# henryhcooperr/FaceRecognition-MultiArchitecture-Pipeline

Measured on AMD Instinct MI355X. Metric: faces/sec (224x224 embed+match), higher is better.
Workload: dtype bf16; 1 GPU; ResNet18 ('cnn') embed + L2-normalise + top-1 match, batch 256/GPU, 36-ID gallery, 224x224x3 fp32 NCHW inputs resident in HBM, seeded random-init weights with calibrated BatchNorm statistics (BASELINE.json configs[1]); global_batch=256, parallelism=dp1 (faces sharded, 1 all-gather of 8 B/face), execution=HIP graph replay, 2 concurrent micro-batch streams

## Files before the change

facerecognition-multiarchitecture-pipeline_amd/_lib.py:

```python
from __future__ import annotations

import ctypes as C
import os
import threading

_PKG_DIR = os.path.dirname(os.path.abspath(__file__))
LIB_PATH = os.environ.get("FRMAP_LIB") or os.path.join(_PKG_DIR, "libfrmap_hip.so")
ABI_VERSION = 10

_lock = threading.Lock()
_lib = None

_vp, _i, _f, _sz = C.c_void_p, C.c_int, C.c_float, C.c_size_t

PROTOTYPES = {
    "frmap_abi_version": (_i, []),
    "frmap_set_batch_invariant": (_i, [_i]),
    "frmap_last_error": (C.c_char_p, []),
    "frmap_pack_input_nchw_f32": (_i, [_vp, _vp, _i, _i, _i, _i, _vp]),
    "frmap_pack_conv_weight": (_i, [_vp, _vp, _i, _i, _i, _i, _i, _vp]),
    "frmap_small_cin_kpad": (_i, [_i, _i]),
    "frmap_pack_conv_weight_c3": (_i, [_vp, _vp, _i, _i, _i, _i, _vp]),
    "frmap_conv_small_cin": (_i, [_vp, _vp, _vp, _vp, _i, _i, _i, _i, _i, _i, _i, _i, _i, _i, _vp]),
    "frmap_match_gallery_pack_bytes": (_sz, [_i, _i]),
    "frmap_match_pack_gallery": (_i, [_vp, _vp, _vp, _i, _i, _vp]),
    "frmap_match_pack_gallery_rows": (_i, [_vp, _vp, _vp, _i, _i, _i, _i, _vp]),
    "frmap_match_top1_packed": (_i, [_vp, _vp, _vp, _vp, _vp, _vp, _vp, _vp, _f, _vp, _vp, _i, _i, _i, _vp]),
    "frmap_resize_bilinear_u8": (_i, [_vp, _vp, _vp, _vp, _i, _i, _i, _i, _i, _vp]),
    "frmap_crop_resize_u8": (_i, [_vp, _i, _vp, _vp, _i, _i, _i, _i, _i, _i, _vp]),
    "frmap_resize_coeffs_host": (_i, [_i, _i, _vp, _vp, _vp]),
    "frmap_align_crop_resize_u8": (_i, [_vp, _i, _vp, _vp, _vp, _i, _i, _i, _i, _i, _i, _vp]),
    "frmap_align_warp_host": (_i, [_vp, _i, _i, C.c_longlong, _vp, _i, _i, _i, _i, _i, _vp]),
    "frmap_track_state_bytes": (_sz, [_i, _i]),
    "frmap_track_step": (_i, [_vp, _vp, _vp, _vp, _vp, _i, _i, C.c_double, C.c_double, _vp, _vp, _vp]),
    "frmap_track_step_host": (_i, [_vp, _vp, _vp, _vp, _vp, _i, _i, C.c_double, C.c_double, _vp, _vp]),
    "frmap_track_fuse_state_bytes": (_sz, [_i, _i, _i]),
    "frmap_track_fuse": (_i, [_vp, _vp, _vp, _vp, _vp, _i, _i, _i, _i, _f, _vp, _vp, _vp]),
    "frmap_track_fuse_host": (_i, [_vp, _vp, _vp, _vp, _vp, _i, _i, _i, _i, _f, _vp, _vp]),
    "frmap_gap_linear_norm": (_i, [_vp, _vp, _vp, _vp, _vp, _vp, _f, _i, _i, _i, _i, _i, _i, _vp]),
    "frmap_conv_small_cin_pool2": (_i, [_vp, _vp, _vp, _vp, _i, _i, _i, _i, _i, _i, _vp]),
    "frmap_conv_igemm_pool2_supported": (_i, [_i, _i, _i, _i, _i]),
    "frmap_conv_igemm_pool2_form": (_i, [_i, _i, _i, _i, _i]),
    "frmap_conv3x3_pp_pool_layout": (_i, [_i, _i, _i, _i, _i]),
    "frmap_conv_igemm_pool2": (_i, [_vp, _vp, _vp, _vp, _i, _i, _i, _i, _i, _i, _i, _vp]),
    "frmap_stem7x7_maxpool": (_i, [_vp, _vp, _vp, _vp, _i, _i, _i, _i, _vp]),
    "frmap_stem7x7_maxpool2": (_i, [_vp, _vp, _vp, _vp, _i, _i, _i, _i, _vp]),
    "frmap_stem7x7_maxpool_u8": (_i, [_vp, C.POINTER(C.c_float), C.POINTER(C.c_float), _vp, _vp, _vp, _i, _i, _i, _i, _i, _vp]),
    "frmap_conv_igemm": (_i, [_vp, _vp, _vp, _vp, _vp, _i, _i, _i, _i, _i, _i, _i, _i, _i, _i, _vp]),
    "frmap_conv_pp_tuning": (_i, [_i, _i, _i]),
    "frmap_conv_pp_ri": (_i, [_i]),
    "frmap_conv_pp_pitch": (_i, [_i]),
    "frmap_conv_pp_ds": (_i, [_i]),
    "frmap_conv_pp_im": (_i, [_i]),
    "frmap_conv1x1_pp_layout": (_i, [_i, _i, _i, _i, _i, _i]),
    "frmap_conv3x3_pp_layout": (_i, [_i, _i, _i, _i, _i]),
    "frmap_conv3x3s2_pp_layout": (_i, [_i, _i, _i, _i, _i]),
    "frmap_conv3x3_pp_ds_layout": (_i, [_i, _i, _i, _i, _i, _i, _i, _i, _i]),
    "frmap_conv_igemm_ds_supported": (_i, [_i, _i, _i, _i, _i, _i, _i, _i, _i]),
    "frmap_conv_igemm_ds": (_i, [_vp, _vp, _vp, _vp, _vp, _vp, _i, _i, _i, _i, _i, _i, _i, _i, _i, _i, _i, _vp]),
    "frmap_linear_mfma_workspace_bytes": (_sz, [_i, _i, _i]),
    "frmap_linear_mfma": (_i, [_vp, _vp, _vp, _vp, _vp, _vp, _i, _i, _i, _i, _i, _vp]),
    "frmap_maxpool": (_i, [_vp, _vp, _i, _i, _i, _i, _i, _i, _i, _i, _vp]),
    "frmap_avgpool_global": (_i, [_vp, _vp, _i, _i, _i, _i, _vp]),
    "frmap_avgpool_adaptive": (_i, [_vp, _vp, _i, _i, _i, _i, _i, _i, _i, _vp]),
    "frmap_linear_f32": (_i, [_vp, _vp, _vp, _vp, _vp, _i, _i, _i, _i, _vp]),
    "frmap_l2_normalize_f32": (_i, [_vp, _vp, _i, _i, _f, _vp]),
    "frmap_cast_to_f32": (_i, [_vp, _vp, _sz, _i, _vp]),
    "frmap_cast_from_f32": (_i, [_vp, _vp, _sz, _i, _vp]),
    "frmap_add_pos_layernorm": (_i, [_vp, _vp, _vp, _vp, _vp, _vp, _i, _i, _i, _f, _i, _vp]),
    "frmap_mha_tokens": (_i, [_vp, _vp, _i, _i, _i, _i, _i, _vp]),
    "frmap_mean_layernorm": (_i, [_vp, _vp, _vp, _vp, _i, _i, _i, _f, _i, _vp]),
    "frmap_cnn_attention": (_i, [_vp, _vp, _vp, _vp, _vp, _vp, _vp, _i, _i, _i, _i, _i, _i, _i, _vp]),
    "frmap_normalize_u8_hwc": (_i, [_vp, _vp, _vp, _i, _i, _i, C.POINTER(C.c_float), C.POINTER(C.c_float), _i, _vp]),
    "frmap_softmax_argmax": (_i, [_vp, _vp, _vp, _i, _i, _vp]),
    "frmap_pairwise_distance": (_i, [_vp, _vp, _vp, _vp, _f, _i, _i, _vp]),
    "frmap_head_workspace_bytes": (_sz, [_i, _i]),
    "frmap_match_workspace_bytes": (_sz, [_i, _i]),
    "frmap_match_top1": (_i, [_vp, _vp, _vp, _vp, _vp, _vp, _f, _vp, _i, _i, _i, _vp]),
    "frmap_match_topk_workspace_bytes": (_sz, [_i, _i, _i, _i]),
    "frmap_match_topk": (_i, [_vp, _vp, _vp, _vp, _vp, _vp, _vp, _i, _i, _i, _i, _vp]),
    "frmap_match_topk_packed": (_i, [_vp, _vp, _vp, _vp, _vp, _vp, _vp, _vp, _vp, _i, _i, _i, _i, _vp]),
    "frmap_verify_workspace_bytes": (_sz, [_i, _i, _i, _i]),
    "frmap_verify_counts": (_i, [_vp, _vp, _i, _vp, _vp, _i, _i, _i, _vp, _i, _vp, _vp, _vp, _vp]),
    "frmap_verify_counts_packed": (_i, [_vp, _vp, _i, _vp, _vp, _vp, _vp, _i, _i, _i, _vp, _i, _vp, _vp, _vp, _vp]),
    "frmap_match_radius_workspace_bytes": (_sz, [_i, _i, _i]),
    "frmap_match_radius": (_i, [_vp, _vp, _i, _vp, _vp, _i, _i, _i, _f, _i, _vp, _vp, _vp, _vp, C.c_longlong, _vp, _vp, _vp]),
    "frmap_match_radius_packed": (_i, [_vp, _vp, _i, _vp, _vp, _vp, _vp, _i, _i, _i, _f, _i, _vp, _vp, _vp, _vp, C.c_longlong, _vp,
                                       _vp, _vp]),
    "frmap_gap_norm_match": (_i, [_vp, _vp, _vp, _vp, _vp, _vp, _vp, _f, _i, _f, _i, _i, _i, _i, _i, _vp]),
    "frmap_cosine_logits": (_i, [_vp, _vp, _vp, _vp, _vp, _i, _i, _i, _f, _vp]),
    "frmap_arcmargin_eval": (_i, [_vp, _vp, _vp, _vp, _vp, _vp, _i, _i, _i, _f, _f, _i, _vp]),
    "frmap_model_create": (_i, [C.POINTER(_vp), C.c_char_p, _i, _i]),
    "frmap_model_load_tensor": (_i, [_vp, C.c_char_p, _vp, _sz, _i]),
    "frmap_model_set_input_normalization": (_i, [_vp, C.POINTER(C.c_float), C.POINTER(C.c_float)]),
    "frmap_model_finalize": (_i, [_vp, _vp]),
    "frmap_model_embedding_dim": (_i, [_vp]),
    "frmap_model_workspace_bytes": (_sz, [_vp, _i, _i, _i]),
    "frmap_model_match_workspace_bytes": (_sz, [_vp, _i, _i, _i, _i]),
    "frmap_model_forward": (_i, [_vp, _vp, _i, _i, _i, _i, _i, _vp, _vp, _vp]),
    "frmap_model_embed_and_match": (_i, [_vp, _vp, _i, _i, _i, _i, _vp, _vp, _vp, _i, _f, _i, _vp, _vp, _vp, _vp, _vp, _vp, _vp]),
    "frmap_model_search_workspace_bytes": (_sz, [_vp, _i, _i, _i, _i, _i]),
    "frmap_model_embed_and_search": (_i, [_vp, _vp, _i, _i, _i, _i, _vp, _vp, _vp, _vp, _i, _i, _i, _vp, _vp, _vp, _vp, _vp, _vp]),
    "frmap_model_trace": (_i, [_vp, _i]),
    "frmap_model_trace_read": (_i, [_vp, _vp, _i]),
    "frmap_model_destroy": (None, [_vp]),
}


def lib_available() -> bool:
    return os.path.isfile(LIB_PATH)


def load() -> C.CDLL:
    global _lib
    if _lib is not None:
        return _lib
    with _lock:
        if _lib is not None:
            return _lib
        if not lib_available():
            raise RuntimeError(
                f"HIP extension not built: {LIB_PATH} is missing. Build it with "
                "`python -c 'import __graft_entry__ as g; g.build()'` (hipcc --offload-arch=gfx950). "
                "There is no CPU / PyTorch fallback for this path.")
        lib = C.CDLL(LIB_PATH)
        for name, (res, args) in PROTOTYPES.items():
            fn = getattr(lib, name)
            fn.restype = res
            fn.argtypes = args
        if lib.frmap_abi_version() != ABI_VERSION:
            raise RuntimeError(f"libfrmap_hip.so ABI {lib.frmap_abi_version()} != expected {ABI_VERSION}; rebuild")
        _lib = lib
    return _lib


def check(rc: int, what: str) -> None:
# ... 6 lines not shown
```

facerecognition-multiarchitecture-pipeline_amd/csrc/conv_igemm.hip:

```cpp
#include "frmap_common.h"
#include <stdlib.h>
#include <string.h>

struct ConvParams {
  const void* in;
  const void* wpk;
  const float* shift;
  const void* res;
  void* out;
  int N, Hi, Wi, Cin, Ho, Wo, Cout;
  int stride, pad, relu;
  int M, HoWo, Hp, Wp;
  uint32_t magic_Wp, magic_Hp;
  FrmapDiv dHoWo, dWo;
  int nchunks;
  int halo_bytes;
  int nblocks;
  int ksplit;
  float* slab;
  int dbg;
  const void* ds_in;
  const void* ds_w;
  int ds_Hi, ds_Wi, ds_Cin, ds_stride, ds_chunks;
  FrmapPoolOrder pool;
// ... 873 lines not shown
  u32x4_t hv[CKS][NIT], wv[CKS];
  auto prefetch = [&](int stg) {
#pragma unroll
    for (int sc = 0; sc < CKS; ++sc) {
#pragma unroll
      for (int it = 0; it < NIT; ++it) hv[sc][it] = *(const u32x4_t*)(inp + gsrc[it] + (size_t)(stg * CKS + sc) * 32);
      wv[sc] = *(const u32x4_t*)(wbase + (size_t)(stg * CKS + sc) * 4096);
    }
  };
  f32x4_t acc[MI][NI];
#pragma unroll
  for (int mi = 0; mi < MI; ++mi)
#pragma unroll
    for (int ni = 0; ni < NI; ++ni) acc[mi][ni] = (f32x4_t){0.f, 0.f, 0.f, 0.f};

  if (st_lo < st_hi) prefetch(st_lo);
  for (int stg = st_lo; stg < st_hi; ++stg) {
    if (stg > st_lo) __syncthreads();
#pragma unroll
    for (int sc = 0; sc < CKS; ++sc) {
      *(u32x4_t*)(wl + sc * 4096 + tid * 16) = wv[sc];
#pragma unroll
      for (int it = 0; it < NIT; ++it)
        *(u32x4_t*)(halo + sc * (BM * 64) + px_off<1>((it * 256 + tid) >> 2, tid & 3)) = hv[sc][it];
    }
    __syncthreads();
    if (stg + 1 < st_hi) prefetch(stg + 1);
#pragma unroll
    for (int sc = 0; sc < CKS; ++sc) {
      vec8 wf[NI], pf[MI];
#pragma unroll
      for (int ni = 0; ni < NI; ++ni) wf[ni] = *(const vec8*)(wl + sc * 4096 + ni * 1024 + woff);
#pragma unroll
      for (int mi = 0; mi < MI; ++mi) pf[mi] = *(const vec8*)(halo + sc * (BM * 64) + poff[mi]);
#pragma unroll
      for (int mi = 0; mi < MI; ++mi)
#pragma unroll
        for (int ni = 0; ni < NI; ++ni) acc[mi][ni] = TT::mfma(wf[ni], pf[mi], acc[mi][ni]);
    }
  }
  __syncthreads();
  if (p.ksplit > 1)
    conv_epilogue_partial<MI, NI>(acc, smem + wave * (16 * (NI * 64 + 16)), m0 + wave * 64, p.M, p.Cout, nt << 6,
                                  p.slab + (size_t)kslice * p.M * p.Cout, lane);
  else
    conv_epilogue<TT, MI, NI>(acc, smem + wave * (16 * (NI * 64 + 16)), m0 + wave * 64, p.M, p.Cout, nt << 6, p.shift,
                              (const typename TT::elem*)p.res, (typename TT::elem*)p.out, p.relu, lane);
}

template <typename TT>
__global__ void splitk_finalize_kernel(const float* __restrict__ slab, int ksplit, const float* __restrict__ shift,
                                       const typename TT::elem* __restrict__ res, typename TT::elem* __restrict__ out,
                                       size_t MN, int N, int act) {
  size_t i = ((size_t)blockIdx.x * blockDim.x + threadIdx.x) * 4;
  const size_t stride = (size_t)gridDim.x * blockDim.x * 4;
  for (; i < MN; i += stride) {
    f32x4_t a = *(const f32x4_t*)(slab + i);
    for (int s = 1; s < ksplit; ++s) {
      const f32x4_t b = *(const f32x4_t*)(slab + (size_t)s * MN + i);
      a[0] += b[0]; a[1] += b[1]; a[2] += b[2]; a[3] += b[3];
    }
    const int n = (int)(i % N);
    const f32x4_t sh = *(const f32x4_t*)(shift + n);
    float v[4] = {a[0] + sh[0], a[1] + sh[1], a[2] + sh[2], a[3] + sh[3]};
    if (res) {
      float r[4];
      unpack4<TT>(*(const u32x2_t*)(res + i), r);
      v[0] += r[0]; v[1] += r[1]; v[2] += r[2]; v[3] += r[3];
    }
#pragma unroll
    for (int e = 0; e < 4; ++e) {
      if (act == 1) v[e] = fmaxf(v[e], 0.f);
      else if (act == 2) v[e] = 0.5f * v[e] * (1.0f + erff(v[e] * 0.70710678118654752f));
    }
    *(u32x2_t*)(out + i) = pack4<TT>(v[0], v[1], v[2], v[3]);
  }
}

static ConvPlan plan_of(const ConvLayer& L) { return conv_plan(L, conv_tuning(), frmap_cu_count(), frmap_batch_invariant() != 0); }
ConvPlan frmap_conv_plan(const ConvLayer& L) { return plan_of(L); }

struct ConvPtrs {
  const void* in; const void* w; const float* shift; const void* res; void* out;
  const void* ds_in; const void* ds_w; float* slab;
};

static ConvParams conv_params(const ConvLayer& L, const ConvPlan& q, const ConvPtrs& a, int relu, int dbg) {
  ConvParams p{};
  p.in = a.in; p.wpk = a.w; p.shift = a.shift; p.res = a.res; p.out = a.out;
  p.N = L.B; p.Hi = L.Hi; p.Wi = L.Wi; p.Cin = L.Cin; p.Ho = L.Ho(); p.Wo = L.Wo(); p.Cout = L.Cout;
  p.stride = L.stride; p.pad = L.pad; p.relu = relu;
  p.M = L.B * p.Ho * p.Wo; p.HoWo = p.Ho * p.Wo; p.Hp = L.Hi + 2 * L.pad; p.Wp = q.Wp;
  p.magic_Wp = frmap_magic((uint32_t)p.Wp); p.magic_Hp = frmap_magic((uint32_t)p.Hp);
  p.dHoWo = frmap_div_make((uint32_t)p.HoWo); p.dWo = frmap_div_make((uint32_t)p.Wo);
  p.nchunks = L.Cin / 32 / (q.kernel == CK_1X1 ? q.CKS : 1);
  p.halo_bytes = q.halo_bytes; p.nblocks = q.nblocks;
  p.ksplit = q.ksplit; p.slab = a.slab; p.dbg = dbg;
  if (L.fuse == FUSE_SHORTCUT) {
    p.ds_in = a.ds_in; p.ds_w = a.ds_w; p.ds_Hi = L.ds_Hi; p.ds_Wi = L.ds_Wi; p.ds_Cin = L.ds_Cin; p.ds_stride = L.ds_stride;
    p.ds_chunks = L.ds_Cin / 32;
  }
  if (L.fuse == FUSE_POOL2) {
    p.pool.Wo2 = L.Wi / 2; p.pool.Win = (L.Hi / 2) * (L.Wi / 2);
    p.pool.dWo2 = frmap_div_make((uint32_t)p.pool.Wo2); p.pool.dWin = frmap_div_make((uint32_t)p.pool.Win);
  }
  return p;
}

typedef void (*conv_kern_t)(const ConvParams);
template <typename TT>
static conv_kern_t conv_kernel(const ConvPlan& q) {
  switch (q.kernel) {
    case CK_IGEMM:
      if (q.POOL) return q.BM == 256 ? conv_igemm_kernel<TT, 256, 3, 1, true> : conv_igemm_kernel<TT, 128, 3, 1, true>;
      if (q.KS == 1) return conv_igemm_kernel<TT, 256, 1, 1>;
      if (q.BM == 256) return q.SWZ == 1 ? conv_igemm_kernel<TT, 256, 3, 1> : conv_igemm_kernel<TT, 256, 3, 2>;
      return q.SWZ == 1 ? conv_igemm_kernel<TT, 128, 3, 1> : conv_igemm_kernel<TT, 128, 3, 2>;
    case CK_1X1: return q.CKS == 4 ? conv1x1_kernel<TT, 4> : (q.CKS == 2 ? conv1x1_kernel<TT, 2> : conv1x1_kernel<TT, 1>);
    case CK_WAVE:
      if (!q.POOL) return conv3x3_c64_wave_kernel<TT, 2, false>;
      return q.NCH == 2 ? conv3x3_c64_wave_kernel<TT, 2, true> : conv3x3_c64_wave_kernel<TT, 1, true>;
    case CK_FAST: return q.DS ? conv3x3_fast_kernel<TT, true> : conv3x3_fast_kernel<TT, false>;
    case CK_S2_SPLIT: return conv3x3s2_split_kernel<TT>;
    case CK_S2_FAST: return conv3x3s2_fast_kernel<TT>;
    default: return nullptr;
  }
}

static int conv_launch(const ConvPlan& q, const ConvParams& p, int dtype, hipStream_t st) {
  const conv_kern_t kern = dtype == FRMAP_BF16 ? conv_kernel<BF16>(q) : conv_kernel<F16>(q);
  FRMAP_REQUIRE(kern, "conv_igemm: no kernel for plan %d", q.kernel);
  if (frmap_big_lds((const void*)kern, 160 * 1024)) return -2;
  hipLaunchKernelGGL(kern, dim3(q.nblocks), dim3(q.kernel == CK_WAVE ? 512 : 256), q.lds_bytes, st, p);
  FRMAP_LAUNCH_CHECK();
  return 0;
}

static int conv_run(const ConvLayer& L, const ConvPlan& q, const ConvPtrs& a, int relu, int dtype, hipStream_t st) {
  if (q.kernel >= CK_PP) return frmap_conv_pp_launch(L, q, a.in, a.w, a.shift, a.res, a.out, a.ds_in, a.ds_w, relu, dtype, st);
  return conv_launch(q, conv_params(L, q, a, relu, L.fuse == FUSE_POOL2 ? 0 : conv_tuning().debug), dtype, st);
}

static int conv_igemm_impl(const ConvLayer& L, const ConvPtrs& a, int relu, int dtype, void* stream) {
  FRMAP_REQUIRE(a.in && a.w && a.shift && a.out, "conv_igemm: null pointer");
  FRMAP_REQUIRE(L.K == 1 || L.K == 3, "conv_igemm: kernel size %d not supported (1 or 3)", L.K);
  FRMAP_REQUIRE(L.stride == 1 || L.stride == 2, "conv_igemm: stride %d not supported", L.stride);
  FRMAP_REQUIRE((L.K == 3 && L.pad == 1) || (L.K == 1 && L.pad == 0), "conv_igemm: pad %d with K=%d not supported", L.pad, L.K);
  FRMAP_REQUIRE(L.Cin > 0 && L.Cin % 32 == 0, "conv_igemm: Cin=%d must be a multiple of 32", L.Cin);
  FRMAP_REQUIRE(L.Cout > 0 && L.Cout % 64 == 0, "conv_igemm: Cout=%d must be a multiple of 64", L.Cout);
  FRMAP_REQUIRE(dtype == FRMAP_BF16 || dtype == FRMAP_F16, "conv_igemm: bad dtype %d", dtype);
  FRMAP_REQUIRE(L.B > 0 && L.Hi > 0 && L.Wi > 0, "conv_igemm: empty input");
  FRMAP_REQUIRE(L.Ho() > 0 && L.Wo() > 0, "conv_igemm: empty output");
  FRMAP_REQUIRE((long long)L.B * L.Ho() * L.Wo() < (1ll << 31), "conv_igemm: too many output pixels");
  FRMAP_REQUIRE(L.Wi + 2 * L.pad < 32768 && L.Hi + 2 * L.pad < 32768, "conv_igemm: image too large");
  const ConvPlan q = plan_of(L);
  FRMAP_REQUIRE(q.taken(), "%s", q.error);
  return conv_run(L, q, a, relu, dtype, (hipStream_t)stream);
}

extern "C" int frmap_conv_igemm(const void* in, const void* w_packed, const float* shift, const void* residual,
                                void* out, int B, int Hi, int Wi, int Cin, int Cout, int K, int stride, int pad,
                                int relu, int dtype, void* stream) {
  const ConvLayer L = {B, Hi, Wi, Cin, Cout, K, stride, pad, residual ? FUSE_RESIDUAL : FUSE_NONE, 0, 0, 0, 0};
  return conv_igemm_impl(L, ConvPtrs{in, w_packed, shift, residual, out, nullptr, nullptr, nullptr}, relu, dtype, stream);
}

extern "C" int frmap_conv_igemm_ds_supported(int B, int Hi, int Wi, int Cin, int Cout, int ds_Hi, int ds_Wi, int ds_Cin,
                                             int ds_stride) {
  const ConvLayer L = {B, Hi, Wi, Cin, Cout, 3, 1, 1, FUSE_SHORTCUT, ds_Hi, ds_Wi, ds_Cin, ds_stride};
  return conv_ds_supported(L, conv_tuning(), frmap_batch_invariant() != 0);
}

extern "C" int frmap_conv_igemm_ds(const void* in, const void* w_packed, const float* shift, const void* ds_in,
                                   const void* ds_w_packed, void* out, int B, int Hi, int Wi, int Cin, int Cout,
                                   int ds_Hi, int ds_Wi, int ds_Cin, int ds_stride, int relu, int dtype, void* stream) {
  FRMAP_REQUIRE(ds_in && ds_w_packed, "conv_igemm_ds: null shortcut pointer");
  const ConvLayer L = {B, Hi, Wi, Cin, Cout, 3, 1, 1, FUSE_SHORTCUT, ds_Hi, ds_Wi, ds_Cin, ds_stride};
  return conv_igemm_impl(L, ConvPtrs{in, w_packed, shift, nullptr, out, ds_in, ds_w_packed, nullptr}, relu, dtype, stream);
}

extern "C" int frmap_conv_igemm_pool2_form(int B, int Hi, int Wi, int Cin, int Cout) {
  return plan_of(ConvLayer{B, Hi, Wi, Cin, Cout, 3, 1, 1, FUSE_POOL2, 0, 0, 0, 0}).layout;
}
extern "C" int frmap_conv_igemm_pool2_supported(int B, int Hi, int Wi, int Cin, int Cout) {
  const int f = frmap_conv_igemm_pool2_form(B, Hi, Wi, Cin, Cout);
  return f >= 2 || (f == 1 && Cin <= 96);
}

extern "C" int frmap_conv_igemm_pool2(const void* in, const void* w_packed, const float* shift, void* out, int B, int Hi,
                                      int Wi, int Cin, int Cout, int relu, int dtype, void* stream) {
  FRMAP_REQUIRE(in && w_packed && shift && out, "conv_igemm_pool2: null pointer");
  FRMAP_REQUIRE(dtype == FRMAP_BF16 || dtype == FRMAP_F16, "conv_igemm_pool2: bad dtype %d", dtype);
  FRMAP_REQUIRE(relu == 0 || relu == 1, "conv_igemm_pool2: activation %d does not commute with the max", relu);
  const ConvLayer L = {B, Hi, Wi, Cin, Cout, 3, 1, 1, FUSE_POOL2, 0, 0, 0, 0};
  const ConvPlan q = plan_of(L);
  FRMAP_REQUIRE(q.taken(),
                "conv_igemm_pool2: shape B=%d %dx%d Cin=%d Cout=%d not taken (even H and W, Cin %% 32 == 0, Cout %% 64 == 0, rows fit LDS)",
                B, Hi, Wi, Cin, Cout);
  return conv_run(L, q, ConvPtrs{in, w_packed, shift, nullptr, out, nullptr, nullptr, nullptr}, relu, dtype, (hipStream_t)stream);
}

extern "C" size_t frmap_linear_mfma_workspace_bytes(int M, int K, int N) {
  if (M <= 0 || K <= 0 || N <= 0) return 0;
  const int ks = linear_ksplit(M, K, N, frmap_batch_invariant() != 0);
  return ks > 1 ? (size_t)ks * M * N * sizeof(float) : 0;
}

extern "C" int frmap_linear_mfma(const void* x, const void* w_packed, const float* shift, const void* residual, void* out,
                                 void* workspace, int M, int K, int N, int act, int dtype, void* stream) {
  FRMAP_REQUIRE(x && w_packed && shift && out, "linear_mfma: null pointer");
  FRMAP_REQUIRE(M > 0 && K > 0 && K % 32 == 0 && N > 0 && N % 64 == 0, "linear_mfma: need K %% 32 == 0 and N %% 64 == 0 (M=%d K=%d N=%d)", M, K, N);
  FRMAP_REQUIRE(dtype == FRMAP_BF16 || dtype == FRMAP_F16, "linear_mfma: bad dtype");
  const int ks = linear_ksplit(M, K, N, frmap_batch_invariant() != 0);
  if (ks == 1) return frmap_conv_igemm(x, w_packed, shift, residual, out, M, 1, 1, K, N, 1, 1, 0, act, dtype, stream);
  FRMAP_REQUIRE(workspace, "linear_mfma: workspace required (frmap_linear_mfma_workspace_bytes)");
  const ConvLayer L = {M, 1, 1, K, N, 1, 1, 0, FUSE_NONE, 0, 0, 0, 0};
  const ConvPlan q = plan_1x1(L, ks);
  if (q.ksplit < 2) return frmap_conv_igemm(x, w_packed, shift, residual, out, M, 1, 1, K, N, 1, 1, 0, act, dtype, stream);
  hipStream_t st = (hipStream_t)stream;
  const int rc = conv_launch(q, conv_params(L, q, ConvPtrs{x, w_packed, shift, nullptr, out, nullptr, nullptr, (float*)workspace}, 0, 0), dtype, st);
  if (rc) return rc;
  const size_t MN = (size_t)M * N;
  const int blocks = (int)((MN / 4 + 255) / 256 < 4096 ? (MN / 4 + 255) / 256 : 4096);
  if (dtype == FRMAP_BF16)
    hipLaunchKernelGGL(splitk_finalize_kernel<BF16>, dim3(blocks), dim3(256), 0, st, (const float*)workspace, q.ksplit, shift,
                       (const __bf16*)residual, (__bf16*)out, MN, N, act);
  else
    hipLaunchKernelGGL(splitk_finalize_kernel<F16>, dim3(blocks), dim3(256), 0, st, (const float*)workspace, q.ksplit, shift,
                       (const _Float16*)residual, (_Float16*)out, MN, N, act);
  FRMAP_LAUNCH_CHECK();
  return 0;
}
```

facerecognition-multiarchitecture-pipeline_amd/csrc/conv_plan.cpp:

```cpp
#include "conv_plan.h"

#include <stdio.h>
#include <stdlib.h>
#include <string.h>

#include <array>
#include <map>
#include <mutex>

static int env_int(const char* name, int dflt) {
  const char* e = getenv(name);
  return e ? atoi(e) : dflt;
}

ConvTuning& conv_tuning() {
  static ConvTuning t = [] {
    ConvTuning v{};
    v.debug = env_int("FRMAP_CONV_DEBUG", 0);
    v.s2fast = env_int("FRMAP_CONV_S2FAST", 1);
    v.wres = env_int("FRMAP_CONV_WRES", 1);
    v.dsfuse = env_int("FRMAP_CONV_DSFUSE", 1);
    v.ds_unfuse_small = env_int("FRMAP_DS_UNFUSE_SMALL", 0);
    v.pool_wave = env_int("FRMAP_POOL_WAVE", 1);
    v.pool_min_cin = env_int("FRMAP_PP_POOL_MIN_CIN", 128);
    v.pp = env_int("FRMAP_CONV_PP", 1);
    v.pp_s2 = env_int("FRMAP_CONV_PP_S2", 1);
    v.pp_pool = env_int("FRMAP_CONV_PP_POOL", 1);
    v.pp_1x1 = env_int("FRMAP_CONV_PP_1X1", 1);
    v.pp_ds = env_int("FRMAP_CONV_PP_DS", 1);
    v.min_tiles = env_int("FRMAP_PP_MIN_TILES", 200);
    v.min_cin = env_int("FRMAP_PP_MIN_CIN", 128);
    v.s2_min_cin = env_int("FRMAP_PP_S2_MIN_CIN", 64);
    v.tile_px = env_int("FRMAP_PP_TILE_PX", 0);
    v.bn = env_int("FRMAP_PP_BN", 0);
    v.pitch = env_int("FRMAP_PP_PITCH", 0);
    v.ri = env_int("FRMAP_PP_RI", 0);
    v.im = env_int("FRMAP_PP_IM", 0);
    v.h_on = v.h_px = v.h_bn = v.h_ks = v.h_ds = v.h_pitch = v.h_im = v.h_ri = -1;
    return v;
  }();
  return t;
}

static const long long LDS_MAX = 160 * 1024, LDS_HALF = 80 * 1024;

static long long round1k(long long v) { return (v + 1023) & ~1023ll; }

static int plan_lds(const ConvPlan& q) {
  int lds = 0, scratch = 4 * 16 * (4 * 64 + 16);
  const int wb = (q.KS == 2 ? 2 : 8 / (q.WM ? q.WM : 8)) * 64 * 64;
  const int xch = q.KS == 2 ? 4 * q.MI * 4 * 1024 : 0;
  switch (q.kernel) {
    case CK_IGEMM: case CK_FAST: lds = q.halo_bytes + q.KS * q.KS * 4096; break;
    case CK_S2_SPLIT: case CK_S2_FAST: lds = q.halo_bytes + 6 * 4096; break;
    case CK_1X1: lds = q.CKS * (256 * 64 + 4096); break;
    case CK_WAVE: lds = q.NCH * 9 * 4096 + 8 * (10 * 16 * 64); break;
    case CK_PP:
      lds = q.KS * (2 * q.NHP * (8 / q.KS) * 1024 + (q.RI && q.KS == 1 ? 5 : 4) * wb) + (q.DS ? ((q.WM * q.MI + 7) / 8) * 8192 : 0);
      break;
    case CK_PP_S2: lds = 4 * q.NHP * 8192 + 4 * wb; break;
    case CK_PP_1X1: {
      const int cap = (q.KS == 2 ? 2 : q.WM) * q.MI * 16, gw = 8 / q.KS, ngp = (cap / 16 + gw - 1) / gw;
      lds = q.KS * (3 * ngp * gw * 1024 + 4 * wb);
      break;
    }
  }
  if (q.kernel >= CK_PP) scratch *= 2;
  if (lds < scratch) lds = scratch;
  if (q.kernel >= CK_PP && lds < xch) lds = xch;
  return lds;
}
static ConvPlan finish(ConvPlan q, const char* label) {
  q.label = label;
  if (q.kernel >= CK_PP) q.nblocks = q.mtiles * q.ntiles;
  if (!q.ksplit) q.ksplit = 1;
  if (!q.wg_per_cu) q.wg_per_cu = 1;
  q.lds_bytes = plan_lds(q);
  return q;
}

static int halo_rows_bound(int BM, int Ho, int Wo, int Hp, int stride, int KS) {
  const int rows = (BM + Wo - 2) / Wo + 1;
  const int cross = (BM + Ho * Wo - 2) / (Ho * Wo);
  const int cross_step = Hp - (Ho - 1) * stride;
  const int x = cross < rows - 1 ? cross : rows - 1;
  int gdiff = (rows - 1 - x) * stride + x * (cross_step > stride ? cross_step : stride);
  return gdiff + KS;
}
static int pool_rows_bound(int BM, int Ho, int Wo) {
  const int nw = BM / 4, Wo2 = Wo / 2, Win = (Ho / 2) * Wo2;
  const int pairs = (nw + Wo2 - 2) / Wo2 + 1;
  const int cross = (nw + Win - 2) / Win;
  const int x = cross < pairs - 1 ? cross : pairs - 1;
  return 2 * pairs + 2 * x + 2;
}
static bool prefetch_offsets_fit(int HoWo, long long H, long long W, long long C) { return (256 / HoWo + 3) * H * W * C * 2 < (1ll << 31); }

int pp_max_rows(long long M, int tile_px, int howo, int wo, int hp, int extra, bool inv) {
  if (inv) M = (long long)howo * tile_px;
  static std::mutex mu;
  static std::map<std::array<long long, 6>, int> memo;
  const std::array<long long, 6> key = {M, tile_px, howo, wo, hp, extra};
  {
    std::lock_guard<std::mutex> lock(mu);
    auto it = memo.find(key);
    if (it != memo.end()) return it->second;
  }
  int best = 0;
  const long long mtiles = (M + tile_px - 1) / tile_px;
  const long long lim = mtiles < howo ? mtiles : howo;
  for (long long mt = 0; mt < lim; ++mt) {
    const long long m0 = mt * tile_px, mend = (m0 + tile_px < M ? m0 + tile_px : M) - 1;
    const long long n0 = m0 / howo, n1 = mend / howo;
    const int oy0 = (int)((m0 - n0 * howo) / wo), oy1 = (int)((mend - n1 * howo) / wo);
    const int rows = (int)(n1 - n0) * hp + oy1 - oy0 + extra;
    if (rows > best) best = rows;
  }
  {
    std::lock_guard<std::mutex> lock(mu);
    if (memo.size() > 4096) memo.clear();
    memo[key] = best;
  }
  return best;
}

static int pp_tile_px(int cap, int H, int W, int forced_env, int forced_hook) {
  int tile_px;
  if (H * W <= cap) tile_px = (cap / (H * W)) * H * W;
  else {
    int rows = cap / W;
    for (int r = rows; r * 8 >= rows * 7 && r >= 1; --r)
      if (H % r == 0) { rows = r; break; }
    tile_px = rows * W;
  }
  if (forced_env > 0 && forced_env <= cap) tile_px = forced_env;
  if (forced_hook > 0 && forced_hook <= cap) tile_px = forced_hook;
  return tile_px;
}
static int pp_bn(int Cout, int forced_env, int forced_hook) {
  int bn = Cout % 256 == 0 ? 256 : 128;
  if (forced_env == 128 || forced_env == 256) bn = (forced_env == 256 && Cout % 256) ? 128 : forced_env;
  if (forced_hook == 128 || forced_hook == 256) bn = (forced_hook == 256 && Cout % 256) ? 128 : forced_hook;
  return bn;
}
static bool pp_sizes_fit(long long M, long long in_elems) { return M < (1ll << 31) && in_elems * 2 < (1ll << 46); }

ConvPlan plan_pp_3x3(const ConvLayer& L, const ConvTuning& t, bool inv) {
  constexpr int MI = 7;
  ConvPlan q{};
  const int B = L.B, Hi = L.Hi, Wi = L.Wi, Cin = L.Cin, Cout = L.Cout;
  const bool has_ds = L.fuse == FUSE_SHORTCUT;
  if (!t.pp_enabled(1, Cin, t.min_cin)) return q;
  if (Cin % 32 || Cin > 1024 || Cout % 128) return q;
  const long long Mll = (long long)B * Hi * Wi;
  if (!pp_sizes_fit(Mll, Mll * Cin)) return q;
  const int Hp = Hi + 2;
  int Wp = Wi + 2;
  if (ConvTuning::pick(t.h_pitch, t.pitch)) { while (Wp % 8 != Wi % 8) ++Wp; }
  if (has_ds) {
    if (L.ds_Cin <= 0 || L.ds_Cin % 32 || L.ds_stride < 1 || (L.ds_Hi - 1) / L.ds_stride + 1 != Hi ||
        (L.ds_Wi - 1) / L.ds_stride + 1 != Wi || (long long)B * L.ds_Hi * L.ds_Wi * L.ds_Cin * 2 >= (1ll << 46))
      return q;
    if (!ConvTuning::pick(t.h_ds, t.pp_ds) && !t.forced()) return q;
  }
  auto layout = [&](int cap, int bn, int ks, int& tile_px, int& mtiles, int& ntiles, int& hbytes_out) -> int {
    if (Wi > cap || Cout % bn || (ks == 2 && (Cin / 32) % 2)) return 0;
    tile_px = pp_tile_px(cap, Hi, Wi, t.tile_px, t.h_px);
    mtiles = (int)((Mll + tile_px - 1) / tile_px);
    ntiles = Cout / bn;
    const long long hbytes = (long long)pp_max_rows(Mll, tile_px, Hi * Wi, Wi, Hp, 3, inv) * Wp * 64;
    if (hbytes / 64 >= 65536) return 0;
    hbytes_out = (int)hbytes;
    const int per = (8 / ks) * 1024;
    const int nhp = (int)((hbytes + per - 1) / per);
    return nhp <= (ks == 2 ? 6 : 5) ? nhp : 0;
  };
  int tpx = 0, mtl = 0, ntl = 0, hby = 0, ks = 1, bn = pp_bn(Cout, t.bn, t.h_bn);
  int nhp = layout(bn == 256 ? 2 * MI * 16 : 4 * MI * 16, bn, 1, tpx, mtl, ntl, hby);
  const bool want_ks2 = !has_ds && !inv && (t.h_ks == 2 || (t.h_ks < 0 && (!nhp || (long long)mtl * ntl < t.min_tiles)));
  if (want_ks2 && t.h_ks != 1) {
    int t2 = 0, m2 = 0, n2 = 0, h2 = 0;
    const int nhp2 = layout(2 * MI * 16, 128, 2, t2, m2, n2, h2);
    if (nhp2 && (t.h_ks == 2 || !nhp || (long long)m2 * n2 > (long long)mtl * ntl)) {
      nhp = nhp2; tpx = t2; mtl = m2; ntl = n2; hby = h2; ks = 2; bn = 128;
    }
  }
  if (!nhp) return q;
  if (!inv && !t.forced() && (long long)mtl * ntl < t.min_tiles / 2) return q;
  if (!inv && has_ds && (long long)mtl * ntl < t.min_tiles && !t.forced()) return q;
  q.kernel = CK_PP; q.MI = MI; q.KS = ks; q.DS = has_ds;
  q.tile_px = tpx; q.mtiles = mtl; q.ntiles = ntl; q.Wp = Wp; q.halo_bytes = hby;
  q.layout = ks == 2 ? 3 : (bn == 256 ? 1 : 2);
  q.WM = bn == 256 || ks == 2 ? 2 : 4;
  if (has_ds) {
    q.NHP = bn == 256 && nhp <= 3 ? 3 : 5;
    return finish(q, "conv3x3_pp_kernel<%s, DS>");
  }
  q.RI = ConvTuning::pick(t.h_ri, t.ri) != 0 && !(ks == 2 && nhp > 4);
  q.IM = !q.RI && ConvTuning::pick(t.h_im, t.im) != 0;
  q.NHP = ks == 2 ? (nhp <= 4 ? 4 : 6) : (nhp <= 3 ? 3 : 5);
  return finish(q, "conv3x3_pp_kernel<%s>");
}

ConvPlan plan_pp_s2(const ConvLayer& L, const ConvTuning& t, bool inv) {
  constexpr int MI = 7;
  ConvPlan q{};
  const int B = L.B, Hi = L.Hi, Wi = L.Wi, Cin = L.Cin, Cout = L.Cout;
  if (!t.pp_enabled(t.pp_s2, Cin, t.s2_min_cin)) return q;
  if (Hi % 2 || Wi % 2 || Cin % 32 || Cin > 1024 || Cout % 128) return q;
  const int Ho = Hi / 2, Wo = Wi / 2;
  const long long Mll = (long long)B * Ho * Wo;
  if (!pp_sizes_fit(Mll, (long long)B * Hi * Wi * Cin) || (long long)Hi * Wi * Cin * 2 >= (1ll << 31)) return q;
  const int bn = pp_bn(Cout, 0, t.h_bn);
  const int cap = (bn == 256 ? 2 : 4) * MI * 16;
  if (Wo > cap) return q;
  const int tile_px = pp_tile_px(cap, Ho, Wo, 0, t.h_px);
  q.MI = MI; q.WM = bn == 256 ? 2 : 4; q.KS = 1;
  q.Wp = Wo + 1;
  q.tile_px = tile_px;
  q.mtiles = (int)((Mll + tile_px - 1) / tile_px);
  q.ntiles = Cout / bn;
  const long long hbytes = (long long)pp_max_rows(Mll, tile_px, Ho * Wo, Wo, Ho + 1, 2, inv) * q.Wp * 64;
  if (hbytes / 64 >= 65536) return q;
  q.halo_bytes = (int)hbytes;
  const int need = (int)((hbytes + 8191) / 8192);
  q.NHP = need <= 1 ? 1 : (need <= 2 ? 2 : (need <= 4 ? 4 : 0));
  if (!q.NHP || (q.NHP == 4 && bn == 256)) return q;
  if (!inv && !t.forced() && (long long)q.mtiles * q.ntiles < t.min_tiles) return q;
  q.kernel = CK_PP_S2;
  q.layout = bn == 256 ? 1 : 2;
  return finish(q, "conv3x3s2_pp_kernel<%s>");
}

ConvPlan plan_pp_pool(const ConvLayer& L, const ConvTuning& t, bool inv) {
  ConvPlan q{};
  const int B = L.B, Hi = L.Hi, Wi = L.Wi, Cin = L.Cin, Cout = L.Cout;
  if (!t.pp_enabled(t.pp_pool, Cin, 0)) return q;
  if (Hi % 2 || Wi % 2 || 112 % (2 * Wi) || Cin % 32 || Cin > 1024 || Cout % 128) return q;
  const long long Mll = (long long)B * Hi * Wi;
  if (!pp_sizes_fit(Mll, Mll * Cin)) return q;
  q.Wp = Wi + 2;
  int bn = pp_bn(Cout, 0, t.h_bn), nhp = 0;
  for (int attempt = 0; attempt < 2 && !nhp; ++attempt) {
    const int tile_px = (bn == 256 ? 2 : 4) * 112;
    const long long hbytes = (long long)pp_max_rows(Mll, tile_px, Hi * Wi, Wi, Hi + 2, 3, inv) * q.Wp * 64;
    const int n = (int)((hbytes + 8191) / 8192);
    if (hbytes / 64 < 65536 && n <= 5) { nhp = n; q.tile_px = tile_px; q.halo_bytes = (int)hbytes; }
    else bn = bn == 256 ? 128 : 256;
    if (!nhp && Cout % bn) break;
  }
  if (!nhp) return q;
  q.kernel = CK_PP; q.PL = true; q.MI = 7; q.KS = 1;
  q.WM = bn == 256 ? 2 : 4; q.NHP = nhp <= 3 ? 3 : 5;
  q.mtiles = (int)((Mll + q.tile_px - 1) / q.tile_px); q.ntiles = Cout / bn;
  q.layout = 3;
  return finish(q, "conv3x3_pp_kernel<%s, PL>");
}

ConvPlan plan_pp_1x1(const ConvLayer& L, const ConvTuning& t, int cus, bool inv) {
  ConvPlan q{};
  const int B = L.B, Hi = L.Hi, Wi = L.Wi, Cin = L.Cin, Cout = L.Cout, stride = L.stride;
  if (!t.pp_enabled(t.pp_1x1, Cin, 0)) return q;
  if (inv && !t.forced()) return q;
  if (Cin % 32 || Cin > 16384 || Cout % 128 || stride < 1) return q;
  const int Ho = (Hi - 1) / stride + 1, Wo = (Wi - 1) / stride + 1, nchunks = Cin / 32;
  const long long Mll = (long long)B * Ho * Wo;
  if (!pp_sizes_fit(Mll, (long long)B * Hi * Wi * Cin)) return q;
  auto est_us = [&](int lay) -> double {
    if (lay == 1 && Cout % 256) return 1e30;
    if (lay == 3 && nchunks % 2) return 1e30;
    const int px = lay == 2 ? 448 : 224, bn = lay == 1 ? 256 : 128;
    const long long tiles = ((Mll + px - 1) / px) * (Cout / bn);
    const long long rounds = (tiles + cus - 1) / cus;
    return (double)rounds * ((lay == 3 ? nchunks / 2 : nchunks) * 0.6 + 7.5);
  };
  int layout = 0;
  double best = 1e30;
  for (int lay = 1; lay <= 3; ++lay) {
    if (t.h_bn == 256 && t.h_ks != 2 && lay != 1 && Cout % 256 == 0) continue;
    if (t.h_bn == 128 && t.h_ks == 1 && lay != 2) continue;
    if (t.h_ks == 2 && lay != 3 && nchunks % 2 == 0) continue;
    const double e = est_us(lay);
    if (e < best) { best = e; layout = lay; }
  }
  if (!layout || best >= 1e30) return q;
  if (!t.forced()) {
    const double gen1_us = 2.0 * (double)Mll * Cin * Cout / 470e6;
    if (best > 0.9 * gen1_us || t.min_tiles < 0) return q;
  }
  q.kernel = CK_PP_1X1; q.MI = 7; q.WM = layout == 2 ? 4 : 2; q.KS = layout == 3 ? 2 : 1;
  q.Wp = Wo;
  q.tile_px = layout == 2 ? 448 : 224;
  q.mtiles = (int)((Mll + q.tile_px - 1) / q.tile_px);
  q.ntiles = Cout / (layout == 1 ? 256 : 128);
  q.layout = layout;
  return finish(q, "conv1x1_pp_kernel<%s>");
}

ConvPlan match_gemm_plan(int P, int Gpad) {
  const long long t1 = ((P + 223) / 224) * (long long)(Gpad / 256), t2 = ((P + 447) / 448) * (long long)(Gpad / 128);
  const long long r1 = (t1 + 255) / 256, r2 = (t2 + 255) / 256;
  const bool wide = r2 < r1 || (r2 == r1 && t2 > t1);
  ConvPlan q{};
  q.kernel = CK_PP_1X1; q.MI = 7; q.WM = wide ? 4 : 2; q.KS = 1;
  q.Wp = 1;
  q.tile_px = wide ? 448 : 224;
  q.mtiles = (P + q.tile_px - 1) / q.tile_px;
  q.ntiles = Gpad / (wide ? 128 : 256);
  q.layout = wide ? 2 : 1;
  return finish(q, "conv1x1_pp_kernel<F16, MATCH>");
}

ConvPlan plan_wave(const ConvLayer& L, const ConvTuning& t, int cus) {
// ... 145 lines not shown
```

facerecognition-multiarchitecture-pipeline_amd/csrc/conv_plan.h:

```cpp
#pragma once
#include <stdint.h>

struct ConvTuning {
  int debug;
  int s2fast;
  int wres;
  int dsfuse;
  int ds_unfuse_small;
  int pool_wave;
  int pool_min_cin;
  int pp;
  int pp_s2, pp_pool, pp_1x1;
  int pp_ds;
  int min_tiles;
  int min_cin;
  int s2_min_cin;
  int tile_px, bn;
  int pitch;
  int ri;
  int im;
  int h_on, h_px, h_bn, h_ks, h_ds, h_pitch, h_im, h_ri;

  void set_tuning(int enable, int px, int bn_) {
    h_on = enable;
    h_px = px;
    h_bn = bn_ == 1282 ? 128 : bn_;
    h_ks = bn_ == 1282 ? 2 : (bn_ == 128 || bn_ == 256 ? 1 : -1);
  }
  bool forced() const { return h_on >= 0; }
  bool pp_enabled(int family_on, int cin, int cin_min) const { return h_on >= 0 ? h_on != 0 : (pp && family_on && cin >= cin_min); }
  static int pick(int hook, int env) { return hook >= 0 ? hook : env; }
};
ConvTuning& conv_tuning();

enum ConvFuse { FUSE_NONE = 0, FUSE_RESIDUAL, FUSE_SHORTCUT, FUSE_POOL2 };
struct ConvLayer {
  int B, Hi, Wi, Cin, Cout, K, stride, pad;
  int fuse;
  int ds_Hi, ds_Wi, ds_Cin, ds_stride;
  int Ho() const { return (Hi + 2 * pad - K) / stride + 1; }
  int Wo() const { return (Wi + 2 * pad - K) / stride + 1; }
};

enum ConvKernel {
  CK_NONE = 0,
  CK_IGEMM,
  CK_1X1,
  CK_WAVE,
  CK_FAST,
  CK_S2_SPLIT,
  CK_S2_FAST,
  CK_PP,
  CK_PP_S2,
  CK_PP_1X1,
};
struct ConvPlan {
  int kernel;
  int BM, KS, SWZ, CKS, NCH;
  int MI, WM, NHP;
  bool DS, IM, PL, RI, POOL;
  int tile_px, mtiles, ntiles;
  int nblocks;
  int halo_bytes, Wp, lds_bytes, ksplit;
  int wg_per_cu;
  int layout;
  const char* label;
  char error[112];
  bool taken() const { return kernel != CK_NONE; }
};

ConvPlan plan_pp_3x3(const ConvLayer& L, const ConvTuning& t, bool inv);
ConvPlan plan_pp_s2(const ConvLayer& L, const ConvTuning& t, bool inv);
ConvPlan plan_pp_pool(const ConvLayer& L, const ConvTuning& t, bool inv);
ConvPlan plan_pp_1x1(const ConvLayer& L, const ConvTuning& t, int cus, bool inv);
ConvPlan plan_wave(const ConvLayer& L, const ConvTuning& t, int cus);
ConvPlan plan_fast(const ConvLayer& L, const ConvTuning& t);
ConvPlan plan_s2(const ConvLayer& L, const ConvTuning& t);
ConvPlan plan_1x1(const ConvLayer& L, int ksplit);
ConvPlan plan_generic(const ConvLayer& L);

ConvPlan conv_plan(const ConvLayer& L, const ConvTuning& t, int cus, bool inv);

int conv_ds_supported(const ConvLayer& L, const ConvTuning& t, bool inv);

int linear_ksplit(int M, int K, int N, bool inv);
ConvPlan match_gemm_plan(int P, int Gpad);

int pp_max_rows(long long M, int tile_px, int howo, int wo, int hp, int extra, bool inv);
```

facerecognition-multiarchitecture-pipeline_amd/csrc/conv_pp.hip:

```cpp
#include "frmap_common.h"
#include <stdlib.h>
#include <string.h>

#include <utility>

struct PPParams {
  const void* in;
  const void* wpk;
  const float* shift;
  const void* res;
  void* out;
  int N, Hi, Wi, Cin, Cout, relu;
  int M, HoWo, Hp, Wp;
  uint32_t magic_Wp, magic_Hp;
  FrmapDiv dHoWo, dWo;
  int nchunks;
  int tile_px;
  int mtiles, ntiles;
  const void* ds_in;
  const void* ds_w;
  int ds_Hi, ds_Wi, ds_Cin, ds_stride, dsc;
  int Wo2;
  FrmapDiv dWo2;
  const float* m_stat_a;
  const float* m_stat_w;
  void* m_records;
  int m_G, m_D;
};
struct PPHistParams : PPParams {
  const float* h_A;
  const float* h_B;
  const int32_t* h_lab_a;
  const int32_t* h_lab_b;
  const float* h_tab;
  unsigned long long* h_hist;
  unsigned long long* h_rescored;
  int h_row0, h_T;
};
struct PPJoinParams : PPParams {
  const float* j_A;
  const float* j_B;
  const int32_t* j_lab_a;
  const int32_t* j_lab_b;
  RadiusOut j_out;
  unsigned long long* j_rescored;
  float j_hi;
  int j_row0, j_filter;
};
template <int MM> struct PPArg { using type = PPParams; };
template <> struct PPArg<MATCH_HIST> { using type = PPHistParams; };
template <> struct PPArg<MATCH_JOIN> { using type = PPJoinParams; };
__device__ __forceinline__ bool pp_hist_self(const PPParams&) { return false; }
__device__ __forceinline__ bool pp_hist_self(const PPHistParams& p) { return p.h_row0 >= 0; }
__device__ __forceinline__ bool pp_hist_self(const PPJoinParams& p) { return p.j_row0 >= 0; }

__device__ __attribute__((aligned(4096))) unsigned int g_pp_zero[1024];

__device__ __forceinline__ int pp_xcd_remap(int b, int nb) {
  const int qd = nb >> 3, rm = nb & 7, xcd = b & 7;
  return (xcd < rm ? xcd * (qd + 1) : rm * (qd + 1) + (xcd - rm) * qd) + (b >> 3);
}

__device__ __forceinline__ void pp_dma16(const void* gsrc, unsigned lds_base) {
  unsigned keep;
  asm volatile("s_mov_b32 %0, m0\n\ts_mov_b32 m0, %2\n\ts_nop 0\n\tglobal_load_lds_dwordx4 %1, off\n\ts_mov_b32 m0, %0"
               : "=&s"(keep)
               : "v"(gsrc), "s"(lds_base)
               : "memory");
}
template <int N>
__device__ __forceinline__ void pp_wait_vm() {
  asm volatile("s_waitcnt vmcnt(%0)" ::"i"(N) : "memory");
}
__device__ __forceinline__ void pp_wait_lgkm0() { asm volatile("s_waitcnt lgkmcnt(0)" ::: "memory"); }
__device__ __forceinline__ void pp_barrier() {
  __builtin_amdgcn_sched_barrier(0);
  asm volatile("s_barrier" ::: "memory");
  __builtin_amdgcn_sched_barrier(0);
}

template <int... Is, typename F>
__device__ __forceinline__ void pp_static_for(std::integer_sequence<int, Is...>, F&& f) {
  (f(std::integral_constant<int, Is>{}), ...);
}

template <typename TT, int MI, int WM, int NHP, int KS, bool DS, bool IM = false, bool PL = false, bool RI = false>
__global__ __launch_bounds__(512, 2) void conv3x3_pp_kernel(const PPParams p) {
  static_assert(!(DS && KS == 2), "the fused shortcut is built for the pixel-split layouts only");
  static_assert(!RI || (!DS && !IM), "the interleaved fragment reads are built for the plain layers");
  static_assert(!PL || (KS == 1 && !DS && !IM), "the pooled epilogue is built for the plain pixel-split layouts");
  static_assert(!(DS && IM), "the fused shortcut keeps its DMA in the LOAD segments");
  constexpr int NI = 4, WN = KS == 2 ? 2 : 8 / WM;
  constexpr int CAP = WM * MI * 16;
  constexpr int NGP = DS ? (CAP / 16 + 7) / 8 : 0;
  constexpr int GBYTES = NGP * 8 * 1024;
  constexpr int XT = DS ? 8 - NHP : 1;
  constexpr int PPT = DS ? (NGP + XT - 1) / XT : 0;
  constexpr int TAPS = 9, BN = WN * 64, WB = BN * 64;
  constexpr int GW = 8 / KS;
  constexpr int NWI = (WB / 1024) / GW;
  constexpr int RING = (RI && KS == 1) ? 5 : 4;
  constexpr int HB = NHP * GW * 1024;
  constexpr int GSZ = 2 * HB + RING * WB;
  constexpr int PD = (RI && KS == 1) ? 3 : 2;
  auto slot_of = [](int k) { return RING == 4 ? (k & 3) : k % RING; };
  using vec8 = typename TT::vec8;
  using elem = typename TT::elem;
  extern __shared__ __attribute__((aligned(16))) char smem[];
  const unsigned lds0 = (unsigned)(uintptr_t)(__attribute__((address_space(3))) char*)smem;
  const int tid = threadIdx.x, lane = tid & 63;
  const int wave = __builtin_amdgcn_readfirstlane(tid >> 6);
  const int grp = wave >> 2, q = wave & 3;
  const int gw = KS == 2 ? q : wave;
  const int wn = (KS == 2 || WM == 4) ? (wave & 1) : q;
  const int mslice = KS == 2 ? (q >> 1) : (WM == 2 ? grp : grp * 2 + (q >> 1));
  const int gbase = KS == 2 ? grp * GSZ : 0;
  const int lr = lane & 15, g = lane >> 4;

  const int L = pp_xcd_remap(blockIdx.x, gridDim.x);
  const int mt = L / p.ntiles, nt = L - mt * p.ntiles;
  const int m0 = mt * p.tile_px, mend = min(m0 + p.tile_px, p.M);
  const int nch = p.nchunks / KS;
  const int nk = nch * TAPS;

  const int n0 = frmap_div(m0, p.dHoWo), oy0 = frmap_div(m0 - n0 * p.HoWo, p.dWo);
  const int n1 = frmap_div(mend - 1, p.dHoWo), oy1 = frmap_div(mend - 1 - n1 * p.HoWo, p.dWo);
  const int nrows = (n1 - n0) * p.Hp + oy1 - oy0 + 3;
  const int nitems = nrows * p.Wp * 4;

  const char* hsrc[NHP];
#pragma unroll
  for (int j = 0; j < NHP; ++j) {
    const int item = ((gw + GW * j) << 6) + lane;
    const int px = item >> 2, ps = item & 3;
    const int cg = ps ^ (((px >> 2) & 1) << 1);
    const int r = (int)fast_div((uint32_t)px, p.magic_Wp);
    const int c = px - r * p.Wp;
    const int rr = oy0 + r;
    const int dn = (int)fast_div((uint32_t)rr, p.magic_Hp);
    const int iy = rr - dn * p.Hp - 1, ix = c - 1, n = n0 + dn;
    const bool ok = item < nitems && n < p.N && (unsigned)iy < (unsigned)p.Hi && (unsigned)ix < (unsigned)p.Wi;
    hsrc[j] = ok ? (const char*)p.in + ((((size_t)n * p.Hi + iy) * p.Wi + ix) * p.Cin + cg * 8) * sizeof(elem)
                 : (const char*)g_pp_zero + cg * 16;
  }
  const int wblk = NWI == 2 ? (gw >> 1) : (gw >> 2);
  const int wpart = NWI == 2 ? ((gw & 1) << 1) : (gw & 3);
  const char* wsrc = (const char*)p.wpk + ((size_t)(nt * (BN / 64) + wblk) * p.nchunks * TAPS) * 4096 + wpart * 1024 + lane * 16;
  const unsigned wdst = lds0 + gbase + 2 * HB + wblk * 4096 + wpart * 1024;
  const unsigned hdst = lds0 + gbase + gw * 1024;

  const char* gsrc[DS ? NGP : 1];
  const char* wsrc_ds = nullptr;
  if (DS) {
    const size_t img = (size_t)p.ds_Hi * p.ds_Wi * p.ds_Cin;
#pragma unroll
    for (int e = 0; e < NGP; ++e) {
      const int item = ((wave + 8 * e) << 6) + lane;
      const int px = item >> 2, ps = item & 3;
      const int cg = ps ^ (((px >> 2) & 1) << 1);
      const int m = m0 + px;
      const int n = frmap_div(min(m, p.M - 1), p.dHoWo), rem = min(m, p.M - 1) - n * p.HoWo, oy = frmap_div(rem, p.dWo), ox = rem - oy * p.Wi;
      gsrc[e] = (px < CAP && m < mend)
                    ? (const char*)p.ds_in + ((size_t)n * img + ((size_t)(oy * p.ds_stride) * p.ds_Wi + ox * p.ds_stride) * p.ds_Cin + cg * 8) * sizeof(elem)
                    : (const char*)g_pp_zero + cg * 16;
    }
    wsrc_ds = (const char*)p.ds_w + ((size_t)(nt * (BN / 64) + wblk) * p.dsc) * 4096 + wpart * 1024 + lane * 16;
  }
  auto gbuf = [&](int d) -> unsigned {
    const int r = d % 3;
    return r == 0 ? (unsigned)(nch & 1) * HB : (r == 1 ? (unsigned)(2 * HB + RING * WB) : (unsigned)((nch - 1) & 1) * HB);
// ... 163 lines not shown
        for (int mi = 0; mi < MI; ++mi) asm volatile("" : "+v"(A[mi]));
#pragma unroll
        for (int mi = 0; mi < MI; ++mi) {
#pragma unroll
          for (int ni = 0; ni < NI; ++ni) acc[mi][ni] = TT::mfma(CUR ? wf1[ni] : wf0[ni], pf[mi], acc[mi][ni]);
          __builtin_amdgcn_sched_barrier(0);
          pf[mi] = *(const vec8*)(hb1 + frag_addr(mi, toff1));
          if (mi < NI) {
            if (CUR) wf0[mi] = *(const vec8*)(sl1 + mi * 1024);
            else wf1[mi] = *(const vec8*)(sl1 + mi * 1024);
          }
          __builtin_amdgcn_sched_barrier(0);
        }
        pp_barrier();
      });
    };
    int ci = 0;
    for (; ci + 1 < nch; ci += 2) {
      chunk_ri(ci, std::integral_constant<int, 0>{});
      chunk_ri(ci + 1, std::integral_constant<int, 1>{});
    }
    if (ci < nch) chunk_ri(ci, std::integral_constant<int, 0>{});
  } else if (DS) {
    for (int ci = 0; ci + 1 < nch; ++ci) chunk_body(ci, std::false_type{});
    chunk_body(nch - 1, std::true_type{});
  } else {
    for (int ci = 0; ci < nch; ++ci) chunk_body(ci, std::false_type{});
  }
  if (DS) {
    int Ag[MI];
#pragma unroll
    for (int mi = 0; mi < MI; ++mi) {
      const int at = ((((mslice * MI + mi) << 4) + lr) << 6) | (g << 4);
      Ag[mi] = at ^ ((at >> 3) & 32);
    }
    for (int d = 0; d < p.dsc; ++d) {
      const int k = nk + d;
      vec8 wf[NI], pf[MI];
      {
        const char* sl = slabs + slot_of(k) * WB;
#pragma unroll
        for (int ni = 0; ni < NI; ++ni) wf[ni] = *(const vec8*)(sl + ni * 1024);
        const char* gb = smem + gbuf(d);
#pragma unroll
        for (int mi = 0; mi < MI; ++mi) pf[mi] = *(const vec8*)(gb + Ag[mi]);
      }
#pragma unroll
      for (int e = 0; e < NGP; ++e) issue_gather(d + 2, e);
      issue_slab(nch + (d + 2) / TAPS, (d + 2) % TAPS, slot_of(k + 2));
      pp_wait_vm<NWI + NGP>();
      pp_wait_lgkm0();
      pp_barrier();
      __builtin_amdgcn_sched_barrier(0);
#pragma unroll
      for (int ni = 0; ni < NI; ++ni)
#pragma unroll
        for (int mi = 0; mi < MI; ++mi) acc[mi][ni] = TT::mfma(wf[ni], pf[mi], acc[mi][ni]);
      pp_barrier();
    }
  }
  if (grp == 0) pp_barrier();
  pp_wait_vm<0>();
  pp_barrier();

  if (KS == 2) {
    char* xch = smem + (size_t)q * (MI * NI * 1024) + lane * 16;
    if (grp == 1) {
#pragma unroll
      for (int mi = 0; mi < MI; ++mi)
#pragma unroll
        for (int ni = 0; ni < NI; ++ni) *(f32x4_t*)(xch + (mi * NI + ni) * 1024) = acc[mi][ni];
    }
    __syncthreads();
    if (grp == 0) {
#pragma unroll
      for (int mi = 0; mi < MI; ++mi)
#pragma unroll
        for (int ni = 0; ni < NI; ++ni) {
          const f32x4_t o = *(const f32x4_t*)(xch + (mi * NI + ni) * 1024);
          acc[mi][ni][0] += o[0]; acc[mi][ni][1] += o[1]; acc[mi][ni][2] += o[2]; acc[mi][ni][3] += o[3];
        }
    }
    __syncthreads();
    if (grp == 1) return;
  }

  if constexpr (PL)
    conv_epilogue_pool2<TT, MI, NI>(acc, smem + wave * (16 * (NI * 64 + 16)), (m0 + mslice * (MI * 16)) >> 2, mend >> 2, p.Cout,
                                    nt * BN + wn * 64, p.shift, (elem*)p.out, p.relu, lane);
  else
    conv_epilogue<TT, MI, NI>(acc, smem + (KS == 2 ? q : wave) * (16 * (NI * 64 + 16)), m0 + mslice * (MI * 16), mend, p.Cout,
                              nt * BN + wn * 64, p.shift, (const elem*)p.res, (elem*)p.out, p.relu, lane);
}

template <typename TT, int MI, int WM, int KS, int MM = MATCH_NONE>
__global__ __launch_bounds__(512, 2) void conv1x1_pp_kernel(const typename PPArg<MM>::type p) {
  constexpr int NI = 4, WN = KS == 2 ? 2 : 8 / WM;
  constexpr int CAP = (KS == 2 ? 2 : WM) * MI * 16;
  constexpr int BN = WN * 64, WB = BN * 64;
  constexpr int GW = 8 / KS;
  constexpr int NWI = (WB / 1024) / GW;
  constexpr int NGP = (CAP / 16 + GW - 1) / GW;
  constexpr int IMGB = NGP * GW * 1024;
  constexpr int RING = 4;
  constexpr int GSZ = 3 * IMGB + RING * WB;
  using vec8 = typename TT::vec8;
  using elem = typename TT::elem;
  extern __shared__ __attribute__((aligned(16))) char smem[];
  const unsigned lds0 = (unsigned)(uintptr_t)(__attribute__((address_space(3))) char*)smem;
  const int tid = threadIdx.x, lane = tid & 63;
  const int wave = __builtin_amdgcn_readfirstlane(tid >> 6);
  const int grp = wave >> 2, q = wave & 3;
  const int gw = KS == 2 ? q : wave;
  const int wn = (KS == 2 || WM == 4) ? (wave & 1) : q;
  const int mslice = KS == 2 ? (q >> 1) : (WM == 2 ? grp : grp * 2 + (q >> 1));
  const int gbase = KS == 2 ? grp * GSZ : 0;
  const int lr = lane & 15, g = lane >> 4;

  const int L = pp_hist_self(p) ? (int)blockIdx.x : pp_xcd_remap(blockIdx.x, gridDim.x);
  const int mt = L / p.ntiles, nt = L - mt * p.ntiles;
  const int m0 = mt * p.tile_px, mend = min(m0 + p.tile_px, p.M);
  if constexpr (MM == MATCH_HIST) {
    if (p.h_row0 >= 0 && nt * BN + BN - 1 <= p.h_row0 + m0) return;
  }
  if constexpr (MM == MATCH_JOIN) {
    if (p.j_row0 >= 0 && nt * BN + BN - 1 <= p.j_row0 + m0) return;
  }
  const int nst = p.nchunks / KS;

  const char* gsrc[NGP];
#pragma unroll
  for (int e = 0; e < NGP; ++e) {
    const int item = ((gw + GW * e) << 6) + lane;
    const int px = item >> 2, ps = item & 3;
    const int cg = ps ^ (((px >> 2) & 1) << 1);
    const int m = min(m0 + px, p.M - 1);
    const int n = frmap_div(m, p.dHoWo), rem = m - n * p.HoWo, oy = frmap_div(rem, p.dWo), ox = rem - oy * p.Wp;
    gsrc[e] = (px < CAP && m0 + px < mend)
                  ? (const char*)p.in + ((((size_t)n * p.Hi + (size_t)(oy * p.ds_stride)) * p.Wi + (size_t)(ox * p.ds_stride)) * p.Cin + cg * 8) * sizeof(elem)
                  : (const char*)g_pp_zero + cg * 16;
  }
  const int wblk = NWI == 2 ? (gw >> 1) : (gw >> 2);
  const int wpart = NWI == 2 ? ((gw & 1) << 1) : (gw & 3);
  const char* wsrc = (const char*)p.wpk + ((size_t)(nt * (BN / 64) + wblk) * p.nchunks) * 4096 + wpart * 1024 + lane * 16;
  const unsigned wdst = lds0 + gbase + 3 * IMGB + wblk * 4096 + wpart * 1024;
  const unsigned gdst = lds0 + gbase + gw * 1024;

  auto chunk_of = [&](int st) { return KS == 2 ? grp + 2 * st : st; };
  auto issue_step = [&](int st) {
    const int sc = st < nst ? st : nst - 1;
    const size_t coff = (size_t)chunk_of(sc) * 64;
#pragma unroll
    for (int e = 0; e < NGP; ++e)
      pp_dma16(st < nst ? gsrc[e] + coff : (const char*)g_pp_zero, gdst + (unsigned)(st % 3) * IMGB + e * (GW * 1024));
    const char* sp = wsrc + (size_t)chunk_of(sc) * 4096;
    const unsigned dp = wdst + (unsigned)(st & (RING - 1)) * WB;
    pp_dma16(sp, dp);
    if (NWI == 2) pp_dma16(sp + 1024, dp + 1024);
  };
  issue_step(0);
  issue_step(1);

  int Ag[MI];
#pragma unroll
  for (int mi = 0; mi < MI; ++mi) {
    const int at = ((((mslice * MI + mi) << 4) + lr) << 6) | (g << 4);
    Ag[mi] = at ^ ((at >> 3) & 32);
// ... 14 lines not shown

  for (int st = 0; st < nst; ++st) {
    vec8 wf[NI], pf[MI];
    {
      const char* sl = slabs + (st & (RING - 1)) * WB;
#pragma unroll
      for (int ni = 0; ni < NI; ++ni) wf[ni] = *(const vec8*)(sl + ni * 1024);
      const char* gb = imgs + (st % 3) * IMGB;
#pragma unroll
      for (int mi = 0; mi < MI; ++mi) pf[mi] = *(const vec8*)(gb + Ag[mi]);
    }
    issue_step(st + 2);
    pp_wait_vm<NWI + NGP>();
    pp_wait_lgkm0();
    pp_barrier();
    __builtin_amdgcn_sched_barrier(0);
#pragma unroll
    for (int ni = 0; ni < NI; ++ni)
#pragma unroll
      for (int mi = 0; mi < MI; ++mi) acc[mi][ni] = TT::mfma(wf[ni], pf[mi], acc[mi][ni]);
    pp_barrier();
  }
  if (grp == 0) pp_barrier();
  pp_wait_vm<0>();
  pp_barrier();

  if (KS == 2) {
    char* xch = smem + (size_t)q * (MI * NI * 1024) + lane * 16;
    if (grp == 1) {
#pragma unroll
      for (int mi = 0; mi < MI; ++mi)
#pragma unroll
        for (int ni = 0; ni < NI; ++ni) *(f32x4_t*)(xch + (mi * NI + ni) * 1024) = acc[mi][ni];
    }
    __syncthreads();
    if (grp == 0) {
#pragma unroll
      for (int mi = 0; mi < MI; ++mi)
#pragma unroll
        for (int ni = 0; ni < NI; ++ni) {
          const f32x4_t o = *(const f32x4_t*)(xch + (mi * NI + ni) * 1024);
          acc[mi][ni][0] += o[0]; acc[mi][ni][1] += o[1]; acc[mi][ni][2] += o[2]; acc[mi][ni][3] += o[3];
        }
    }
    __syncthreads();
    if (grp == 1) return;
  }
  if constexpr (MM == MATCH_HIST) {
    unsigned* hist = (unsigned*)(smem + VERIFY_LDS_HIST);
    float* tl = (float*)(smem + VERIFY_LDS_T);
    const int T = p.h_T, nb = 2 * (T + 1);
    for (int i = tid; i < nb; i += 512) hist[i] = 0u;
    for (int i = tid; i < 3 * T; i += 512) tl[(i / T) * VERIFY_MAX_T + i % T] = p.h_tab[i];
    __syncthreads();
    const int b_base = m0 + mslice * (MI * 16), n0 = nt * BN + wn * 64;
    unsigned short* queue = (unsigned short*)(smem + VERIFY_LDS_Q) + wave * VERIFY_QCAP;
    const int cnt = match_epilogue_hist<MI>(acc, b_base, mend, n0, p.m_G, p.m_D, p.M, p.m_stat_a, p.m_stat_w, p.h_lab_a, p.h_lab_b,
                                            p.h_row0, (const float*)(smem + VERIFY_LDS_LO), (const float*)(smem + VERIFY_LDS_HI),
                                            hist, queue, T, lane);
    verify_drain_queue(queue, cnt, b_base, n0, p.h_A, p.h_B, p.h_lab_a, p.h_lab_b, p.m_D, tl, hist, T, lane);
    if (lane == 0 && cnt) atomicAdd(p.h_rescored, (unsigned long long)cnt);
    __syncthreads();
    for (int i = tid; i < nb; i += 512)
      if (hist[i]) atomicAdd(p.h_hist + i, (unsigned long long)hist[i]);
    return;
  } else if constexpr (MM == MATCH_JOIN) {
    const int b_base = m0 + mslice * (MI * 16), n0 = nt * BN + wn * 64;
    unsigned short* queue = (unsigned short*)smem + wave * VERIFY_QCAP;
    const int cnt = match_epilogue_join<MI>(acc, b_base, mend, n0, p.m_G, p.m_D, p.M, p.m_stat_a, p.m_stat_w, p.j_lab_a, p.j_lab_b,
                                            p.j_row0, p.j_filter, p.j_hi, queue, lane);
    int* obuf = (int*)(smem + 8 * VERIFY_QCAP * 2 + wave * RADIUS_OB_BYTES);
    radius_drain_queue(queue, cnt, b_base, n0, p.j_A, p.j_B, p.m_D, p.j_out, obuf, lane);
    if (lane == 0 && cnt) atomicAdd(p.j_rescored, (unsigned long long)cnt);
    return;
  } else if constexpr (MM != MATCH_NONE) {
    match_epilogue<MM, MI>(acc, m0 + mslice * (MI * 16), mend, nt * BN + wn * 64, p.m_G, p.m_D, p.M, p.m_stat_a, p.m_stat_w,
                           p.m_records, lane);
    return;
  }
  conv_epilogue<TT, MI, NI>(acc, smem + (KS == 2 ? q : wave) * (16 * (NI * 64 + 16)), m0 + mslice * (MI * 16), mend, p.Cout,
                            nt * BN + wn * 64, p.shift, (const elem*)p.res, (elem*)p.out, p.relu, lane);
}

template <typename TT, int MI, int WM, int NHP2>
__global__ __launch_bounds__(512, 2) void conv3x3s2_pp_kernel(const PPParams p) {
  constexpr int NI = 4, WN = 8 / WM;
  constexpr int TAPS = 9, BN = WN * 64, WB = BN * 64;
  constexpr int NWI = (WB / 1024) / 8;
  constexpr int RING = 4;
  constexpr int HB = NHP2 * 8 * 1024;
  constexpr int PPH = NHP2 >= 2 ? NHP2 / 2 : 1;
  using vec8 = typename TT::vec8;
  using elem = typename TT::elem;
  extern __shared__ __attribute__((aligned(16))) char smem[];
  const unsigned lds0 = (unsigned)(uintptr_t)(__attribute__((address_space(3))) char*)smem;
  const int tid = threadIdx.x, lane = tid & 63;
  const int wave = __builtin_amdgcn_readfirstlane(tid >> 6);
  const int grp = wave >> 2, q = wave & 3;
  const int wn = WM == 4 ? (wave & 1) : q;
  const int mslice = WM == 2 ? grp : grp * 2 + (q >> 1);
  const int lr = lane & 15, g = lane >> 4;

  const int L = pp_xcd_remap(blockIdx.x, gridDim.x);
  const int mt = L / p.ntiles, nt = L - mt * p.ntiles;
  const int m0 = mt * p.tile_px, mend = min(m0 + p.tile_px, p.M);
  const int nch = p.nchunks, nk = nch * TAPS;
  const int Wo = p.Wi >> 1;

  const int n0 = frmap_div(m0, p.dHoWo), oy0 = frmap_div(m0 - n0 * p.HoWo, p.dWo);
  const int n1 = frmap_div(mend - 1, p.dHoWo), oy1 = frmap_div(mend - 1 - n1 * p.HoWo, p.dWo);
  const int nrows = (n1 - n0) * p.Hp + oy1 - oy0 + 2;
  const int nitems = nrows * p.Wp * 4;

  const char* hsrc[NHP2];
  unsigned hval = 0;
#pragma unroll
  for (int j = 0; j < NHP2; ++j) {
    const int item = ((wave + 8 * j) << 6) + lane;
    const int px = item >> 2, ps = item & 3;
    const int cg = ps ^ (((px >> 2) & 1) << 1);
    const int r = (int)fast_div((uint32_t)px, p.magic_Wp);
    const int c = px - r * p.Wp;
    const int rr = oy0 + r;
    const int dn = (int)fast_div((uint32_t)rr, p.magic_Hp);
    const int yh = rr - dn * p.Hp - 1, xh = c - 1, n = n0 + dn;
    const bool ok = item < nitems && n < p.N && yh >= 0 && xh >= 0;
    hsrc[j] = ok ? (const char*)p.in + ((((size_t)n * p.Hi + 2 * yh) * p.Wi + 2 * xh) * p.Cin + cg * 8) * sizeof(elem)
                 : (const char*)g_pp_zero + cg * 16;
    hval |= ok ? (1u << j) : 0u;
  }
  const int wblk = NWI == 2 ? (wave >> 1) : (wave >> 2);
  const int wpart = NWI == 2 ? ((wave & 1) << 1) : (wave & 3);
  const char* wsrc = (const char*)p.wpk + ((size_t)(nt * (BN / 64) + wblk) * p.nchunks * TAPS) * 4096 + wpart * 1024 + lane * 16;
  const unsigned wdst = lds0 + 4 * HB + wblk * 4096 + wpart * 1024;
  const unsigned hdst = lds0 + wave * 1024;
  const int rowb = p.Wi * p.Cin * (int)sizeof(elem), pxb = p.Cin * (int)sizeof(elem);

  constexpr int TAP_OF[9] = {4, 3, 5, 1, 7, 0, 2, 6, 8};
  constexpr int IMG_OF[9] = {0, 1, 1, 2, 2, 3, 3, 3, 3};
  constexpr int A1_OF[9] = {1, 1, 1, 0, 1, 0, 0, 1, 1};
  constexpr int B1_OF[9] = {1, 0, 1, 1, 1, 0, 1, 0, 1};

  auto issue_slab = [&](int ci, int t, int slot) {
    const int cc = ci < nch ? ci : nch - 1;
    const int tap = ci < nch ? TAP_OF[t] : 8;
    const char* s = wsrc + (size_t)(cc * TAPS + tap) * 4096;
    const unsigned d = wdst + (unsigned)slot * WB;
    pp_dma16(s, d);
    if (NWI == 2) pp_dma16(s + 1024, d + 1024);
  };
  auto issue_img = [&](int ci, int sp, int j) {
    const int off = (sp >> 1) * rowb + (sp & 1) * pxb + ci * 64;
    const bool live = ci < nch && ((hval >> j) & 1u);
    const char* s = live ? hsrc[j] + off : (ci < nch ? hsrc[j] : (const char*)g_pp_zero);
    pp_dma16(s, hdst + (unsigned)sp * HB + j * 8192);
  };

#pragma unroll
  for (int sp = 0; sp < 3; ++sp)
#pragma unroll
    for (int j = 0; j < NHP2; ++j) issue_img(0, sp, j);
  issue_slab(0, 0, 0);
  issue_slab(0, 1, 1);

  int A[MI];
#pragma unroll
  for (int mi = 0; mi < MI; ++mi) {
    const int m = min(m0 + (mslice * MI + mi) * 16 + lr, mend - 1);
    const int n = frmap_div(m, p.dHoWo), rem = m - n * p.HoWo, oy = frmap_div(rem, p.dWo), ox = rem - oy * Wo;
    A[mi] = ((((n - n0) * p.Hp + oy - oy0) * p.Wp + ox) << 6) | (g << 4);
  }
  const int woff = (lr << 6) + ((g ^ (((lr >> 2) & 1) << 1)) << 4);
  const char* slabs = smem + 4 * HB + wn * 4096 + woff;

  f32x4_t acc[MI][NI];
#pragma unroll
  for (int mi = 0; mi < MI; ++mi)
#pragma unroll
    for (int ni = 0; ni < NI; ++ni) acc[mi][ni] = (f32x4_t){0.f, 0.f, 0.f, 0.f};

  pp_wait_vm<0>();
  pp_barrier();
  if (grp == 1) pp_barrier();

  for (int ci = 0; ci < nch; ++ci) {
    pp_static_for(std::make_integer_sequence<int, TAPS>{}, [&](auto tc) {
      constexpr int t = decltype(tc)::value;
      const int k = ci * TAPS + t;
      vec8 wf[NI], pf[MI];
      {
        const char* sl = slabs + (k & (RING - 1)) * WB;
#pragma unroll
        for (int ni = 0; ni < NI; ++ni) wf[ni] = *(const vec8*)(sl + ni * 1024);
        const char* hb = smem + IMG_OF[t] * HB;
        const int toff = (A1_OF[t] * p.Wp + B1_OF[t]) << 6;
#pragma unroll
        for (int mi = 0; mi < MI; ++mi) {
          const int at = A[mi] + toff;
          pf[mi] = *(const vec8*)(hb + (at ^ ((at >> 3) & 32)));
        }
      }
      constexpr int NH = t >= 1 ? ((NHP2 == 1 && ((t - 1) & 1)) ? 0 : PPH) : 0;
      if (t >= 1) {
        constexpr int qi = (t - 1) >> 1, h = (t - 1) & 1;
#pragma unroll
        for (int e = 0; e < NH; ++e) issue_img(qi == 0 ? ci : ci + 1, qi == 0 ? 3 : qi - 1, h * PPH + e);
      }
      issue_slab(t + 2 < TAPS ? ci : ci + 1, (t + 2) % TAPS, (k + 2) & (RING - 1));
      pp_wait_vm<NWI + NH>();
      pp_barrier();
      pp_wait_lgkm0();
      __builtin_amdgcn_sched_barrier(0);
#pragma unroll
      for (int ni = 0; ni < NI; ++ni)
#pragma unroll
        for (int mi = 0; mi < MI; ++mi) acc[mi][ni] = TT::mfma(wf[ni], pf[mi], acc[mi][ni]);
      pp_barrier();
    });
  }
  if (grp == 0) pp_barrier();
  pp_wait_vm<0>();
  pp_barrier();

  conv_epilogue<TT, MI, NI>(acc, smem + wave * (16 * (NI * 64 + 16)), m0 + mslice * (MI * 16), mend, p.Cout,
                            nt * BN + wn * 64, p.shift, (const elem*)p.res, (elem*)p.out, p.relu, lane);
}

extern "C" int frmap_conv_pp_tuning(int enable, int tile_px, int bn) { conv_tuning().set_tuning(enable, tile_px, bn); return 0; }
extern "C" int frmap_conv_pp_pitch(int v) { conv_tuning().h_pitch = v; return 0; }
extern "C" int frmap_conv_pp_ds(int v) { conv_tuning().h_ds = v; return 0; }
extern "C" int frmap_conv_pp_im(int v) { conv_tuning().h_im = v; return 0; }
extern "C" int frmap_conv_pp_ri(int v) { conv_tuning().h_ri = v; return 0; }

static PPParams pp_params(const ConvPlan& q, const void* in, const void* w, int N, int Hi, int Wi, int Cin, int Cout, int Ho, int Wo,
                          int Hp) {
  PPParams p{};
  p.in = in; p.wpk = w;
  p.N = N; p.Hi = Hi; p.Wi = Wi; p.Cin = Cin; p.Cout = Cout;
  p.M = N * Ho * Wo; p.HoWo = Ho * Wo; p.Hp = Hp; p.Wp = q.Wp;
  p.magic_Wp = frmap_magic((uint32_t)p.Wp); p.magic_Hp = frmap_magic((uint32_t)p.Hp);
  p.dHoWo = frmap_div_make((uint32_t)p.HoWo); p.dWo = frmap_div_make((uint32_t)Wo); p.dWo2 = frmap_div_make(1u);
  p.nchunks = Cin / 32;
  p.tile_px = q.tile_px; p.mtiles = q.mtiles; p.ntiles = q.ntiles;
  return p;
}

template <typename TT, int WM, int NHP, int KS>
static const void* pp_kernel_3x3(const ConvPlan& q) {
  if constexpr (KS == 1 && !(WM == 4 && NHP == 3)) {
    if (q.DS) return (const void*)conv3x3_pp_kernel<TT, 7, WM, NHP, KS, true, false>;
  }
  if constexpr (KS == 1) {
    if (q.PL) return (const void*)conv3x3_pp_kernel<TT, 7, WM, NHP, KS, false, false, true>;
  }
  if constexpr (NHP != 6) {
    if (q.RI) return (const void*)conv3x3_pp_kernel<TT, 7, WM, NHP, KS, false, false, false, true>;
  }
  return q.IM ? (const void*)conv3x3_pp_kernel<TT, 7, WM, NHP, KS, false, true> : (const void*)conv3x3_pp_kernel<TT, 7, WM, NHP, KS, false, false>;
}
template <typename TT>
static const void* pp_kernel(const ConvPlan& q) {
  const int key = q.WM * 100 + q.NHP * 10 + q.KS;
  switch (q.kernel) {
    case CK_PP:
      switch (key) {
        case 231: return pp_kernel_3x3<TT, 2, 3, 1>(q);
        case 251: return pp_kernel_3x3<TT, 2, 5, 1>(q);
        case 431: return pp_kernel_3x3<TT, 4, 3, 1>(q);
        case 451: return pp_kernel_3x3<TT, 4, 5, 1>(q);
        case 242: return pp_kernel_3x3<TT, 2, 4, 2>(q);
        case 262: return pp_kernel_3x3<TT, 2, 6, 2>(q);
      }
      return nullptr;
    case CK_PP_S2:
      switch (key) {
        case 211: return (const void*)conv3x3s2_pp_kernel<TT, 7, 2, 1>;
        case 221: return (const void*)conv3x3s2_pp_kernel<TT, 7, 2, 2>;
        case 411: return (const void*)conv3x3s2_pp_kernel<TT, 7, 4, 1>;
        case 421: return (const void*)conv3x3s2_pp_kernel<TT, 7, 4, 2>;
        case 441: return (const void*)conv3x3s2_pp_kernel<TT, 7, 4, 4>;
      }
      return nullptr;
    case CK_PP_1X1:
      if (q.KS == 2) return (const void*)conv1x1_pp_kernel<TT, 7, 2, 2>;
      return q.WM == 4 ? (const void*)conv1x1_pp_kernel<TT, 7, 4, 1> : (const void*)conv1x1_pp_kernel<TT, 7, 2, 1>;
  }
  return nullptr;
}

template <typename P>
static int pp_launch(const void* kern, const ConvPlan& q, int lds, const P& p, hipStream_t st) {
  FRMAP_REQUIRE(kern, "conv_pp: no kernel for plan %d (WM %d, NHP %d, KS %d)", q.kernel, q.WM, q.NHP, q.KS);
  if (frmap_big_lds(kern, 160 * 1024)) return -2;
  void* args[] = {(void*)&p};
  (void)hipLaunchKernel(kern, dim3(q.mtiles * q.ntiles), dim3(512), args, lds, st);
  FRMAP_LAUNCH_CHECK();
  return 0;
}

int frmap_conv_pp_launch(const ConvLayer& L, const ConvPlan& q, const void* in, const void* w_packed, const float* shift,
                         const void* residual, void* out, const void* ds_in, const void* ds_w, int relu, int dtype, hipStream_t st) {
  const int Ho = L.Ho(), Wo = L.Wo(), Hp = q.kernel == CK_PP ? L.Hi + 2 : (q.kernel == CK_PP_S2 ? Ho + 1 : Ho);
  PPParams p = pp_params(q, in, w_packed, L.B, L.Hi, L.Wi, L.Cin, L.Cout, Ho, Wo, Hp);
  p.shift = shift; p.res = residual; p.out = out; p.relu = relu;
  if (q.kernel == CK_PP_1X1) p.ds_stride = L.stride;
  if (q.DS) {
    p.ds_in = ds_in; p.ds_w = ds_w; p.ds_Hi = L.ds_Hi; p.ds_Wi = L.ds_Wi; p.ds_Cin = L.ds_Cin; p.ds_stride = L.ds_stride;
    p.dsc = L.ds_Cin / 32;
  }
  if (q.PL) { p.Wo2 = L.Wi / 2; p.dWo2 = frmap_div_make((uint32_t)p.Wo2); }
  return pp_launch(dtype == FRMAP_BF16 ? pp_kernel<BF16>(q) : pp_kernel<F16>(q), q, q.lds_bytes, p, st);
}

template <int MM>
static int pp_match_launch(const ConvPlan& q, const typename PPArg<MM>::type& p, hipStream_t st) {
  int lds = q.lds_bytes;
  if (MM == MATCH_HIST && lds < VERIFY_LDS_GEMM) lds = VERIFY_LDS_GEMM;
  if (MM == MATCH_JOIN && lds < 8 * (VERIFY_QCAP * 2 + RADIUS_OB_BYTES)) lds = 8 * (VERIFY_QCAP * 2 + RADIUS_OB_BYTES);
  const void* kern = q.WM == 4 ? (const void*)conv1x1_pp_kernel<F16, 7, 4, 1, MM> : (const void*)conv1x1_pp_kernel<F16, 7, 2, 1, MM>;
  return pp_launch(kern, q, lds, p, st);
}

int frmap_match_gemm(int mode, const void* probes3, const void* gallery_packed, const float* stat_a, const float* stat_w, void* out,
                     int P, int G, int D, hipStream_t st) {
  const int K3 = 3 * D, Gpad = (G + 255) / 256 * 256;
  const FrmapVerifyGemm* v = mode == MATCH_HIST ? (const FrmapVerifyGemm*)out : nullptr;
  if (K3 % 32 || K3 > 16384 || P <= 0 || G <= 0 || (v && (v->T < 1 || v->T > VERIFY_MAX_T))) return 0;
  if (!probes3) return 1;
  const ConvPlan q = match_gemm_plan(P, Gpad);
  PPHistParams p{};
  static_cast<PPParams&>(p) = pp_params(q, probes3, gallery_packed, P, 1, 1, K3, Gpad, 1, 1, 1);
  p.ds_stride = 1;
  p.m_stat_a = stat_a; p.m_stat_w = stat_w; p.m_G = G; p.m_D = D;
  int rc;
  if (mode == MATCH_JOIN) {
    const FrmapRadiusGemm* r = (const FrmapRadiusGemm*)out;
    PPJoinParams pj{};
    static_cast<PPParams&>(pj) = p;
    pj.j_A = r->A; pj.j_B = r->B; pj.j_lab_a = r->lab_a; pj.j_lab_b = r->lab_b; pj.j_out = r->out; pj.j_rescored = r->rescored;
    pj.j_hi = r->hi; pj.j_row0 = r->row0; pj.j_filter = r->filter;
    rc = pp_match_launch<MATCH_JOIN>(q, pj, st);
  } else if (v) {
    p.h_A = v->A; p.h_B = v->B; p.h_lab_a = v->lab_a; p.h_lab_b = v->lab_b; p.h_tab = v->tab; p.h_hist = v->hist;
    p.h_rescored = v->rescored; p.h_row0 = v->row0; p.h_T = v->T;
    rc = pp_match_launch<MATCH_HIST>(q, p, st);
  } else {
    p.m_records = out;
    rc = mode == MATCH_TOPR ? pp_match_launch<MATCH_TOPR>(q, static_cast<const PPParams&>(p), st)
                            : pp_match_launch<MATCH_TOP1>(q, static_cast<const PPParams&>(p), st);
  }
  return rc ? rc : 1;
}

static bool pp_query_ok(int B, int Hi, int Wi, int Cin, int Cout) { return B > 0 && Hi > 0 && Wi > 0 && Cin > 0 && Cout > 0; }
static bool pp_inv() { return frmap_batch_invariant() != 0; }

extern "C" int frmap_conv1x1_pp_layout(int B, int Hi, int Wi, int Cin, int Cout, int stride) {
  if (!pp_query_ok(B, Hi, Wi, Cin, Cout)) return 0;
  return plan_pp_1x1(ConvLayer{B, Hi, Wi, Cin, Cout, 1, stride, 0, FUSE_NONE, 0, 0, 0, 0}, conv_tuning(), frmap_cu_count(), pp_inv()).layout;
}
extern "C" int frmap_conv3x3_pp_pool_layout(int B, int Hi, int Wi, int Cin, int Cout) {
  if (!pp_query_ok(B, Hi, Wi, Cin, Cout)) return 0;
  return plan_pp_pool(ConvLayer{B, Hi, Wi, Cin, Cout, 3, 1, 1, FUSE_POOL2, 0, 0, 0, 0}, conv_tuning(), pp_inv()).taken();
}
extern "C" int frmap_conv3x3_pp_layout(int B, int Hi, int Wi, int Cin, int Cout) {
  if (!pp_query_ok(B, Hi, Wi, Cin, Cout)) return 0;
  return plan_pp_3x3(ConvLayer{B, Hi, Wi, Cin, Cout, 3, 1, 1, FUSE_NONE, 0, 0, 0, 0}, conv_tuning(), pp_inv()).layout;
}
extern "C" int frmap_conv3x3_pp_ds_layout(int B, int Hi, int Wi, int Cin, int Cout, int ds_Hi, int ds_Wi, int ds_Cin, int ds_stride) {
  if (!pp_query_ok(B, Hi, Wi, Cin, Cout)) return 0;
  return plan_pp_3x3(ConvLayer{B, Hi, Wi, Cin, Cout, 3, 1, 1, FUSE_SHORTCUT, ds_Hi, ds_Wi, ds_Cin, ds_stride}, conv_tuning(), pp_inv()).layout;
}
extern "C" int frmap_conv3x3s2_pp_layout(int B, int Hi, int Wi, int Cin, int Cout) {
  if (!pp_query_ok(B, Hi, Wi, Cin, Cout)) return 0;
  return plan_pp_s2(ConvLayer{B, Hi, Wi, Cin, Cout, 3, 2, 1, FUSE_NONE, 0, 0, 0, 0}, conv_tuning(), pp_inv()).layout;
}
```

facerecognition-multiarchitecture-pipeline_amd/csrc/frmap_common.h:

```cpp
#pragma once
#include <hip/hip_runtime.h>
#include <stdint.h>
#include <stdio.h>

#include "../../include/frmap_hip.h"
#include "conv_plan.h"

typedef __attribute__((ext_vector_type(8))) __bf16 bf16x8_t;
typedef __attribute__((ext_vector_type(8))) _Float16 f16x8_t;
typedef __attribute__((ext_vector_type(4))) float f32x4_t;
typedef __attribute__((ext_vector_type(16))) float f32x16_t;
typedef __attribute__((ext_vector_type(4))) unsigned int u32x4_t;
typedef __attribute__((ext_vector_type(2))) unsigned int u32x2_t;

struct BF16 {
  using elem = __bf16;
  using vec8 = bf16x8_t;
  static __device__ __forceinline__ f32x4_t mfma(vec8 a, vec8 b, f32x4_t c) {
    return __builtin_amdgcn_mfma_f32_16x16x32_bf16(a, b, c, 0, 0, 0);
  }
  static __device__ __forceinline__ float to_f32(elem v) { return (float)v; }
  static __device__ __forceinline__ elem from_f32(float v) { return (elem)v; }
};
struct F16 {
// ... 364 lines not shown
    atomicAdd(o.count + i, 1);
    const int pos = w + __popcll(m & ((1ull << lane) - 1ull));
    ((int2*)obuf)[pos] = make_int2(i, j);
    ((float*)(obuf + 2 * RADIUS_OB))[pos] = dist;
  }
  w += __popcll(m);
  if (w > RADIUS_OB - NB) radius_flush(o, obuf, w, lane);
}

template <int MI>
__device__ __forceinline__ int match_epilogue_join(const f32x4_t (&acc)[MI][4], int b_base, int b_end, int n0, int G, int D, int M,
                                                   const float* __restrict__ stat_a, const float* __restrict__ stat_w,
                                                   const int32_t* __restrict__ lab_a, const int32_t* __restrict__ lab_b, int row0,
                                                   int filter, float hi, unsigned short* queue, int lane) {
  const int lr = lane & 15, g = lane >> 4;
  const float eps = 1e-6f, kf = (float)D, keps = kf * eps * eps, kap = match_kappa(3 * D);
  int cnt = 0;
#pragma unroll
  for (int mi = 0; mi < MI; ++mi) {
    const int b = b_base + mi * 16 + lr;
    const f32x4_t sa = *(const f32x4_t*)(stat_a + 4 * (size_t)min(b, M - 1));
    const float a2 = sa[0], as = sa[1], ai = sa[2], ab = sa[3] + keps;
    const int la = filter ? lab_a[min(b, M - 1)] : 0;
    const int nmin = row0 >= 0 ? row0 + b + 1 : 0;
    const float* sw_p = stat_w;
    const int32_t* lb_p = lab_b;
    asm volatile("" : "+s"(sw_p), "+s"(lb_p));
#pragma unroll
    for (int ni = 0; ni < 4; ++ni) {
#pragma unroll
      for (int j = 0; j < 4; ++j) {
        const int n = n0 + ni * 16 + 4 * g + j;
        const f32x4_t sw = *(const f32x4_t*)(sw_p + 4 * (size_t)min(n, G - 1));
        const float d2 = a2 + sw[0] - 2.f * (acc[mi][ni][j] * ai * sw[2]) + 2.f * eps * (as - sw[1]) + keps;
        const float L = d2 - kap * (ab + sw[3]);
        bool keep = n < G && b < b_end && n >= nmin && !(L > hi);
        if (filter && keep) keep = radius_filter_ok(filter, la, lb_p[min(n, G - 1)]);
        const unsigned long long m = __ballot(keep);
        if (keep) {
          const int pos = cnt + (int)__builtin_amdgcn_mbcnt_hi((unsigned)(m >> 32), __builtin_amdgcn_mbcnt_lo((unsigned)m, 0u));
          queue[pos] = (unsigned short)(((mi * 16 + lr) << 6) | (ni * 16 + 4 * g + j));
        }
        cnt += __popcll(m);
      }
    }
    __builtin_amdgcn_sched_barrier(0);
  }
  return cnt;
}

__device__ __forceinline__ void radius_drain_queue(const unsigned short* queue, int cnt, int b_base, int n0, const float* __restrict__ A,
                                                   const float* __restrict__ B, int D, const RadiusOut& o, int* obuf, int lane) {
  constexpr int NB = 8;
  int w = 0;
  for (int q0 = 0; q0 < cnt; q0 += NB) {
    const float* pa[NB];
    const float* pb[NB];
    bool valid[NB];
    int pi[NB], pj[NB];
#pragma unroll
    for (int q = 0; q < NB; ++q) {
      valid[q] = q0 + q < cnt;
      const int e = queue[valid[q] ? q0 + q : q0];
      pi[q] = b_base + (e >> 6); pj[q] = n0 + (e & 63);
      pa[q] = A + (size_t)pi[q] * D; pb[q] = B + (size_t)pj[q] * D;
    }
    double d2[NB];
    match_exact_d2_n<NB>(pa, pb, D, lane, d2);
    radius_emit<NB>(d2, valid, pi, pj, o, obuf, w, lane);
  }
  radius_flush(o, obuf, w, lane);
}

template <int MM, int MI>
__device__ __forceinline__ void match_epilogue(const f32x4_t (&acc)[MI][4], int b_base, int b_end, int n0, int G, int D, int M,
                                               const float* __restrict__ stat_a, const float* __restrict__ stat_w, void* recs,
                                               int lane) {
  if constexpr (MM == MATCH_TOP1)
    match_epilogue_records<MI>(acc, b_base, b_end, n0, G, D, M, stat_a, stat_w, (MatchRec*)recs, lane);
  else
    match_epilogue_topr<MI>(acc, b_base, b_end, n0, G, D, M, stat_a, stat_w, (MatchRecK*)recs, lane);
}

template <typename TT, int MI, int NI>
__device__ __forceinline__ void conv_epilogue(const f32x4_t (&acc)[MI][NI], char* scratch, int m_wave0, int M,
                                              int Cout, int co0, const float* __restrict__ shift,
                                              const typename TT::elem* __restrict__ res,
                                              typename TT::elem* __restrict__ out, int relu, int lane,
                                              const u32x4_t* rv_pre = nullptr) {
  constexpr int PITCH = NI * 64 + 16;
  constexpr int PARTS = NI * 2;
  constexpr int PER_LANE = PARTS / 4;
  const int lr = lane & 15, g = lane >> 4;
  float sh[PER_LANE][8];
  int part[PER_LANE], prow[PER_LANE];
#pragma unroll
  for (int j = 0; j < PER_LANE; ++j) {
    const int idx = j * 64 + lane;
    prow[j] = idx / PARTS;
    part[j] = idx % PARTS;
    const f32x4_t s0 = *(const f32x4_t*)(shift + co0 + part[j] * 8), s1 = *(const f32x4_t*)(shift + co0 + part[j] * 8 + 4);
    sh[j][0] = s0[0]; sh[j][1] = s0[1]; sh[j][2] = s0[2]; sh[j][3] = s0[3];
    sh[j][4] = s1[0]; sh[j][5] = s1[1]; sh[j][6] = s1[2]; sh[j][7] = s1[3];
  }
  u32x4_t rv[MI][PER_LANE];
  if (res) {
#pragma unroll
    for (int mi = 0; mi < MI; ++mi)
#pragma unroll
      for (int j = 0; j < PER_LANE; ++j) {
        const int m = m_wave0 + mi * 16 + prow[j];
        rv[mi][j] = (u32x4_t){0u, 0u, 0u, 0u};
        if (rv_pre) rv[mi][j] = rv_pre[mi * PER_LANE + j];
        else if (m < M) rv[mi][j] = *(const u32x4_t*)(res + (size_t)m * Cout + co0 + part[j] * 8);
      }
  }
#pragma unroll
  for (int mi = 0; mi < MI; ++mi) {
#pragma unroll
    for (int ni = 0; ni < NI; ++ni) *(f32x4_t*)(scratch + lr * PITCH + ni * 64 + g * 16) = acc[mi][ni];
#pragma unroll
    for (int j = 0; j < PER_LANE; ++j) {
      const f32x4_t a = *(const f32x4_t*)(scratch + prow[j] * PITCH + part[j] * 32);
      const f32x4_t b = *(const f32x4_t*)(scratch + prow[j] * PITCH + part[j] * 32 + 16);
      const int m = m_wave0 + mi * 16 + prow[j];
      if (m < M) {
        const size_t o = (size_t)m * Cout + co0 + part[j] * 8;
        float v[8] = {a[0] + sh[j][0], a[1] + sh[j][1], a[2] + sh[j][2], a[3] + sh[j][3],
                      b[0] + sh[j][4], b[1] + sh[j][5], b[2] + sh[j][6], b[3] + sh[j][7]};
        if (res) {
          float r[8];
          unpack8<TT>(rv[mi][j], r);
#pragma unroll
          for (int e = 0; e < 8; ++e) v[e] += r[e];
        }
        if (relu == 1) {
#pragma unroll
          for (int e = 0; e < 8; ++e) v[e] = fmaxf(v[e], 0.f);
        } else if (relu == 2) {
#pragma unroll
          for (int e = 0; e < 8; ++e) v[e] = 0.5f * v[e] * (1.0f + erff(v[e] * 0.70710678118654752f));
        }
        *(u32x4_t*)(out + o) = pack8<TT>(v);
      }
    }
  }
}

template <typename TT, int MI, int NI>
__device__ __forceinline__ void conv_epilogue_pool2(const f32x4_t (&acc)[MI][NI], char* scratch, int mp_wave0, int MP,
                                                    int Cout, int co0, const float* __restrict__ shift,
                                                    typename TT::elem* __restrict__ out, int relu, int lane) {
  constexpr int PITCH = NI * 64 + 16, PARTS = NI * 2;
  const int lr = lane & 15, g = lane >> 4;
  const bool active = lane < 4 * PARTS;
  const int win = (lane / PARTS) & 3, part = lane % PARTS;
  float sh[8];
  {
    const f32x4_t s0 = *(const f32x4_t*)(shift + co0 + part * 8), s1 = *(const f32x4_t*)(shift + co0 + part * 8 + 4);
    sh[0] = s0[0]; sh[1] = s0[1]; sh[2] = s0[2]; sh[3] = s0[3];
    sh[4] = s1[0]; sh[5] = s1[1]; sh[6] = s1[2]; sh[7] = s1[3];
  }
#pragma unroll
  for (int mi = 0; mi < MI; ++mi) {
    __builtin_amdgcn_wave_barrier();
#pragma unroll
    for (int ni = 0; ni < NI; ++ni) *(f32x4_t*)(scratch + lr * PITCH + ni * 64 + g * 16) = acc[mi][ni];
    __builtin_amdgcn_wave_barrier();
    const char* src = scratch + (win * 4) * PITCH + part * 32;
    f32x4_t a = *(const f32x4_t*)src, b = *(const f32x4_t*)(src + 16);
#pragma unroll
    for (int q = 1; q < 4; ++q) {
      const f32x4_t a2 = *(const f32x4_t*)(src + q * PITCH), b2 = *(const f32x4_t*)(src + q * PITCH + 16);
#pragma unroll
      for (int e = 0; e < 4; ++e) { a[e] = fmaxf(a[e], a2[e]); b[e] = fmaxf(b[e], b2[e]); }
    }
    const int mp = mp_wave0 + mi * 4 + win;
    if (active && mp < MP) {
      float v[8] = {a[0] + sh[0], a[1] + sh[1], a[2] + sh[2], a[3] + sh[3], b[0] + sh[4], b[1] + sh[5], b[2] + sh[6], b[3] + sh[7]};
      if (relu == 1) {
#pragma unroll
        for (int e = 0; e < 8; ++e) v[e] = fmaxf(v[e], 0.f);
      }
      *(u32x4_t*)(out + (size_t)mp * Cout + co0 + part * 8) = pack8<TT>(v);
    }
  }
}

template <int MI, int NI>
__device__ __forceinline__ void conv_epilogue_partial(const f32x4_t (&acc)[MI][NI], char* scratch, int m_wave0, int M,
                                                      int Cout, int co0, float* __restrict__ slab, int lane) {
  constexpr int PITCH = NI * 64 + 16, PARTS = NI * 2, PER_LANE = PARTS / 4;
  const int lr = lane & 15, g = lane >> 4;
#pragma unroll
  for (int mi = 0; mi < MI; ++mi) {
#pragma unroll
    for (int ni = 0; ni < NI; ++ni) *(f32x4_t*)(scratch + lr * PITCH + ni * 64 + g * 16) = acc[mi][ni];
#pragma unroll
    for (int j = 0; j < PER_LANE; ++j) {
      const int idx = j * 64 + lane, prow = idx / PARTS, part = idx % PARTS;
      const f32x4_t a = *(const f32x4_t*)(scratch + prow * PITCH + part * 32);
      const f32x4_t b = *(const f32x4_t*)(scratch + prow * PITCH + part * 32 + 16);
      const int m = m_wave0 + mi * 16 + prow;
      if (m < M) {
        float* o = slab + (size_t)m * Cout + co0 + part * 8;
        *(f32x4_t*)o = a;
        *(f32x4_t*)(o + 4) = b;
      }
    }
  }
}

__host__ __device__ inline uint32_t frmap_magic(uint32_t d) {
  return (uint32_t)(((1ull << 32) + d - 1) / d);
}
__device__ __forceinline__ uint32_t fast_div(uint32_t n, uint32_t magic) { return __umulhi(n, magic); }

struct FrmapDiv {
  uint32_t m;
  uint32_t sh;
};
__host__ inline FrmapDiv frmap_div_make(uint32_t d) {
  FrmapDiv r = {0u, 0u};
  if (d <= 1) return r;
  uint32_t k = 0;
  while ((1ull << k) < d) ++k;
  r.m = (uint32_t)((((unsigned long long)1 << (31 + k)) + d - 1) / d);
  r.sh = k - 1;
  return r;
}
__device__ __forceinline__ int frmap_div(int n, FrmapDiv d) { return d.m ? (int)(__umulhi((uint32_t)n, d.m) >> d.sh) : n; }

struct FrmapPoolOrder {
  FrmapDiv dWin, dWo2;
  int Win, Wo2;
};
__device__ __forceinline__ void frmap_pool_coords(int m, const FrmapPoolOrder& o, int& n, int& oy, int& ox) {
  const int w = m >> 2, q = m & 3;
  n = frmap_div(w, o.dWin);
  const int rem = w - n * o.Win;
  const int py = frmap_div(rem, o.dWo2);
  oy = 2 * py + (q >> 1);
  ox = 2 * (rem - py * o.Wo2) + (q & 1);
}

void frmap_set_error(const char* fmt, ...);
int frmap_big_lds(const void* kern, int bytes);
int frmap_stem_s2d(const float* x_nchw, const unsigned char* x_u8, const float* mean3, const float* std3, const void* w_packed_c3,
                   const float* shift, void* out, int B, int Hi, int Wi, int dtype, hipStream_t st);
int frmap_batch_invariant();
int frmap_cu_count();
ConvPlan frmap_conv_plan(const ConvLayer& L);
int frmap_conv_pp_launch(const ConvLayer& L, const ConvPlan& q, const void* in, const void* w_packed, const float* shift,
                         const void* residual, void* out, const void* ds_in, const void* ds_w, int relu, int dtype, hipStream_t st);
struct FrmapVerifyGemm {
  const float* A;
  const float* B;
  const int32_t* lab_a;
  const int32_t* lab_b;
  const float* tab;
  unsigned long long* hist;
  unsigned long long* rescored;
  int row0;
  int T;
};
struct FrmapRadiusGemm {
  const float* A;
  const float* B;
  const int32_t* lab_a;
  const int32_t* lab_b;
  RadiusOut out;
  unsigned long long* rescored;
  float hi;
  int row0;
  int filter;
};
int frmap_match_gemm(int mode, const void* probes3, const void* gallery_packed, const float* stat_a, const float* stat_w, void* out,
                     int P, int G, int D, hipStream_t st);
int frmap_match_topk_fill_labels(int32_t* label_out, int n, hipStream_t st);
#define FRMAP_REQUIRE(cond, ...)        \
  do {                                  \
    if (!(cond)) {                      \
      frmap_set_error(__VA_ARGS__);     \
      return -1;                        \
    }                                   \
  } while (0)
#define FRMAP_LAUNCH_CHECK()                                           \
  do {                                                                 \
    hipError_t e__ = hipGetLastError();                                \
    if (e__ != hipSuccess) {                                           \
      frmap_set_error("launch failed: %s", hipGetErrorString(e__));    \
      return -2;                                                       \
    }                                                                  \
  } while (0)
```

facerecognition-multiarchitecture-pipeline_amd/csrc/head_match.hip:

```cpp
#include "frmap_common.h"
#include <type_traits>

enum { MODE_LINEAR = 0, MODE_COS = 1, MODE_ARC = 2, MODE_DIST = 3 };

struct GemmEpi {
  const float* scale;
  const float* shift;
  int relu;
  const float* inv_a;
  const float* inv_w;
  float s;
  float m;
  int easy;
  const int64_t* label;
  unsigned int* minmax_key;
  unsigned long long* argkey;
  const float* stat_a;
  const float* stat_w;
  MatchRec* recs;
  float* out;
};

static inline int waves_blocks(int rows) { return (rows + 3) / 4; }

// ... 253 lines not shown
  const float* a = emb + (size_t)b * D;
  float ug = INFINITY;
  for (int s = lane; s < nslots; s += 64) ug = fminf(ug, recs[(size_t)s * B + b].up);
#pragma unroll
  for (int o = 32; o > 0; o >>= 1) ug = fminf(ug, __shfl_xor(ug, o, 64));
  double best = INFINITY;
  int besti = -1;
  for (int s0 = 0; s0 < nslots; s0 += 64) {
    MatchRec r; r.lo1 = INFINITY; r.idx = -1; r.lo2 = INFINITY; r.up = INFINITY;
    if (s0 + lane < nslots) r = recs[(size_t)(s0 + lane) * B + b];
    unsigned long long mask = __ballot(r.lo1 <= ug && r.idx >= 0);
    while (mask) {
      const int l = __ffsll((long long)mask) - 1;
      mask &= mask - 1;
      const int ci = __shfl(r.idx, l, 64);
      const float l2 = __shfl(r.lo2, l, 64);
      if (l2 <= ug) {
        const int g0 = (s0 + l) * slot_w, g1 = min(g0 + slot_w, G);
        for (int g = g0; g < g1; ++g) {
          const double d = match_exact_d2(a, gal + (size_t)g * D, D, lane);
          if (d < best) { best = d; besti = g; }
        }
      } else {
        const double d = match_exact_d2(a, gal + (size_t)ci * D, D, lane);
        if (d < best) { best = d; besti = ci; }
      }
    }
  }
  if (lane == 0) {
    const float d = besti >= 0 ? (float)sqrt(best) : INFINITY;
    idx_out[b] = besti; dist_out[b] = d;
    const int idt = (besti >= 0 && d <= thresh) ? besti : -1;
    if (id_thr_out) id_thr_out[b] = idt;
    if (packed_out) { packed_out[2 * b] = idt; packed_out[2 * b + 1] = __float_as_int(d); }
  }
}

__global__ __launch_bounds__(256) void match_small_kernel(const float* __restrict__ emb, const float* __restrict__ gal,
                                                          int32_t* __restrict__ idx_out, float* __restrict__ dist_out,
                                                          int32_t* __restrict__ id_thr_out, int32_t* __restrict__ packed_out,
                                                          float thresh, int B, int G, int D) {
  __shared__ float s_best[4];
  __shared__ int s_idx[4];
  const int b = blockIdx.x, lane = threadIdx.x & 63, wave = threadIdx.x >> 6;
  float best = INFINITY;
  int besti = 0x7FFFFFFF;
  for (int g0 = wave * 8; g0 < G; g0 += 32) {
    float s2[8];
#pragma unroll
    for (int j = 0; j < 8; ++j) s2[j] = 0.f;
    for (int k = lane; k < D; k += 64) {
      const float e = emb[(size_t)b * D + k];
#pragma unroll
      for (int j = 0; j < 8; ++j) {
        const int gi = min(g0 + j, G - 1);
        const float d = (e - gal[(size_t)gi * D + k]) + 1e-6f;
        s2[j] += d * d;
      }
    }
#pragma unroll
    for (int j = 0; j < 8; ++j) {
      float v = s2[j];
#pragma unroll
      for (int o = 32; o > 0; o >>= 1) v += __shfl_xor(v, o, 64);
      if (g0 + j < G && v < best) { best = v; besti = g0 + j; }
    }
  }
  if (lane == 0) { s_best[wave] = best; s_idx[wave] = besti; }
  __syncthreads();
  if (threadIdx.x == 0) {
    for (int w = 1; w < 4; ++w)
      if (s_best[w] < best || (s_best[w] == best && s_idx[w] < besti)) { best = s_best[w]; besti = s_idx[w]; }
    const bool any = besti != 0x7FFFFFFF;
    const float d = any ? sqrtf(best) : INFINITY;
    const int bi = any ? besti : -1;
    idx_out[b] = bi;
    dist_out[b] = d;
    const int idt = (any && d <= thresh) ? bi : -1;
    if (id_thr_out) id_thr_out[b] = idt;
    if (packed_out) { packed_out[2 * b] = idt; packed_out[2 * b + 1] = __float_as_int(d); }
  }
}

template <typename TT>
__global__ __launch_bounds__(256) void gap_norm_match_kernel(const typename TT::elem* __restrict__ map, const float* __restrict__ gal,
                                                             float* __restrict__ emb_out, int32_t* __restrict__ idx_out,
                                                             float* __restrict__ dist_out, int32_t* __restrict__ id_thr_out,
                                                             int32_t* __restrict__ packed_out, float thresh, int normalize,
                                                             float eps, int HW, int C, int G) {
  extern __shared__ float s_e[];
  float* s_red = s_e + C;
  int* s_idx = (int*)(s_red + 4);
  const int b = blockIdx.x, tid = threadIdx.x, lane = tid & 63, wave = tid >> 6;
  const typename TT::elem* src = map + (size_t)b * HW * C;
  const int C8 = C >> 3, nparts = C8 < 256 ? 256 / C8 : 1;
  float* s_part = s_e + C + 8;
  auto pool_group = [&](int c8, int part) {
    float a[8] = {0, 0, 0, 0, 0, 0, 0, 0};
    int s = part;
    for (; s + 15 * nparts < HW; s += 16 * nparts) {
      u32x4_t r[16];
#pragma unroll
      for (int q = 0; q < 16; ++q) r[q] = *(const u32x4_t*)(src + (size_t)(s + q * nparts) * C + c8 * 8);
#pragma unroll
      for (int q = 0; q < 16; ++q) {
        float f[8];
        unpack8<TT>(r[q], f);
#pragma unroll
        for (int j = 0; j < 8; ++j) a[j] += f[j];
      }
    }
    {
      u32x4_t r[16];
      const int n = s < HW ? (HW - 1 - s) / nparts + 1 : 0;
#pragma unroll
      for (int q = 0; q < 16; ++q) r[q] = *(const u32x4_t*)(src + (size_t)min(s + q * nparts, HW - 1) * C + c8 * 8);
#pragma unroll
      for (int q = 0; q < 16; ++q) {
        float f[8];
        unpack8<TT>(r[q], f);
        const float wq = q < n ? 1.0f : 0.0f;
#pragma unroll
        for (int j = 0; j < 8; ++j) a[j] = fmaf(wq, f[j], a[j]);
      }
    }
#pragma unroll
    for (int j = 0; j < 8; ++j) s_part[part * C + c8 * 8 + j] = a[j];
  };
  if (C8 < 256) {
    if (tid < C8 * nparts) pool_group(tid % C8, tid / C8);
  } else {
    for (int c8 = tid; c8 < C8; c8 += 256) pool_group(c8, 0);
  }
  __syncthreads();
  float ss = 0.f;
  {
    const float inv = 1.0f / (float)HW;
    for (int k = tid; k < C; k += 256) {
      float v = 0.f;
      for (int q = 0; q < nparts; ++q) v += s_part[q * C + k];
      v *= inv;
      s_e[k] = v;
      ss += v * v;
    }
  }
#pragma unroll
  for (int o = 32; o > 0; o >>= 1) ss += __shfl_xor(ss, o, 64);
  if (lane == 0) s_red[wave] = ss;
  __syncthreads();
  if (normalize) {
    const float denom = fmaxf(sqrtf(s_red[0] + s_red[1] + s_red[2] + s_red[3]), eps);
    for (int k = tid; k < C; k += 256) s_e[k] = s_e[k] / denom;
    __syncthreads();
  }
  if (emb_out)
    for (int k = tid; k < C; k += 256) emb_out[(size_t)b * C + k] = s_e[k];
  float best = INFINITY;
  int besti = 0x7FFFFFFF;
  constexpr int RPW = 10;
  for (int g0 = 0; g0 < G; g0 += 4 * RPW) {
    float s2[RPW];
#pragma unroll
    for (int j = 0; j < RPW; ++j) s2[j] = 0.f;
    for (int kk = lane * 8; kk < C; kk += 512) {
      f32x4_t r[RPW][2];
#pragma unroll
      for (int j = 0; j < RPW; ++j) {
        const float* gp = gal + (size_t)min(g0 + 4 * j + wave, G - 1) * C + kk;
        r[j][0] = *(const f32x4_t*)gp;
        r[j][1] = *(const f32x4_t*)(gp + 4);
      }
      const f32x4_t e0 = *(const f32x4_t*)(s_e + kk), e1 = *(const f32x4_t*)(s_e + kk + 4);
#pragma unroll
      for (int j = 0; j < RPW; ++j)
#pragma unroll
        for (int c = 0; c < 4; ++c) {
          const float d0 = (e0[c] - r[j][0][c]) + 1e-6f, d1 = (e1[c] - r[j][1][c]) + 1e-6f;
          s2[j] = fmaf(d0, d0, s2[j]);
          s2[j] = fmaf(d1, d1, s2[j]);
        }
    }
#pragma unroll
    for (int j = 0; j < RPW; ++j) {
      float v = s2[j];
#pragma unroll
      for (int o = 32; o > 0; o >>= 1) v += __shfl_xor(v, o, 64);
      const int gi = g0 + 4 * j + wave;
      if (gi < G && v < best) { best = v; besti = gi; }
    }
  }
  __syncthreads();
  if (lane == 0) { s_red[wave] = best; s_idx[wave] = besti; }
  __syncthreads();
  if (tid == 0) {
    for (int w = 1; w < 4; ++w)
      if (s_red[w] < best || (s_red[w] == best && s_idx[w] < besti)) { best = s_red[w]; besti = s_idx[w]; }
    const bool any = besti != 0x7FFFFFFF;
    const float d = any ? sqrtf(best) : INFINITY;
    const int bi = any ? besti : -1;
    idx_out[b] = bi;
    dist_out[b] = d;
    const int idt = (any && d <= thresh) ? bi : -1;
    if (id_thr_out) id_thr_out[b] = idt;
    if (packed_out) { packed_out[2 * b] = idt; packed_out[2 * b + 1] = __float_as_int(d); }
  }
}

extern "C" int frmap_gap_norm_match(const void* map, const float* gallery, float* emb_out, int32_t* idx_out, float* dist_out,
                                    int32_t* id_or_unknown_out, int32_t* packed_out, float thresh, int normalize, float eps,
                                    int B, int HW, int C, int G, int dtype, void* stream) {
  FRMAP_REQUIRE(map && idx_out && dist_out, "gap_norm_match: null pointer");
  FRMAP_REQUIRE(dtype == FRMAP_BF16 || dtype == FRMAP_F16, "gap_norm_match: bad dtype");
  FRMAP_REQUIRE(B > 0 && HW > 0 && C > 0 && C % 8 == 0 && C <= 4096, "gap_norm_match: bad shape B=%d HW=%d C=%d", B, HW, C);
  FRMAP_REQUIRE(G >= 0 && G <= 64 && (G == 0 || gallery), "gap_norm_match: gallery of 0..64 rows expected (got %d)", G);
  const int c8 = C / 8, nparts = c8 < 256 ? 256 / c8 : 1;
  const size_t lds = (size_t)(C + 8 + nparts * C) * sizeof(float);
  hipStream_t st = (hipStream_t)stream;
  if (dtype == FRMAP_BF16)
    hipLaunchKernelGGL(gap_norm_match_kernel<BF16>, dim3(B), dim3(256), lds, st, (const __bf16*)map, gallery, emb_out, idx_out,
                       dist_out, id_or_unknown_out, packed_out, thresh, normalize, eps, HW, C, G);
  else
    hipLaunchKernelGGL(gap_norm_match_kernel<F16>, dim3(B), dim3(256), lds, st, (const _Float16*)map, gallery, emb_out, idx_out,
                       dist_out, id_or_unknown_out, packed_out, thresh, normalize, eps, HW, C, G);
  FRMAP_LAUNCH_CHECK();
  return 0;
}

template <typename TT, int FB, int NPT>
__global__ __launch_bounds__(256) void gap_linear_norm_kernel(const typename TT::elem* __restrict__ map, const float* __restrict__ wt,
                                                              const float* __restrict__ scale, const float* __restrict__ shift,
                                                              float* __restrict__ pre_out, float* __restrict__ emb_out, float eps,
                                                              int B, int HW, int K, int relu, int stagger) {
  constexpr int N = NPT * 256;
  extern __shared__ float s_all[];
  float* s_x = s_all;
  float* s_red = s_all + K * FB;
  const int tid = threadIdx.x, lane = tid & 63, wave = tid >> 6;
  const int b0 = blockIdx.x * FB;
  const int C8 = K >> 3;
  const float inv = 1.0f / (float)HW;
  static_assert(FB == 8, "two faces per wave, four waves");
  const int nsub = C8 >= 64 ? 1 : 64 / C8;
  float* s_part = s_red + FB * 4;
  {
    const int fa = wave, fb = wave + 4;
    const typename TT::elem* sa = map + (size_t)min(b0 + fa, B - 1) * HW * K;
    const typename TT::elem* sb = map + (size_t)min(b0 + fb, B - 1) * HW * K;
    const int sub = nsub > 1 ? lane / C8 : 0;
    for (int c8 = nsub > 1 ? lane % C8 : lane; c8 < C8 && sub < nsub; c8 += 64) {
      float a[8] = {0, 0, 0, 0, 0, 0, 0, 0}, c[8] = {0, 0, 0, 0, 0, 0, 0, 0};
      for (int s0 = sub; s0 < HW; s0 += 8 * nsub) {
        u32x4_t ra[8], rb[8];
#pragma unroll
        for (int q = 0; q < 8; ++q) {
          const size_t o = (size_t)min(s0 + q * nsub, HW - 1) * K + c8 * 8;
          ra[q] = *(const u32x4_t*)(sa + o);
          rb[q] = *(const u32x4_t*)(sb + o);
        }
#pragma unroll
        for (int q = 0; q < 8; ++q) {
          float va[8], vb[8];
          unpack8<TT>(ra[q], va);
          unpack8<TT>(rb[q], vb);
          const float wq = s0 + q * nsub < HW ? 1.0f : 0.0f;
#pragma unroll
          for (int j = 0; j < 8; ++j) { a[j] = fmaf(wq, va[j], a[j]); c[j] = fmaf(wq, vb[j], c[j]); }
        }
      }
      if (nsub == 1) {
#pragma unroll
        for (int j = 0; j < 8; ++j) {
          s_x[(c8 * 8 + j) * FB + fa] = a[j] * inv;
          s_x[(c8 * 8 + j) * FB + fb] = c[j] * inv;
        }
      } else {
#pragma unroll
        for (int j = 0; j < 8; ++j) {
          s_part[((size_t)fa * nsub + sub) * K + c8 * 8 + j] = a[j];
          s_part[((size_t)fb * nsub + sub) * K + c8 * 8 + j] = c[j];
        }
      }
      if (nsub > 1) break;
    }
  }
  __syncthreads();
  if (nsub > 1) {
    for (int i = tid; i < K * FB; i += 256) {
      const int k = i / FB, f = i - k * FB;
      float v = 0.f;
      for (int q = 0; q < nsub; ++q) v += s_part[((size_t)f * nsub + q) * K + k];
      s_x[i] = v * inv;
    }
    __syncthreads();
  }
  float acc[NPT][FB];
#pragma unroll
  for (int j = 0; j < NPT; ++j)
#pragma unroll
    for (int f = 0; f < FB; ++f) acc[j][f] = 0.f;
  const int kstart = (int)(((long long)blockIdx.x * stagger) % (K / 8)) * 8;
  auto krow = [&](int it) { return it + kstart < K ? it + kstart : it + kstart - K; };
  float wc[8][NPT], wn[8][NPT];
  auto load_w = [&](float (&w)[8][NPT], int k0) {
#pragma unroll
    for (int u = 0; u < 8; ++u)
#pragma unroll
// ... 878 lines not shown
```

facerecognition-multiarchitecture-pipeline_amd/csrc/model_api.cpp:

```cpp
#include <math.h>
#include <string.h>

#include "model_api.h"

namespace {

const int kStagePlanes[4] = {64, 128, 256, 512};

bool canonical_key(int kind, const std::string& key, std::string* out) {
  static const char* feat_child[8] = {"conv1", "bn1", nullptr, nullptr, "layer1", "layer2", "layer3", "layer4"};
  auto starts = [&](const char* p) { return key.compare(0, strlen(p), p) == 0; };
  if (key.size() > 19 && key.compare(key.size() - 19, 19, "num_batches_tracked") == 0) return false;
  if (starts("features.")) {
    const size_t dot = key.find('.', 9);
    if (dot == std::string::npos) return false;
    const int idx = atoi(key.substr(9, dot - 9).c_str());
    if (idx < 0 || idx > 7 || !feat_child[idx]) return false;
    *out = std::string("trunk.") + feat_child[idx] + key.substr(dot);
    return true;
  }
  if (kind >= KIND_BASELINE) return frmap_family_key(kind, key, out);
  if (kind == KIND_CNN) {
    if (starts("resnet.fc.1.")) { *out = "fc." + key.substr(12); return true; }
    if (starts("resnet.fc.")) return false;
// ... 85 lines not shown
                     int k, int stride, int pad, PackedConv* pc, hipStream_t st, const std::vector<float>* w_override) {
  std::vector<float> scale(cout, 1.f), shift(cout, 0.f);
  if (!bnkey.empty()) frmap_model_bn_fold(m, bnkey, cout, &scale, &shift);
  if (!bkey.empty()) {
    const auto& b = m->raw.at(bkey);
    for (int o = 0; o < cout; ++o) { volatile float bs = b[o] * scale[o]; shift[o] = shift[o] + bs; }
  }
  std::vector<float> w = w_override ? *w_override : m->raw.at(wkey);
  const size_t per = (size_t)cin * k * k;
  if (!bnkey.empty())
    for (int o = 0; o < cout; ++o)
      for (size_t i = 0; i < per; ++i) w[o * per + i] *= scale[o];
  float* wdev = nullptr;
  if (hipMalloc((void**)&wdev, w.size() * sizeof(float)) != hipSuccess) { frmap_set_error("model_finalize: out of device memory"); return -2; }
  hipMemcpy(wdev, w.data(), w.size() * sizeof(float), hipMemcpyHostToDevice);
  const size_t elems = cin == 3 ? (size_t)cout * frmap_small_cin_kpad(k, k) : w.size();
  pc->wpk = frmap_model_dev_alloc(m, elems * 2);
  pc->shift = frmap_model_dev_upload(m, shift);
  pc->cout = cout; pc->cin = cin; pc->k = k; pc->stride = stride; pc->pad = pad;
  int rc = -2;
  if (pc->wpk && pc->shift)
    rc = cin == 3 ? frmap_pack_conv_weight_c3(wdev, pc->wpk, cout, k, k, m->dtype, st)
                  : frmap_pack_conv_weight(wdev, pc->wpk, cout, cin, k, k, m->dtype, st);
  hipStreamSynchronize(st);
  hipFree(wdev);
  pc->shift_host = shift;
  return rc;
}

frmap_traced::frmap_traced(frmap_run& r_, const char* fmt, double flop, double bytes) : r(r_), on(r_.m->trace && !r_.dry) {
  if (!on) return;
  snprintf(rec.kernel, sizeof(rec.kernel), fmt, r.dt);
  rec.flop = flop; rec.bytes = bytes;
  hipEventCreate(&rec.e0); hipEventCreate(&rec.e1);
  hipEventRecord(rec.e0, r.st);
}
frmap_traced::~frmap_traced() {
  if (!on) return;
  hipEventRecord(rec.e1, r.st);
  std::lock_guard<std::mutex> lock(r.m->trace_mu);
  r.m->recs.push_back(rec);
}

namespace {

auto& dev_alloc = frmap_model_dev_alloc;
auto& dev_upload = frmap_model_dev_upload;
auto& bn_fold = frmap_model_bn_fold;
int pack_conv(frmap_model* m, const std::string& wkey, const std::string& bnkey, int cout, int cin, int k, int stride, int pad,
              PackedConv* pc, std::vector<float>* shift_host, hipStream_t st) {
  const int rc = frmap_model_pack(m, wkey, "", bnkey, cout, cin, k, stride, pad, pc, st);
  if (shift_host) *shift_host = pc->shift_host;
  return rc;
}

using Run = frmap_run;
using Traced = frmap_traced;

const char* dt_name(int dtype) { return dtype == FRMAP_BF16 ? "BF16" : "F16"; }

void conv(Run& r, const PackedConv& c, const void* in, int Hi, int Wi, const void* residual, void* out, int relu) {
  if (r.rc) return;
  const int Ho = (Hi + 2 * c.pad - c.k) / c.stride + 1, Wo = (Wi + 2 * c.pad - c.k) / c.stride + 1;
  const char* name = "conv_igemm_kernel<%s>";
  if (r.m->trace && !r.dry) {
    const ConvPlan q = frmap_conv_plan(ConvLayer{r.B, Hi, Wi, c.cin, c.cout, c.k, c.stride, c.pad, residual ? FUSE_RESIDUAL : FUSE_NONE, 0, 0, 0, 0});
    if (q.taken()) name = q.label;
  }
  const double M = (double)r.B * Ho * Wo;
  Traced t(r, name, 2.0 * M * c.cout * c.cin * c.k * c.k,
           2.0 * ((double)r.B * Hi * Wi * c.cin + M * c.cout * (residual ? 2 : 1) + (double)c.cout * c.cin * c.k * c.k));
  r.rc = frmap_conv_igemm(in, c.wpk, c.shift, residual, out, r.B, Hi, Wi, c.cin, c.cout, c.k, c.stride, c.pad, relu, r.m->dtype, r.st);
}

struct MapOut { void* p; int h, w; };

size_t act_slot_bytes(int B, int H, int W) {
  const int Hc = (H - 1) / 2 + 1, Wc = (W - 1) / 2 + 1;
  const size_t conv_out = (size_t)B * Hc * Wc * 64 * 2, in4 = (size_t)B * H * W * 4 * 2;
  const size_t s = conv_out > in4 ? conv_out : in4;
  return (s + 255) / 256 * 256;
}

MapOut trunk_features(Run& r, const void* x, int x_kind, int H, int W, char* slots, size_t slot, void* final_out) {
  frmap_model* m = r.m;
  void* buf[3] = {slots, slots + slot, slots + 2 * slot};
  const int Hc = (H + 6 - 7) / 2 + 1, Wc = (W + 6 - 7) / 2 + 1;
  const int Hq = (Hc + 2 - 3) / 2 + 1, Wq = (Wc + 2 - 3) / 2 + 1;
  int cur = 0;
  const double stem_flop = 2.0 * r.B * Hc * Wc * 64 * 147;
  const double stem_out = (double)r.B * Hq * Wq * 64 * 2;
  if (x_kind == 1) {
    if (Wq <= 56 && W % 4 == 0) {
      Traced t(r, ((uintptr_t)x & 3) == 0 ? "stem_s2d_kernel<%s, U8>" : "stem_pool_u8_kernel<%s>", stem_flop, (double)r.B * H * W * 3 + stem_out);
      r.rc = frmap_stem7x7_maxpool_u8((const unsigned char*)x, m->mean, m->stdv, m->stem.wpk, m->stem.shift, buf[0], r.B, H, W, 1, m->dtype, r.st);
    } else {
      r.rc = frmap_normalize_u8_hwc((const unsigned char*)x, nullptr, buf[1], r.B, H, W, m->mean, m->stdv, m->dtype, r.st);
      if (!r.rc) r.rc = frmap_conv_small_cin(buf[1], m->stem.wpk, m->stem.shift, buf[2], r.B, H, W, 64, 7, 7, 2, 3, 1, m->dtype, r.st);
      if (!r.rc) r.rc = frmap_maxpool(buf[2], buf[0], r.B, Hc, Wc, 64, 3, 2, 1, m->dtype, r.st);
    }
  } else if (Wq <= 56) {
    Traced t(r, (W % 4 == 0 && ((uintptr_t)x & 15) == 0) ? "stem_s2d_kernel<%s>" : "stem_pool_kernel<%s>", stem_flop, (double)r.B * H * W * 3 * 4 + stem_out);
    r.rc = frmap_stem7x7_maxpool((const float*)x, m->stem.wpk, m->stem.shift, buf[0], r.B, H, W, m->dtype, r.st);
  } else {
    r.rc = frmap_pack_input_nchw_f32((const float*)x, buf[1], r.B, H, W, m->dtype, r.st);
    if (!r.rc) r.rc = frmap_conv_small_cin(buf[1], m->stem.wpk, m->stem.shift, buf[2], r.B, H, W, 64, 7, 7, 2, 3, 1, m->dtype, r.st);
    if (!r.rc) r.rc = frmap_maxpool(buf[2], buf[0], r.B, Hc, Wc, 64, 3, 2, 1, m->dtype, r.st);
  }
  int h = Hq, w = Wq;
  for (int bi = 0; bi < 8 && !r.rc; ++bi) {
    const Block& b = m->blocks[bi];
    const bool last = bi == 7 && final_out;
    void* xin = buf[cur];
    void* hb = buf[(cur + 1) % 3];
    void* third = buf[(cur + 2) % 3];
    const int ho = (h + 2 - 3) / b.c1.stride + 1, wo = (w + 2 - 3) / b.c1.stride + 1;
    conv(r, b.c1, xin, h, w, nullptr, hb, 1);
    if (!b.has_ds) {
      void* dst = last ? final_out : third;
      conv(r, b.c2, hb, ho, wo, xin, dst, 1);
      if (!last) cur = (cur + 2) % 3;
      else buf[cur] = dst;
    } else if (b.ds.k == 1 && frmap_conv_igemm_ds_supported(r.B, ho, wo, b.c2.cin, b.c2.cout, h, w, b.ds.cin, b.ds.stride)) {
      void* dst = last ? final_out : third;
      if (!r.rc) {
        const double M = (double)r.B * ho * wo;
        const char* name = "conv3x3_fast_kernel<%s, true>";
        if (m->trace && !r.dry) {
          const ConvPlan q = frmap_conv_plan(ConvLayer{r.B, ho, wo, b.c2.cin, b.c2.cout, 3, 1, 1, FUSE_SHORTCUT, h, w, b.ds.cin, b.ds.stride});
          if (q.taken()) name = q.label;
        }
        Traced t(r, name, 2.0 * M * b.c2.cout * (b.c2.cin * 9 + b.ds.cin),
                 2.0 * (M * b.c2.cin + M * b.c2.cout + (double)b.c2.cout * b.c2.cin * 9 + (double)b.c2.cout * b.ds.cin + M * b.ds.cin));
        r.rc = frmap_conv_igemm_ds(hb, b.c2.wpk, b.fshift, xin, b.ds.wpk, dst, r.B, ho, wo, b.c2.cin, b.c2.cout, h, w, b.ds.cin,
                                   b.ds.stride, 1, m->dtype, r.st);
      }
      if (!last) cur = (cur + 2) % 3;
      else buf[cur] = dst;
    } else {
      conv(r, b.ds, xin, h, w, nullptr, third, 0);
      void* dst = last ? final_out : xin;
      conv(r, b.c2, hb, ho, wo, third, dst, 1);
      if (last) buf[cur] = dst;
    }
    h = ho; w = wo;
  }
  return MapOut{buf[cur], h, w};
}

size_t align256(size_t v) { return (v + 255) / 256 * 256; }

int check_ready(const frmap_model* m, const char* what) {
  if (!m) { frmap_set_error("%s: null model", what); return -1; }
  if (!m->finalized) { frmap_set_error("%s: frmap_model_finalize has not run", what); return -1; }
  int dev = -1;
  hipGetDevice(&dev);
  if (dev != m->device) { frmap_set_error("%s: the model lives on device %d but the calling thread's current device is %d", what, m->device, dev); return -1; }
  return 0;
}

}

extern "C" int frmap_model_create(frmap_model** out, const char* model_type, int num_classes, int dtype) {
  FRMAP_REQUIRE(out && model_type, "model_create: null pointer");
  FRMAP_REQUIRE(dtype == FRMAP_BF16 || dtype == FRMAP_F16, "model_create: bad dtype %d", dtype);
  int kind;
  if (!strcmp(model_type, "cnn")) kind = KIND_CNN;
  else if (!strcmp(model_type, "arcface")) kind = KIND_ARCFACE;
  else if (!strcmp(model_type, "resnet18_trunk")) kind = KIND_TRUNK;
  else if (!strcmp(model_type, "baseline")) kind = KIND_BASELINE;
  else if (!strcmp(model_type, "siamese")) kind = KIND_SIAMESE;
  else if (!strcmp(model_type, "hybrid")) kind = KIND_HYBRID;
  else { frmap_set_error("Invalid model type: %s (model handles exist for 'baseline', 'cnn', 'siamese', 'arcface', 'hybrid', 'resnet18_trunk')", model_type); return -1; }
  FRMAP_REQUIRE(kind == KIND_TRUNK || kind == KIND_SIAMESE || num_classes > 0, "model_create: num_classes=%d", num_classes);
  frmap_model* m = new (std::nothrow) frmap_model();
  FRMAP_REQUIRE(m, "model_create: out of host memory");
  m->kind = kind; m->dtype = dtype; m->num_classes = num_classes;
  if (hipGetDevice(&m->device) != hipSuccess) { delete m; frmap_set_error("model_create: no HIP device"); return -2; }
  *out = m;
  return 0;
}

extern "C" int frmap_model_load_tensor(frmap_model* m, const char* key, const void* data, size_t numel, int on_device) {
  FRMAP_REQUIRE(m && key && data, "model_load_tensor: null pointer");
  FRMAP_REQUIRE(!m->finalized, "model_load_tensor: the model is finalized (create a new handle for new weights)");
  std::string ck;
  if (!canonical_key(m->kind, key, &ck)) return 1;
  const auto want = expected_tensors(m);
  const auto it = want.find(ck);
  if (it == want.end()) return 1;
  FRMAP_REQUIRE(it->second == numel, "model_load_tensor: %s has %zu elements, expected %zu", key, numel, it->second);
  std::vector<float> v(numel);
  if (on_device) {
    const hipError_t e = hipMemcpy(v.data(), data, numel * sizeof(float), hipMemcpyDeviceToHost);
    if (e != hipSuccess) { frmap_set_error("model_load_tensor: %s", hipGetErrorString(e)); return -2; }
  } else {
    memcpy(v.data(), data, numel * sizeof(float));
  }
  m->raw[ck] = std::move(v);
  return 0;
// ... 118 lines not shown
    return r.rc;
  }
  const MapOut map = trunk_features(r, x, x_kind, H, W, ws, slot, what == FRMAP_OUT_TRUNK_MAP ? out : nullptr);
  if (r.rc) return r.rc;
  const int HW = map.h * map.w;
  if (what == FRMAP_OUT_TRUNK_MAP) return 0;
  FRMAP_REQUIRE(m->kind != KIND_HYBRID || what == FRMAP_OUT_POOLED, "model_forward: bad output selector");
  const bool arc = m->kind == KIND_ARCFACE;
  if (what == FRMAP_OUT_POOLED || (!arc && what == FRMAP_OUT_EMBEDDING))
    return frmap_avgpool_global(map.p, (float*)out, B, HW, 512, m->dtype, r.st);
  if (!arc) {
    int rc = frmap_avgpool_global(map.p, scratch0, B, HW, 512, m->dtype, r.st);
    if (!rc) rc = frmap_linear_f32(scratch0, m->fc_w, nullptr, m->fc_b, (float*)out, B, 512, m->num_classes, 0, r.st);
    return rc;
  }
  float* emb = what == FRMAP_OUT_EMBEDDING ? (float*)out : scratch0;
  {
    Traced t(r, "gap_linear_norm_kernel<%s>", 2.0 * B * 512 * 512, 2.0 * B * HW * 512 + 4.0 * 512 * 512 + 4.0 * B * 512);
    r.rc = frmap_gap_linear_norm(map.p, m->emb_wt, m->bn_scale, m->bn_shift, nullptr, emb, 1e-12f, B, HW, 512, 512, 0, m->dtype, r.st);
  }
  if (r.rc || what == FRMAP_OUT_EMBEDDING) return r.rc;
  return frmap_linear_f32(emb, m->cls_wn, nullptr, m->cls_b, (float*)out, B, 512, m->num_classes, 0, r.st);
}

static int model_match_embedding(Run& r, const void* x, int x_kind, int H, int W, int normalize, float* emb_out, char* ws, float** emb_ptr) {
  frmap_model* m = r.m;
  const int B = r.B;
  const size_t slot = act_slot_bytes(B, H, W);
  if (m->kind >= KIND_BASELINE) {
    const size_t model_ws = frmap_model_workspace_bytes(m, B, H, W);
    float* e0 = (float*)(ws + model_ws - 2 * align256((size_t)B * 512 * sizeof(float)) - 256);
    float* e1 = e0 + align256((size_t)B * 512 * sizeof(float)) / sizeof(float);
    float* emb = emb_out ? emb_out : e0;
    if (m->kind == KIND_HYBRID) {
      int th = ((H + 6 - 7) / 2 + 1 + 2 - 3) / 2 + 1, tw = ((W + 6 - 7) / 2 + 1 + 2 - 3) / 2 + 1;
      for (int i = 0; i < 3; ++i) { th = (th - 1) / 2 + 1; tw = (tw - 1) / 2 + 1; }
      FRMAP_REQUIRE(th * tw == 49, "model_embed_and_match: HybridNet expects a 49-token feature map (224x224 input), got %d", th * tw);
      void* tmap = ws + 3 * slot;
      trunk_features(r, x, x_kind, H, W, ws, slot, tmap);
      if (r.rc) return r.rc;
      frmap_family_forward(r, nullptr, x_kind, H, W, FRMAP_OUT_EMBEDDING, normalize ? e1 : emb, normalize ? emb : nullptr,
                           ws + 3 * slot + align256((size_t)B * 49 * 512 * 2), tmap);
    } else if (m->kind == KIND_BASELINE) {
      frmap_family_forward(r, x, x_kind, H, W, FRMAP_OUT_EMBEDDING, normalize ? e1 : emb, normalize ? emb : nullptr, ws, nullptr);
    } else {
      frmap_family_forward(r, x, x_kind, H, W, FRMAP_OUT_EMBEDDING, emb, nullptr, ws, nullptr);
    }
    *emb_ptr = emb;
    return r.rc;
  }
  float* scratch0 = (float*)(ws + 3 * slot);
  float* scratch1 = (float*)(ws + 3 * slot + align256((size_t)B * 512 * sizeof(float)));
  const MapOut map = trunk_features(r, x, x_kind, H, W, ws, slot, nullptr);
  if (r.rc) return r.rc;
  const int HW = map.h * map.w;
  float* emb = emb_out ? emb_out : scratch0;
  if (m->kind == KIND_CNN) {
    r.rc = frmap_avgpool_global(map.p, normalize ? scratch1 : emb, B, HW, 512, m->dtype, r.st);
    if (!r.rc && normalize) r.rc = frmap_l2_normalize_f32(scratch1, emb, B, 512, 1e-12f, r.st);
  } else {
    Traced t(r, "gap_linear_norm_kernel<%s>", 2.0 * B * 512 * 512, 2.0 * B * HW * 512 + 4.0 * 512 * 512 + 4.0 * B * 512);
    r.rc = frmap_gap_linear_norm(map.p, m->emb_wt, m->bn_scale, m->bn_shift, nullptr, emb, 1e-12f, B, HW, 512, 512, 0, m->dtype, r.st);
  }
  *emb_ptr = emb;
  return r.rc;
}

static inline bool match_use_pack(int G, int D) { return G >= 512 && D % 32 == 0; }

extern "C" int frmap_model_embed_and_match(frmap_model* m, const void* x, int x_kind, int B, int H, int W, const float* gallery,
                                           const void* gallery_packed, const float* gallery_stat, int G, float thresh,
                                           int normalize, int32_t* idx_out, float* dist_out, int32_t* id_or_unknown_out,
                                           int32_t* packed_out, float* emb_out, void* workspace, void* stream) {
  if (int rc = check_ready(m, "model_embed_and_match")) return rc;
  FRMAP_REQUIRE(x && idx_out && dist_out && workspace, "model_embed_and_match: null pointer");
  FRMAP_REQUIRE(m->kind != KIND_TRUNK, "model_embed_and_match: a bare trunk has no embedding");
  FRMAP_REQUIRE(B > 0 && H >= 7 && W >= 7 && G >= 0 && (G == 0 || gallery), "model_embed_and_match: bad shape B=%d H=%d W=%d G=%d", B, H, W, G);
  FRMAP_REQUIRE(x_kind == FRMAP_INPUT_F32_NCHW || x_kind == FRMAP_INPUT_U8_HWC, "model_embed_and_match: bad input kind %d", x_kind);
  Run r{m, (hipStream_t)stream, B, dt_name(m->dtype)};
  char* match_ws = (char*)workspace + frmap_model_workspace_bytes(m, B, H, W);
  const int D = m->kind >= KIND_BASELINE ? frmap_model_embedding_dim(m) : 512;
  if (m->kind == KIND_CNN && G <= 64) {
    const size_t slot = act_slot_bytes(B, H, W);
    const MapOut map = trunk_features(r, x, x_kind, H, W, (char*)workspace, slot, nullptr);
    if (r.rc) return r.rc;
    const int HW = map.h * map.w;
    Traced t(r, "gap_norm_match_kernel<%s>", 2.0 * B * 512 * G, 2.0 * B * HW * 512 + 4.0 * G * 512 + 16.0 * B);
    return frmap_gap_norm_match(map.p, gallery, emb_out, idx_out, dist_out, id_or_unknown_out, packed_out, thresh, normalize ? 1 : 0,
                                1e-12f, B, HW, 512, G, m->dtype, r.st);
  }
  float* emb = nullptr;
  if (int rc = model_match_embedding(r, x, x_kind, H, W, normalize, emb_out, (char*)workspace, &emb)) return rc;
  if (m->kind >= KIND_BASELINE) {
    if (gallery_packed && gallery_stat && match_use_pack(G, D)) {
      void* split = match_ws + align256(frmap_match_workspace_bytes(B, G));
      return frmap_match_top1_packed(emb, gallery, gallery_packed, gallery_stat, idx_out, dist_out, id_or_unknown_out, packed_out, thresh,
                                     match_ws, split, B, G, D, r.st);
    }
    return frmap_match_top1(emb, gallery, idx_out, dist_out, id_or_unknown_out, packed_out, thresh, match_ws, B, G, D, r.st);
  }
  if (gallery_packed && gallery_stat && match_use_pack(G, D)) {
    void* split = match_ws + align256(frmap_match_workspace_bytes(B, G));
    Traced t(r, "match_top1 (conv1x1_pp_kernel<F16, MATCH> + finalize)", 6.0 * B * D * G, 4.0 * B * D + 6.0 * G * D + 16.0 * B);
    return frmap_match_top1_packed(emb, gallery, gallery_packed, gallery_stat, idx_out, dist_out, id_or_unknown_out, packed_out, thresh,
                                   match_ws, split, B, G, D, r.st);
  }
  Traced t(r, "match_top1 (gemm_nt_f32_kernel + finalize)", 2.0 * B * D * G, 4.0 * B * D + 4.0 * G * D + 16.0 * B);
  return frmap_match_top1(emb, gallery, idx_out, dist_out, id_or_unknown_out, packed_out, thresh, match_ws, B, G, D, r.st);
}

extern "C" size_t frmap_model_search_workspace_bytes(const frmap_model* m, int B, int H, int W, int G, int k) {
  if (!m || B <= 0) return 0;
  const size_t a = frmap_model_match_workspace_bytes(m, B, H, W, G);
  const size_t b = frmap_model_workspace_bytes(m, B, H, W) + align256(frmap_match_topk_workspace_bytes(B, G, frmap_model_embedding_dim(m), k));
  return a > b ? a : b;
}

extern "C" int frmap_model_embed_and_search(frmap_model* m, const void* x, int x_kind, int B, int H, int W, const float* gallery,
                                            const void* gallery_packed, const float* gallery_stat, const int32_t* labels, int G,
                                            int k, int normalize, int32_t* idx_out, float* dist_out, int32_t* label_out,
                                            float* emb_out, void* workspace, void* stream) {
  if (int rc = check_ready(m, "model_embed_and_search")) return rc;
  FRMAP_REQUIRE(x && idx_out && dist_out && workspace, "model_embed_and_search: null pointer");
  FRMAP_REQUIRE(m->kind != KIND_TRUNK, "model_embed_and_search: a bare trunk has no embedding");
  FRMAP_REQUIRE(k >= 1 && k <= 64, "model_embed_and_search: k=%d out of range (1 <= k <= 64)", k);
  FRMAP_REQUIRE(B > 0 && H >= 7 && W >= 7 && G >= 0 && (G == 0 || gallery), "model_embed_and_search: bad shape B=%d H=%d W=%d G=%d", B, H, W, G);
  FRMAP_REQUIRE(x_kind == FRMAP_INPUT_F32_NCHW || x_kind == FRMAP_INPUT_U8_HWC, "model_embed_and_search: bad input kind %d", x_kind);
  if (k == 1 && !labels) {
    const int rc = frmap_model_embed_and_match(m, x, x_kind, B, H, W, gallery, gallery_packed, gallery_stat, G, INFINITY, normalize,
                                               idx_out, dist_out, nullptr, nullptr, emb_out, workspace, stream);
    if (rc || !label_out) return rc;
    return frmap_match_topk_fill_labels(label_out, B, (hipStream_t)stream);
  }
  Run r{m, (hipStream_t)stream, B, dt_name(m->dtype)};
  char* match_ws = (char*)workspace + frmap_model_workspace_bytes(m, B, H, W);
  const int D = frmap_model_embedding_dim(m);
  if (m->kind == KIND_HYBRID) {
    int th = ((H + 6 - 7) / 2 + 1 + 2 - 3) / 2 + 1, tw = ((W + 6 - 7) / 2 + 1 + 2 - 3) / 2 + 1;
    for (int i = 0; i < 3; ++i) { th = (th - 1) / 2 + 1; tw = (tw - 1) / 2 + 1; }
    FRMAP_REQUIRE(th * tw == 49, "model_embed_and_search: HybridNet expects a 49-token feature map (224x224 input), got %d", th * tw);
  }
  float* emb = nullptr;
  if (int rc = model_match_embedding(r, x, x_kind, H, W, normalize, emb_out, (char*)workspace, &emb)) return rc;
  if (gallery_packed && gallery_stat && match_use_pack(G, D)) {
    Traced t(r, "match_topk (conv1x1_pp_kernel<F16, MATCH_TOPR> + finalize)", 6.0 * B * D * G, 4.0 * B * D + 6.0 * G * D + 64.0 * B * k);
    return frmap_match_topk_packed(emb, gallery, gallery_packed, gallery_stat, labels, idx_out, dist_out, label_out, match_ws, B, G, D, k, r.st);
  }
  Traced t(r, "match_topk (exact scan)", 2.0 * B * D * G, 4.0 * B * D + 4.0 * G * D + 8.0 * B * k);
  return frmap_match_topk(emb, gallery, labels, idx_out, dist_out, label_out, match_ws, B, G, D, k, r.st);
}

extern "C" int frmap_model_trace(frmap_model* m, int enable) {
  FRMAP_REQUIRE(m, "model_trace: null model");
  std::lock_guard<std::mutex> lock(m->trace_mu);
  m->trace = enable != 0;
  return 0;
}

extern "C" int frmap_model_trace_read(frmap_model* m, frmap_trace_record* out, int max_records) {
  FRMAP_REQUIRE(m && (out || max_records == 0), "model_trace_read: null pointer");
  std::lock_guard<std::mutex> lock(m->trace_mu);
  int n = 0;
  for (auto& rec : m->recs) {
    hipEventSynchronize(rec.e1);
    float ms = 0.f;
    hipEventElapsedTime(&ms, rec.e0, rec.e1);
    if (n < max_records) {
      memset(&out[n], 0, sizeof(out[n]));
      strncpy(out[n].kernel, rec.kernel, sizeof(out[n].kernel) - 1);
// ... 16 lines not shown
```

facerecognition-multiarchitecture-pipeline_amd/ops.py:

```python
from __future__ import annotations

import functools
from typing import Optional, Tuple

import numpy as np
import torch

from . import _lib

BF16, F16 = 0, 1
_DT = {torch.bfloat16: BF16, torch.float16: F16}


def _stream() -> int:
    return torch.cuda.current_stream().cuda_stream


def _on_operand_device(fn):
    @functools.wraps(fn)
    def guarded(*args, **kwargs):
        dev = None
        for v in args:
            if isinstance(v, torch.Tensor) and v.is_cuda:
                if dev is None:
# ... 103 lines not shown
        raise ValueError("stem7x7_maxpool: expected 3 input channels")
    if pool3:
        Hq, Wq = stem_pool_dims(H, W)
    else:
        Hq, Wq = ((H + 6 - 7) // 2 + 1) // 2, ((W + 6 - 7) // 2 + 1) // 2
    out = torch.empty((B, Hq, Wq, 64), dtype=dtype, device=x.device)
    fn = _lib.load().frmap_stem7x7_maxpool if pool3 else _lib.load().frmap_stem7x7_maxpool2
    _lib.check(fn(x.data_ptr(), _dev(wpk, "wpk", dtype).data_ptr(),
                                                 _dev(shift, "shift", torch.float32).data_ptr(), out.data_ptr(),
                                                 B, H, W, dt_code(dtype), _stream()), "stem7x7_maxpool")
    return out


def stem7x7_maxpool_u8(x_u8: torch.Tensor, wpk: torch.Tensor, shift: torch.Tensor, mean, std, dtype: torch.dtype,
                       pool3: bool = True) -> torch.Tensor:
    import ctypes as C
    if not isinstance(x_u8, torch.Tensor) or x_u8.dtype != torch.uint8 or x_u8.dim() != 4 or x_u8.shape[3] != 3:
        raise TypeError("stem7x7_maxpool_u8: expected a uint8 tensor of shape [B, H, W, 3]")
    x_u8 = _dev(x_u8, "stem7x7_maxpool_u8.x")
    B, H, W, _ = x_u8.shape
    if pool3:
        Hq, Wq = stem_pool_dims(H, W)
    else:
        Hq, Wq = ((H + 6 - 7) // 2 + 1) // 2, ((W + 6 - 7) // 2 + 1) // 2
    out = torch.empty((B, Hq, Wq, 64), dtype=dtype, device=x_u8.device)
    m = (C.c_float * 3)(*[float(v) for v in mean])
    sd = (C.c_float * 3)(*[float(v) for v in std])
    _lib.check(_lib.load().frmap_stem7x7_maxpool_u8(x_u8.data_ptr(), m, sd, _dev(wpk, "wpk", dtype).data_ptr(),
                                                    _dev(shift, "shift", torch.float32).data_ptr(), out.data_ptr(),
                                                    B, H, W, int(bool(pool3)), dt_code(dtype), _stream()), "stem7x7_maxpool_u8")
    return out


def conv_igemm(x: torch.Tensor, wpk: torch.Tensor, shift: torch.Tensor, Cout: int, k: int, stride: int, pad: int,
               relu, residual: Optional[torch.Tensor] = None) -> torch.Tensor:
    x = _dev(x, "conv_igemm.x")
    B, H, W, Cin = x.shape
    Ho, Wo = (H + 2 * pad - k) // stride + 1, (W + 2 * pad - k) // stride + 1
    out = torch.empty((B, Ho, Wo, Cout), dtype=x.dtype, device=x.device)
    res_ptr = 0
    if residual is not None:
        residual = _dev(residual, "conv_igemm.residual", x.dtype)
        if tuple(residual.shape) != tuple(out.shape):
            raise ValueError(f"conv_igemm: residual shape {tuple(residual.shape)} != output {tuple(out.shape)}")
        res_ptr = residual.data_ptr()
    if wpk.numel() != Cout * Cin * k * k or wpk.dtype != x.dtype:
        raise ValueError("conv_igemm: packed weight does not match Cout*Cin*k*k / dtype")
    if shift.numel() != Cout:
        raise ValueError("conv_igemm: shift must have Cout elements")
    _lib.check(_lib.load().frmap_conv_igemm(x.data_ptr(), _dev(wpk, "wpk").data_ptr(),
                                            _dev(shift, "shift", torch.float32).data_ptr(), res_ptr, out.data_ptr(),
                                            B, H, W, Cin, Cout, k, stride, pad, int(relu), dt_code(x.dtype),
                                            _stream()), "conv_igemm")
    return out


_pool2_cache: dict = {}


def conv_pool2_supported(B: int, H: int, W: int, Cin: int, Cout: int) -> bool:
    key = (B, H, W, Cin, Cout)
    if key not in _pool2_cache:
        _pool2_cache[key] = bool(_lib.load().frmap_conv_igemm_pool2_supported(B, H, W, Cin, Cout))
    return _pool2_cache[key]


def conv_pool2_form(B: int, H: int, W: int, Cin: int, Cout: int) -> int:
    return int(_lib.load().frmap_conv_igemm_pool2_form(B, H, W, Cin, Cout))


def conv_igemm_pool2(x: torch.Tensor, wpk: torch.Tensor, shift: torch.Tensor, Cout: int, relu) -> torch.Tensor:
    x = _dev(x, "conv_igemm_pool2.x")
    B, H, W, Cin = x.shape
    if wpk.numel() != Cout * Cin * 9 or wpk.dtype != x.dtype:
        raise ValueError("conv_igemm_pool2: packed weight does not match Cout*Cin*9 / dtype")
    if shift.numel() != Cout:
        raise ValueError("conv_igemm_pool2: shift must have Cout elements")
    out = torch.empty((B, H // 2, W // 2, Cout), dtype=x.dtype, device=x.device)
    _lib.check(_lib.load().frmap_conv_igemm_pool2(x.data_ptr(), _dev(wpk, "wpk").data_ptr(),
                                                  _dev(shift, "shift", torch.float32).data_ptr(), out.data_ptr(),
                                                  B, H, W, Cin, Cout, int(relu), dt_code(x.dtype), _stream()),
               "conv_igemm_pool2")
    return out


_ds_ok_cache: dict = {}


def conv_ds_supported(B: int, H: int, W: int, Cin: int, Cout: int, dsH: int, dsW: int, dsCin: int, ds_stride: int) -> bool:
    key = (B, H, W, Cin, Cout, dsH, dsW, dsCin, ds_stride)
    v = _ds_ok_cache.get(key)
    if v is None:
        v = _ds_ok_cache[key] = bool(_lib.load().frmap_conv_igemm_ds_supported(*key))
    return v


def conv_igemm_ds(x: torch.Tensor, wpk: torch.Tensor, shift: torch.Tensor, Cout: int, x_ds: torch.Tensor, wpk_ds: torch.Tensor,
                  ds_stride: int, relu) -> torch.Tensor:
    x = _dev(x, "conv_igemm_ds.x")
    x_ds = _dev(x_ds, "conv_igemm_ds.x_ds", x.dtype)
    B, H, W, Cin = x.shape
    Bd, Hd, Wd, Cd = x_ds.shape
    if Bd != B or wpk.numel() != Cout * Cin * 9 or wpk_ds.numel() != Cout * Cd or wpk.dtype != x.dtype or wpk_ds.dtype != x.dtype:
        raise ValueError("conv_igemm_ds: operand shapes / dtypes do not match")
    if shift.numel() != Cout:
        raise ValueError("conv_igemm_ds: shift must have Cout elements")
    out = torch.empty((B, H, W, Cout), dtype=x.dtype, device=x.device)
    _lib.check(_lib.load().frmap_conv_igemm_ds(x.data_ptr(), _dev(wpk, "wpk").data_ptr(),
                                               _dev(shift, "shift", torch.float32).data_ptr(), x_ds.data_ptr(),
                                               _dev(wpk_ds, "wpk_ds").data_ptr(), out.data_ptr(), B, H, W, Cin, Cout,
                                               Hd, Wd, Cd, ds_stride, int(relu), dt_code(x.dtype), _stream()), "conv_igemm_ds")
    return out


def linear_mfma(x2d: torch.Tensor, wpk: torch.Tensor, shift: torch.Tensor, N: int, act=0,
                residual: Optional[torch.Tensor] = None) -> torch.Tensor:
    x2d = _dev(x2d, "linear_mfma.x")
    M, K = x2d.shape
    out = torch.empty((M, N), dtype=x2d.dtype, device=x2d.device)
    lib = _lib.load()
    nbytes = lib.frmap_linear_mfma_workspace_bytes(M, K, N)
    ws = torch.empty((nbytes // 4,), dtype=torch.float32, device=x2d.device) if nbytes else None
    rp = 0
    if residual is not None:
        residual = _dev(residual, "linear_mfma.residual", x2d.dtype)
        if tuple(residual.shape) != (M, N):
            raise ValueError("linear_mfma: residual must be [M, N]")
        rp = residual.data_ptr()
    if wpk.numel() != N * K or wpk.dtype != x2d.dtype:
        raise ValueError("linear_mfma: packed weight does not match N*K / dtype")
    _lib.check(lib.frmap_linear_mfma(x2d.data_ptr(), _dev(wpk, "wpk").data_ptr(), _dev(shift, "shift", torch.float32).data_ptr(),
                                     rp, out.data_ptr(), ws.data_ptr() if ws is not None else 0, M, K, N, int(act),
                                     dt_code(x2d.dtype), _stream()), "linear_mfma")
    return out


def maxpool(x: torch.Tensor, k: int, stride: int, pad: int) -> torch.Tensor:
    x = _dev(x, "maxpool.x")
    B, H, W, Cc = x.shape
    Ho, Wo = (H + 2 * pad - k) // stride + 1, (W + 2 * pad - k) // stride + 1
    out = torch.empty((B, Ho, Wo, Cc), dtype=x.dtype, device=x.device)
    _lib.check(_lib.load().frmap_maxpool(x.data_ptr(), out.data_ptr(), B, H, W, Cc, k, stride, pad, dt_code(x.dtype),
                                         _stream()), "maxpool")
    return out


def avgpool_global(x: torch.Tensor) -> torch.Tensor:
    x = _dev(x, "avgpool_global.x")
    B, H, W, Cc = x.shape
    out = torch.empty((B, Cc), dtype=torch.float32, device=x.device)
    _lib.check(_lib.load().frmap_avgpool_global(x.data_ptr(), out.data_ptr(), B, H * W, Cc, dt_code(x.dtype),
                                                _stream()), "avgpool_global")
    return out


def avgpool_adaptive(x: torch.Tensor, OH: int, OW: int) -> torch.Tensor:
    x = _dev(x, "avgpool_adaptive.x")
    B, H, W, Cc = x.shape
    out = torch.empty((B, OH, OW, Cc), dtype=x.dtype, device=x.device)
    _lib.check(_lib.load().frmap_avgpool_adaptive(x.data_ptr(), out.data_ptr(), B, H, W, Cc, OH, OW,
                                                  dt_code(x.dtype), _stream()), "avgpool_adaptive")
    return out


def linear_f32(x: torch.Tensor, w: torch.Tensor, scale: Optional[torch.Tensor] = None,
               shift: Optional[torch.Tensor] = None, relu: bool = False) -> torch.Tensor:
# ... 883 lines not shown
```

include/frmap_hip.h:

```cpp
#ifndef FRMAP_HIP_H
#define FRMAP_HIP_H

#include <stddef.h>
#include <stdint.h>

#ifdef __cplusplus
extern "C" {
#endif

#define FRMAP_BF16 0
#define FRMAP_F16 1

int frmap_set_batch_invariant(int on);

int frmap_abi_version(void);
const char* frmap_last_error(void);

int frmap_pack_input_nchw_f32(const float* x_nchw, void* out_nhwc4, int B, int H, int W,
                              int dtype, void* stream);

int frmap_normalize_u8_hwc(const unsigned char* img_u8, float* out_nchw_f32, void* out_nhwc4, int B, int H,
                           int W, const float* mean3_host, const float* std3_host, int dtype, void* stream);

int frmap_resize_bilinear_u8(const unsigned char* src_pool, const void* items, const int* tables, unsigned char* out,
                             int B, int out_h, int out_w, int rows_per_block, int lds_rows, void* stream);

int frmap_crop_resize_u8(const void* frames, int n_frames, const int32_t* rois, unsigned char* out, int N, int out_h,
                         int out_w, int max_roi_h, int max_roi_w, int bgr, void* stream);
int frmap_resize_coeffs_host(int in_size, int out_size, int32_t* bounds_out, int32_t* coeffs_out, int* ksize_out);

int frmap_align_crop_resize_u8(const void* frames, int n_frames, const int32_t* rois, const double* mats, unsigned char* out, int N,
                               int out_h, int out_w, int max_roi_h, int max_roi_w, int bgr, void* stream);
int frmap_align_warp_host(const unsigned char* frame, int H, int W, long long pitch, const double* mat6, int x1, int y1, int x2,
                          int y2, int bgr, unsigned char* out);

size_t frmap_track_state_bytes(int n_streams, int max_boxes);
int frmap_track_step(void* state, const float* boxes, const float* probs, const int32_t* counts, const int32_t* frame_hw,
                     int n_streams, int max_boxes, double det_thresh, double iou_thresh, int32_t* ids_out, int32_t* rois_out,
                     void* stream);
int frmap_track_step_host(void* state, const float* boxes, const float* probs, const int32_t* counts, const int32_t* frame_hw,
                          int n_streams, int max_boxes, double det_thresh, double iou_thresh, int32_t* ids_out, int32_t* rois_out);

size_t frmap_track_fuse_state_bytes(int n_streams, int max_boxes, int dim);
int frmap_track_fuse(void* state, const int32_t* ids, const int32_t* counts, const float* emb, const int32_t* rows, int n_rows,
                     int n_streams, int max_boxes, int dim, float decay, float* fused, float* frames_out, void* stream);
int frmap_track_fuse_host(void* state, const int32_t* ids, const int32_t* counts, const float* emb, const int32_t* rows, int n_rows,
                          int n_streams, int max_boxes, int dim, float decay, float* fused, float* frames_out);

int frmap_pack_conv_weight(const float* w_oihw, void* w_packed, int Cout, int Cin, int KH, int KW,
                           int dtype, void* stream);
int frmap_small_cin_kpad(int KH, int KW);
int frmap_pack_conv_weight_c3(const float* w_oihw, void* w_packed, int Cout, int KH, int KW,
                              int dtype, void* stream);

int frmap_conv_small_cin(const void* in_nhwc4, const void* w_packed, const float* shift, void* out,
                         int B, int Hi, int Wi, int Cout, int KH, int KW, int stride, int pad,
                         int relu, int dtype, void* stream);
int frmap_conv_small_cin_pool2(const void* in_nhwc4, const void* w_packed, const float* shift, void* out,
                               int B, int Hi, int Wi, int Cout, int relu, int dtype, void* stream);

int frmap_stem7x7_maxpool(const float* x_nchw, const void* w_packed_c3, const float* shift, void* out,
                          int B, int Hi, int Wi, int dtype, void* stream);
int frmap_stem7x7_maxpool2(const float* x_nchw, const void* w_packed_c3, const float* shift, void* out,
                           int B, int Hi, int Wi, int dtype, void* stream);
int frmap_stem7x7_maxpool_u8(const unsigned char* x_u8_hwc, const float* mean3_host, const float* std3_host,
                             const void* w_packed_c3, const float* shift, void* out, int B, int Hi, int Wi,
                             int pool3, int dtype, void* stream);

int frmap_conv_igemm(const void* in, const void* w_packed, const float* shift, const void* residual,
                     void* out, int B, int Hi, int Wi, int Cin, int Cout, int K, int stride, int pad,
                     int relu, int dtype, void* stream);
int frmap_conv_igemm_pool2_supported(int B, int Hi, int Wi, int Cin, int Cout);
int frmap_conv_igemm_pool2_form(int B, int Hi, int Wi, int Cin, int Cout);
int frmap_conv1x1_pp_layout(int B, int Hi, int Wi, int Cin, int Cout, int stride);
int frmap_conv3x3_pp_pool_layout(int B, int Hi, int Wi, int Cin, int Cout);
int frmap_conv_igemm_pool2(const void* in, const void* w_packed, const float* shift, void* out, int B, int Hi,
                           int Wi, int Cin, int Cout, int relu, int dtype, void* stream);

int frmap_conv_pp_tuning(int enable, int tile_px, int bn);
int frmap_conv_pp_ri(int v);
int frmap_conv_pp_pitch(int v);
int frmap_conv_pp_ds(int v);
int frmap_conv_pp_im(int v);
int frmap_conv3x3_pp_layout(int B, int Hi, int Wi, int Cin, int Cout);
int frmap_conv3x3s2_pp_layout(int B, int Hi, int Wi, int Cin, int Cout);
int frmap_conv3x3_pp_ds_layout(int B, int Hi, int Wi, int Cin, int Cout, int ds_Hi, int ds_Wi, int ds_Cin, int ds_stride);

int frmap_conv_igemm_ds_supported(int B, int Hi, int Wi, int Cin, int Cout, int ds_Hi, int ds_Wi, int ds_Cin,
                                  int ds_stride);
int frmap_conv_igemm_ds(const void* in, const void* w_packed, const float* shift, const void* ds_in,
                        const void* ds_w_packed, void* out, int B, int Hi, int Wi, int Cin, int Cout,
                        int ds_Hi, int ds_Wi, int ds_Cin, int ds_stride, int relu, int dtype, void* stream);

size_t frmap_linear_mfma_workspace_bytes(int M, int K, int N);
int frmap_linear_mfma(const void* x, const void* w_packed, const float* shift, const void* residual,
                      void* out, void* workspace, int M, int K, int N, int act, int dtype, void* stream);

int frmap_maxpool(const void* in, void* out, int B, int H, int W, int C, int k, int stride, int pad,
                  int dtype, void* stream);
int frmap_avgpool_global(const void* in, float* out_f32, int B, int HW, int C, int dtype, void* stream);
int frmap_avgpool_adaptive(const void* in, void* out, int B, int H, int W, int C, int OH, int OW,
                           int dtype, void* stream);

int frmap_linear_f32(const float* x, const float* w, const float* scale, const float* shift,
                     float* out, int B, int K, int N, int relu, void* stream);
int frmap_l2_normalize_f32(const float* x, float* out, int B, int D, float eps, void* stream);
int frmap_cast_to_f32(const void* in, float* out, size_t n, int dtype, void* stream);
int frmap_cast_from_f32(const float* in, void* out, size_t n, int dtype, void* stream);

int frmap_add_pos_layernorm(const void* x, const float* pos, const float* gamma, const float* beta,
                            void* t_out, void* y_out, int B, int L, int D, float eps, int dtype,
                            void* stream);
int frmap_mha_tokens(const void* qkv, void* out, int B, int L, int D, int H, int dtype, void* stream);
int frmap_mean_layernorm(const void* t, const float* gamma, const float* beta, float* out_f32,
                         int B, int L, int D, float eps, int dtype, void* stream);

int frmap_cnn_attention(const void* qkv, const void* x, const float* gamma, const float* spatial_w,
                        const float* spatial_b, void* out_map, float* out_pool, int B, int H, int W, int Cq,
                        int C, int KS, int dtype, void* stream);

int frmap_softmax_argmax(const float* logits, float* probs_out, int32_t* pred_out, int B, int C, void* stream);
int frmap_pairwise_distance(const float* a, const float* b, float* dist_out, int32_t* same_out, float thresh,
                            int B, int D, void* stream);

size_t frmap_head_workspace_bytes(int B, int C);
size_t frmap_match_workspace_bytes(int B, int G);
int frmap_match_top1(const float* emb, const float* gallery, int32_t* idx_out, float* dist_out,
                     int32_t* id_or_unknown_out, int32_t* packed_out, float thresh, void* workspace,
                     int B, int G, int D, void* stream);
size_t frmap_match_gallery_pack_bytes(int G, int D);
int frmap_match_pack_gallery(const float* gallery, void* packed_out, float* stat_w_out, int G, int D, void* stream);
int frmap_match_pack_gallery_rows(const float* gallery, void* packed_out, float* stat_w_out, int row_lo, int row_hi,
                                  int G, int D, void* stream);
int frmap_match_top1_packed(const float* emb, const float* gallery, const void* gallery_packed, const float* stat_w,
                            int32_t* idx_out, float* dist_out, int32_t* id_or_unknown_out, int32_t* packed_out,
                            float thresh, void* workspace, void* probe_split, int B, int G, int D, void* stream);

size_t frmap_match_topk_workspace_bytes(int B, int G, int D, int k);
int frmap_match_topk(const float* emb, const float* gallery, const int32_t* labels, int32_t* idx_out, float* dist_out,
                     int32_t* label_out, void* workspace, int B, int G, int D, int k, void* stream);
int frmap_match_topk_packed(const float* emb, const float* gallery, const void* gallery_packed, const float* stat_w,
                            const int32_t* labels, int32_t* idx_out, float* dist_out, int32_t* label_out,
                            void* workspace, int B, int G, int D, int k, void* stream);

size_t frmap_verify_workspace_bytes(int P, int Q, int D, int T);
int frmap_verify_counts(const float* a, const int32_t* label_a, int P, const float* b, const int32_t* label_b, int Q, int D,
                        int a_row0, const float* thresholds, int T, uint64_t* accepted_out, uint64_t* rescored_out,
                        void* workspace, void* stream);
int frmap_verify_counts_packed(const float* a, const int32_t* label_a, int P, const float* b, const void* b_packed,
                               const float* stat_w, const int32_t* label_b, int Q, int D, int a_row0, const float* thresholds,
                               int T, uint64_t* accepted_out, uint64_t* rescored_out, void* workspace, void* stream);

size_t frmap_match_radius_workspace_bytes(int P, int Q, int D);
int frmap_match_radius(const float* a, const int32_t* label_a, int P, const float* b, const int32_t* label_b, int Q, int D,
                       int a_row0, float thresh, int pair_filter, int32_t* count_out, uint64_t* total_out, int32_t* pair_out,
                       float* dist_out, long long capacity, uint64_t* rescored_out, void* workspace, void* stream);
int frmap_match_radius_packed(const float* a, const int32_t* label_a, int P, const float* b, const void* b_packed,
                              const float* stat_w, const int32_t* label_b, int Q, int D, int a_row0, float thresh,
                              int pair_filter, int32_t* count_out, uint64_t* total_out, int32_t* pair_out, float* dist_out,
                              long long capacity, uint64_t* rescored_out, void* workspace, void* stream);

int frmap_gap_norm_match(const void* map, const float* gallery, float* emb_out, int32_t* idx_out, float* dist_out,
                         int32_t* id_or_unknown_out, int32_t* packed_out, float thresh, int normalize, float eps,
                         int B, int HW, int C, int G, int dtype, void* stream);
int frmap_gap_linear_norm(const void* map, const float* wt, const float* scale, const float* shift, float* pre_out,
                          float* emb_out, float eps, int B, int HW, int K, int N, int relu, int dtype, void* stream);
int frmap_cosine_logits(const float* x, const float* w, float* logits_out, int32_t* argmax_out,
                        void* workspace, int B, int C, int D, float s, void* stream);
int frmap_arcmargin_eval(const float* x, const float* w, const int64_t* label, float* logits_out,
                         float* minmax_out, void* workspace, int B, int C, int D, float s, float m,
                         int easy_margin, void* stream);

#define FRMAP_INPUT_F32_NCHW 0
#define FRMAP_INPUT_U8_HWC 1
#define FRMAP_OUT_TRUNK_MAP 0
#define FRMAP_OUT_POOLED 1
#define FRMAP_OUT_EMBEDDING 2
#define FRMAP_OUT_LOGITS 3
typedef struct frmap_model frmap_model;
typedef struct frmap_trace_record {
  char kernel[64];
  double flop;
  double bytes;
  float us;
} frmap_trace_record;
int frmap_model_create(frmap_model** out, const char* model_type, int num_classes, int dtype);
int frmap_model_load_tensor(frmap_model* m, const char* key, const void* data, size_t numel, int on_device);
int frmap_model_set_input_normalization(frmap_model* m, const float* mean3_host, const float* std3_host);
int frmap_model_finalize(frmap_model* m, void* stream);
int frmap_model_embedding_dim(const frmap_model* m);
size_t frmap_model_workspace_bytes(const frmap_model* m, int B, int H, int W);
size_t frmap_model_match_workspace_bytes(const frmap_model* m, int B, int H, int W, int G);
int frmap_model_forward(frmap_model* m, const void* x, int x_kind, int B, int H, int W, int what, void* out,
                        void* workspace, void* stream);
int frmap_model_embed_and_match(frmap_model* m, const void* x, int x_kind, int B, int H, int W, const float* gallery,
                                const void* gallery_packed, const float* gallery_stat, int G, float thresh, int normalize,
                                int32_t* idx_out, float* dist_out, int32_t* id_or_unknown_out, int32_t* packed_out,
                                float* emb_out, void* workspace, void* stream);
size_t frmap_model_search_workspace_bytes(const frmap_model* m, int B, int H, int W, int G, int k);
int frmap_model_embed_and_search(frmap_model* m, const void* x, int x_kind, int B, int H, int W, const float* gallery,
                                 const void* gallery_packed, const float* gallery_stat, const int32_t* labels, int G,
                                 int k, int normalize, int32_t* idx_out, float* dist_out, int32_t* label_out,
                                 float* emb_out, void* workspace, void* stream);
int frmap_model_trace(frmap_model* m, int enable);
int frmap_model_trace_read(frmap_model* m, frmap_trace_record* out, int max_records);
void frmap_model_destroy(frmap_model* m);

#ifdef __cplusplus
}
#endif
#endif
```

Baseline: 231,800 faces/s.

## Fuse global average pooling into final conv epilogue and pair stride-2 channel chunks

The last residual 3x3 conv of the ResNet18 trunk can now reduce its output tile to per-image channel sums in its epilogue, so the final 7x7x512 map is never written to HBM. The gap+norm+match kernel then reads the pooled sums directly. Separately, the stride-2 3x3 conv kernel gains a PAIR mode that processes two input channel chunks per outer iteration with a reordered halo/slab prefetch schedule, aimed at deepening pipelining. The fused epilogue adds an LDS staging pass and a serial per-channel sum loop at the end of the conv, and requires the whole image to fit in one tile.

New measurement: 227,300 faces/s. -2.0%, worse.

```diff
diff --git a/facerecognition-multiarchitecture-pipeline_amd/_lib.py b/facerecognition-multiarchitecture-pipeline_amd/_lib.py
--- a/facerecognition-multiarchitecture-pipeline_amd/_lib.py
+++ b/facerecognition-multiarchitecture-pipeline_amd/_lib.py
@@ -52,6 +52,12 @@
     "frmap_conv_pp_pitch": (_i, [_i]),
     "frmap_conv_pp_ds": (_i, [_i]),
     "frmap_conv_pp_im": (_i, [_i]),
+    "frmap_conv_pp_s2_pair": (_i, [_i]),
+    "frmap_conv_pp_gap": (_i, [_i]),
+    "frmap_gap_norm_match_pooled": (_i, [_vp, _vp, _vp, _vp, _vp, _vp, _vp, _f, _i, _f, _i, _i, _i, _i, _vp]),
+    "frmap_conv_igemm_gap_supported": (_i, [_i, _i, _i, _i, _i]),
+    "frmap_conv_igemm_gap_workspace_bytes": (_sz, [_i, _i, _i, _i, _i]),
+    "frmap_conv_igemm_gap": (_i, [_vp, _vp, _vp, _vp, _vp, _vp, _vp, _i, _i, _i, _i, _i, _i, _i, _vp]),
     "frmap_conv1x1_pp_layout": (_i, [_i, _i, _i, _i, _i, _i]),
     "frmap_conv3x3_pp_layout": (_i, [_i, _i, _i, _i, _i]),
     "frmap_conv3x3s2_pp_layout": (_i, [_i, _i, _i, _i, _i]),
diff --git a/facerecognition-multiarchitecture-pipeline_amd/csrc/conv_igemm.hip b/facerecognition-multiarchitecture-pipeline_amd/csrc/conv_igemm.hip
--- a/facerecognition-multiarchitecture-pipeline_amd/csrc/conv_igemm.hip
+++ b/facerecognition-multiarchitecture-pipeline_amd/csrc/conv_igemm.hip
@@ -979,7 +979,7 @@
 
 struct ConvPtrs {
   const void* in; const void* w; const float* shift; const void* res; void* out;
-  const void* ds_in; const void* ds_w; float* slab;
+  const void* ds_in; const void* ds_w; float* slab; float* gap;
 };
 
 static ConvParams conv_params(const ConvLayer& L, const ConvPlan& q, const ConvPtrs& a, int relu, int dbg) {
@@ -1034,7 +1034,7 @@
 }
 
 static int conv_run(const ConvLayer& L, const ConvPlan& q, const ConvPtrs& a, int relu, int dtype, hipStream_t st) {
-  if (q.kernel >= CK_PP) return frmap_conv_pp_launch(L, q, a.in, a.w, a.shift, a.res, a.out, a.ds_in, a.ds_w, relu, dtype, st);
+  if (q.kernel >= CK_PP) return frmap_conv_pp_launch(L, q, a.in, a.w, a.shift, a.res, a.out, a.ds_in, a.ds_w, relu, dtype, st, a.gap);
   return conv_launch(q, conv_params(L, q, a, relu, L.fuse == FUSE_POOL2 ? 0 : conv_tuning().debug), dtype, st);
 }
 
@@ -1095,6 +1095,37 @@
                 "conv_igemm_pool2: shape B=%d %dx%d Cin=%d Cout=%d not taken (even H and W, Cin %% 32 == 0, Cout %% 64 == 0, rows fit LDS)",
                 B, Hi, Wi, Cin, Cout);
   return conv_run(L, q, ConvPtrs{in, w_packed, shift, nullptr, out, nullptr, nullptr, nullptr}, relu, dtype, (hipStream_t)stream);
+}
+
+static ConvLayer gap_layer(int B, int Hi, int Wi, int Cin, int Cout, bool res) {
+  return ConvLayer{B, Hi, Wi, Cin, Cout, 3, 1, 1, res ? FUSE_RESIDUAL : FUSE_NONE, 0, 0, 0, 0};
+}
+static bool gap_shape_ok(int B, int Hi, int Wi, int Cin, int Cout) {
+  return B > 0 && Hi > 0 && Wi > 0 && Cin > 0 && Cin % 32 == 0 && Cout > 0 && Cout % 64 == 0 && (long long)B * Hi * Wi < (1ll << 31) &&
+         Wi + 2 < 32768 && Hi + 2 < 32768;
+}
+extern "C" int frmap_conv_igemm_gap_supported(int B, int Hi, int Wi, int Cin, int Cout) {
+  if (!gap_shape_ok(B, Hi, Wi, Cin, Cout)) return 0;
+  return plan_pp_gap(gap_layer(B, Hi, Wi, Cin, Cout, false), conv_tuning(), frmap_batch_invariant() != 0).taken() ? 1 : 0;
+}
+extern "C" size_t frmap_conv_igemm_gap_workspace_bytes(int B, int Hi, int Wi, int Cin, int Cout) {
+  if (!gap_shape_ok(B, Hi, Wi, Cin, Cout) || frmap_conv_igemm_gap_supported(B, Hi, Wi, Cin, Cout)) return 0;
+  return (size_t)B * Hi * Wi * Cout * 2;
+}
+extern "C" int frmap_conv_igemm_gap(const void* in, const void* w_packed, const float* shift, const void* residual, void* out,
+                                    float* pooled, void* workspace, int B, int Hi, int Wi, int Cin, int Cout, int relu, int dtype,
+                                    void* stream) {
+  FRMAP_REQUIRE(in && w_packed && shift && pooled, "conv_igemm_gap: null pointer");
+  FRMAP_REQUIRE(dtype == FRMAP_BF16 || dtype == FRMAP_F16, "conv_igemm_gap: bad dtype %d", dtype);
+  FRMAP_REQUIRE(gap_shape_ok(B, Hi, Wi, Cin, Cout), "conv_igemm_gap: bad shape B=%d %dx%d Cin=%d Cout=%d (Cin %% 32 == 0, Cout %% 64 == 0)", B, Hi, Wi, Cin, Cout);
+  const ConvLayer L = gap_layer(B, Hi, Wi, Cin, Cout, residual != nullptr);
+  const ConvPlan q = plan_pp_gap(L, conv_tuning(), frmap_batch_invariant() != 0);
+  if (q.taken())
+    return conv_run(L, q, ConvPtrs{in, w_packed, shift, residual, out, nullptr, nullptr, nullptr, pooled}, relu, dtype, (hipStream_t)stream);
+  void* map = out ? out : workspace;
+  FRMAP_REQUIRE(map, "conv_igemm_gap: this shape runs as two launches and needs `out` or a workspace (frmap_conv_igemm_gap_workspace_bytes)");
+  if (int rc = frmap_conv_igemm(in, w_packed, shift, residual, map, B, Hi, Wi, Cin, Cout, 3, 1, 1, relu, dtype, stream)) return rc;
+  return frmap_gap_sum_launch(map, pooled, B, Hi * Wi, Cout, dtype, (hipStream_t)stream);
 }
 
 extern "C" size_t frmap_linear_mfma_workspace_bytes(int M, int K, int N) {
diff --git a/facerecognition-multiarchitecture-pipeline_amd/csrc/conv_plan.cpp b/facerecognition-multiarchitecture-pipeline_amd/csrc/conv_plan.cpp
--- a/facerecognition-multiarchitecture-pipeline_amd/csrc/conv_plan.cpp
+++ b/facerecognition-multiarchitecture-pipeline_amd/csrc/conv_plan.cpp
@@ -36,7 +36,9 @@
     v.pitch = env_int("FRMAP_PP_PITCH", 0);
     v.ri = env_int("FRMAP_PP_RI", 0);
     v.im = env_int("FRMAP_PP_IM", 0);
-    v.h_on = v.h_px = v.h_bn = v.h_ks = v.h_ds = v.h_pitch = v.h_im = v.h_ri = -1;
+    v.s2_pair = env_int("FRMAP_PP_S2_PAIR", -1);
+    v.gap = env_int("FRMAP_PP_GAP", 1);
+    v.h_on = v.h_px = v.h_bn = v.h_ks = v.h_ds = v.h_pitch = v.h_im = v.h_ri = v.h_s2_pair = v.h_gap = -1;
     return v;
   }();
   return t;
@@ -57,6 +59,10 @@
     case CK_WAVE: lds = q.NCH * 9 * 4096 + 8 * (10 * 16 * 64); break;
     case CK_PP:
       lds = q.KS * (2 * q.NHP * (8 / q.KS) * 1024 + (q.RI && q.KS == 1 ? 5 : 4) * wb) + (q.DS ? ((q.WM * q.MI + 7) / 8) * 8192 : 0);
+      if (q.GP) {
+        const int copy = 2 * scratch + q.WM * q.MI * 16 * (wb / 64) * 2;
+        if (lds < copy) lds = copy;
+      }
       break;
     case CK_PP_S2: lds = 4 * q.NHP * 8192 + 4 * wb; break;
     case CK_PP_1X1: {
@@ -200,6 +206,17 @@
   q.IM = !q.RI && ConvTuning::pick(t.h_im, t.im) != 0;
   q.NHP = ks == 2 ? (nhp <= 4 ? 4 : 6) : (nhp <= 3 ? 3 : 5);
   return finish(q, "conv3x3_pp_kernel<%s>");
+}
+
+ConvPlan plan_pp_gap(const ConvLayer& L, const ConvTuning& t, bool inv) {
+  ConvPlan none{};
+  if (!ConvTuning::pick(t.h_gap, t.gap) || t.debug != 0 || L.K != 3 || L.stride != 1 || L.pad != 1) return none;
+  if (L.fuse != FUSE_NONE && L.fuse != FUSE_RESIDUAL) return none;
+  ConvPlan q = plan_pp_3x3(L, t, inv);
+  const int hw = L.Hi * L.Wi;
+  if (!q.taken() || q.DS || q.IM || q.PL || q.RI || hw > q.tile_px || q.tile_px % hw) return none;
+  q.GP = true;
+  return finish(q, "conv3x3_pp_kernel<%s, GP>");
 }
 
 ConvPlan plan_pp_s2(const ConvLayer& L, const ConvTuning& t, bool inv) {
@@ -229,6 +246,8 @@
   if (!inv && !t.forced() && (long long)q.mtiles * q.ntiles < t.min_tiles) return q;
   q.kernel = CK_PP_S2;
   q.layout = bn == 256 ? 1 : 2;
+  const int pair = ConvTuning::pick(t.h_s2_pair, t.s2_pair);
+  q.PAIR = (Cin / 32) % 2 == 0 && (pair >= 0 ? pair != 0 : q.NHP == 4);
   return finish(q, "conv3x3s2_pp_kernel<%s>");
 }
 
diff --git a/facerecognition-multiarchitecture-pipeline_amd/csrc/conv_plan.h b/facerecognition-multiarchitecture-pipeline_amd/csrc/conv_plan.h
--- a/facerecognition-multiarchitecture-pipeline_amd/csrc/conv_plan.h
+++ b/facerecognition-multiarchitecture-pipeline_amd/csrc/conv_plan.h
@@ -19,7 +19,11 @@
   int pitch;
   int ri;
   int im;
+  int gap;
+  int s2_pair;
   int h_on, h_px, h_bn, h_ks, h_ds, h_pitch, h_im, h_ri;
+  int h_gap;
+  int h_s2_pair;
 
   void set_tuning(int enable, int px, int bn_) {
     h_on = enable;
@@ -59,6 +63,8 @@
   int BM, KS, SWZ, CKS, NCH;
   int MI, WM, NHP;
   bool DS, IM, PL, RI, POOL;
+  bool GP;
+  bool PAIR;
   int tile_px, mtiles, ntiles;
   int nblocks;
   int halo_bytes, Wp, lds_bytes, ksplit;
@@ -71,6 +77,7 @@
 
 ConvPlan plan_pp_3x3(const ConvLayer& L, const ConvTuning& t, bool inv);
 ConvPlan plan_pp_s2(const ConvLayer& L, const ConvTuning& t, bool inv);
+ConvPlan plan_pp_gap(const ConvLayer& L, const ConvTuning& t, bool inv);
 ConvPlan plan_pp_pool(const ConvLayer& L, const ConvTuning& t, bool inv);
 ConvPlan plan_pp_1x1(const ConvLayer& L, const ConvTuning& t, int cus, bool inv);
 ConvPlan plan_wave(const ConvLayer& L, const ConvTuning& t, int cus);
diff --git a/facerecognition-multiarchitecture-pipeline_amd/csrc/conv_pp.hip b/facerecognition-multiarchitecture-pipeline_amd/csrc/conv_pp.hip
--- a/facerecognition-multiarchitecture-pipeline_amd/csrc/conv_pp.hip
+++ b/facerecognition-multiarchitecture-pipeline_amd/csrc/conv_pp.hip
@@ -26,6 +26,7 @@
   const float* m_stat_w;
   void* m_records;
   int m_G, m_D;
+  float* gap_out;
 };
 struct PPHistParams : PPParams {
   const float* h_A;
@@ -84,8 +85,9 @@
   (f(std::integral_constant<int, Is>{}), ...);
 }
 
-template <typename TT, int MI, int WM, int NHP, int KS, bool DS, bool IM = false, bool PL = false, bool RI = false>
+template <typename TT, int MI, int WM, int NHP, int KS, bool DS, bool IM = false, bool PL = false, bool RI = false, bool GP = false>
 __global__ __launch_bounds__(512, 2) void conv3x3_pp_kernel(const PPParams p) {
+  static_assert(!GP || (!DS && !IM && !PL && !RI), "the pooled epilogue is built for the plain burst-read form");
   static_assert(!(DS && KS == 2), "the fused shortcut is built for the pixel-split layouts only");
   static_assert(!RI || (!DS && !IM), "the interleaved fragment reads are built for the plain layers");
   static_assert(!PL || (KS == 1 && !DS && !IM), "the pooled epilogue is built for the plain pixel-split layouts");
@@ -415,7 +417,32 @@
         }
     }
     __syncthreads();
-    if (grp == 1) return;
+    if (!GP && grp == 1) return;
+  }
+  if constexpr (GP) {
+    constexpr int SCR = 8 * (16 * (NI * 64 + 16));
+    char* stage = smem + SCR;
+    const int mw0 = m0 + mslice * (MI * 16);
+    if (!(KS == 2 && grp == 1))
+      conv_epilogue<TT, MI, NI, true>(acc, smem + (KS == 2 ? q : wave) * (16 * (NI * 64 + 16)), mw0, mend, p.Cout, nt * BN + wn * 64,
+                                      p.shift, (const elem*)p.res, (elem*)p.out, p.relu, lane, nullptr,
+                                      stage + ((mw0 - m0) * BN + wn * 64) * (int)sizeof(elem), BN * (int)sizeof(elem));
+    __syncthreads();
+    const int nimg = frmap_div(mend - m0, p.dHoWo);
+    for (int e = tid; e < nimg * (BN / 2); e += 512) {
+      const int i = e / (BN / 2), c2 = e - i * (BN / 2);
+      const char* s = stage + ((i * p.HoWo) * BN + c2 * 2) * (int)sizeof(elem);
+      float a0 = 0.f, a1 = 0.f;
+#pragma unroll 7
+      for (int px = 0; px < p.HoWo; ++px) {
+        float f[8];
+        unpack8<TT>((u32x4_t){*(const unsigned*)(s + px * (BN * (int)sizeof(elem))), 0u, 0u, 0u}, f);
+        a0 += f[0]; a1 += f[1];
+      }
+      float* o = p.gap_out + (size_t)(n0 + i) * p.Cout + nt * BN + c2 * 2;
+      o[0] = a0; o[1] = a1;
+    }
+    return;
   }
 
   if constexpr (PL)
@@ -596,7 +623,7 @@
                             nt * BN + wn * 64, p.shift, (const elem*)p.res, (elem*)p.out, p.relu, lane);
 }
 
-template <typename TT, int MI, int WM, int NHP2>
+template <typename TT, int MI, int WM, int NHP2, bool PAIR = false>
 __global__ __launch_bounds__(512, 2) void conv3x3s2_pp_kernel(const PPParams p) {
   constexpr int NI = 4, WN = 8 / WM;
   constexpr int TAPS = 9, BN = WN * 64, WB = BN * 64;
@@ -663,19 +690,24 @@
     pp_dma16(s, d);
     if (NWI == 2) pp_dma16(s + 1024, d + 1024);
   };
-  auto issue_img = [&](int ci, int sp, int j) {
+  auto issue_img = [&](int ci, int sp, int slot, int j) {
     const int off = (sp >> 1) * rowb + (sp & 1) * pxb + ci * 64;
     const bool live = ci < nch && ((hval >> j) & 1u);
     const char* s = live ? hsrc[j] + off : (ci < nch ? hsrc[j] : (const char*)g_pp_zero);
-    pp_dma16(s, hdst + (unsigned)sp * HB + j * 8192);
+    pp_dma16(s, hdst + (unsigned)slot * HB + j * 8192);
   };
-
-#pragma unroll
-  for (int sp = 0; sp < 3; ++sp)
-#pragma unroll
-    for (int j = 0; j < NHP2; ++j) issue_img(0, sp, j);
-  issue_slab(0, 0, 0);
-  issue_slab(0, 1, 1);
+  constexpr int PCH_OF[18] = {0, 1, 0, 0, 1, 1, 0, 0, 1, 1, 0, 0, 0, 0, 1, 1, 1, 1};
+  constexpr int PT_OF[18] = {0, 0, 1, 2, 1, 2, 3, 4, 3, 4, 5, 6, 7, 8, 5, 6, 7, 8};
+
+#pragma unroll
+  for (int i = 0; i < 3; ++i)
+#pragma unroll
+    for (int j = 0; j < NHP2; ++j) {
+      if (PAIR) issue_img(i & 1, i >> 1, i, j);
+      else issue_img(0, i, i, j);
+    }
+  issue_slab(PAIR ? PCH_OF[0] : 0, 0, 0);
+  issue_slab(PAIR ? PCH_OF[1] : 0, PAIR ? PT_OF[1] : 1, 1);
 
   int A[MI];
 #pragma unroll
@@ -697,40 +729,81 @@
   pp_barrier();
   if (grp == 1) pp_barrier();
 
-  for (int ci = 0; ci < nch; ++ci) {
-    pp_static_for(std::make_integer_sequence<int, TAPS>{}, [&](auto tc) {
-      constexpr int t = decltype(tc)::value;
-      const int k = ci * TAPS + t;
-      vec8 wf[NI], pf[MI];
-      {
-        const char* sl = slabs + (k & (RING - 1)) * WB;
-#pragma unroll
-        for (int ni = 0; ni < NI; ++ni) wf[ni] = *(const vec8*)(sl + ni * 1024);
-        const char* hb = smem + IMG_OF[t] * HB;
-        const int toff = (A1_OF[t] * p.Wp + B1_OF[t]) << 6;
-#pragma unroll
-        for (int mi = 0; mi < MI; ++mi) {
-          const int at = A[mi] + toff;
-          pf[mi] = *(const vec8*)(hb + (at ^ ((at >> 3) & 32)));
+  if constexpr (PAIR) {
+    for (int pi = 0; pi < (nch >> 1); ++pi) {
+      pp_static_for(std::make_integer_sequence<int, 2 * TAPS>{}, [&](auto uc) {
+        constexpr int u = decltype(uc)::value, t = PT_OF[u];
+        constexpr int slot = (2 * IMG_OF[t] + PCH_OF[u]) & 3;
+        const int k = pi * (2 * TAPS) + u;
+        vec8 wf[NI], pf[MI];
+        {
+          const char* sl = slabs + (k & (RING - 1)) * WB;
+#pragma unroll
+          for (int ni = 0; ni < NI; ++ni) wf[ni] = *(const vec8*)(sl + ni * 1024);
+          const char* hb = smem + slot * HB;
+          const int toff = (A1_OF[t] * p.Wp + B1_OF[t]) << 6;
+#pragma unroll
+          for (int mi = 0; mi < MI; ++mi) {
+            const int at = A[mi] + toff;
+            pf[mi] = *(const vec8*)(hb + (at ^ ((at >> 3) & 32)));
+          }
         }
-      }
-      constexpr int NH = t >= 1 ? ((NHP2 == 1 && ((t - 1) & 1)) ? 0 : PPH) : 0;
-      if (t >= 1) {
-        constexpr int qi = (t - 1) >> 1, h = (t - 1) & 1;
-#pragma unroll
-        for (int e = 0; e < NH; ++e) issue_img(qi == 0 ? ci : ci + 1, qi == 0 ? 3 : qi - 1, h * PPH + e);
-      }
-      issue_slab(t + 2 < TAPS ? ci : ci + 1, (t + 2) % TAPS, (k + 2) & (RING - 1));
-      pp_wait_vm<NWI + NH>();
-      pp_barrier();
-      pp_wait_lgkm0();
-      __builtin_amdgcn_sched_barrier(0);
-#pragma unroll
-      for (int ni = 0; ni < NI; ++ni)
-#pragma unroll
-        for (int mi = 0; mi < MI; ++mi) acc[mi][ni] = TT::mfma(wf[ni], pf[mi], acc[mi][ni]);
-      pp_barrier();
-    });
+        constexpr bool ISS = u >= 1 && u <= 16;
+        constexpr int NH = ISS ? ((NHP2 == 1 && ((u - 1) & 1)) ? 0 : PPH) : 0;
+        if (ISS) {
+          constexpr int gi = ((u - 1) >> 1) + 3, h = (u - 1) & 1, ii = gi & 7;
+#pragma unroll
+          for (int e = 0; e < NH; ++e) issue_img(2 * (gi >= 8 ? pi + 1 : pi) + (ii & 1), ii >> 1, ii & 3, h * PPH + e);
+        }
+        constexpr int u2 = (u + 2) % (2 * TAPS);
+        issue_slab(2 * (u + 2 < 2 * TAPS ? pi : pi + 1) + PCH_OF[u2], PT_OF[u2], (k + 2) & (RING - 1));
+        pp_wait_vm<NWI + NH>();
+        pp_barrier();
+        pp_wait_lgkm0();
+        __builtin_amdgcn_sched_barrier(0);
+#pragma unroll
+        for (int ni = 0; ni < NI; ++ni)
+#pragma unroll
+          for (int mi = 0; mi < MI; ++mi) acc[mi][ni] = TT::mfma(wf[ni], pf[mi], acc[mi][ni]);
+        pp_barrier();
+      });
+    }
+  } else {
+    for (int ci = 0; ci < nch; ++ci) {
+      pp_static_for(std::make_integer_sequence<int, TAPS>{}, [&](auto tc) {
+        constexpr int t = decltype(tc)::value;
+        const int k = ci * TAPS + t;
+        vec8 wf[NI], pf[MI];
+        {
+          const char* sl = slabs + (k & (RING - 1)) * WB;
+  #pragma unroll
+          for (int ni = 0; ni < NI; ++ni) wf[ni] = *(const vec8*)(sl + ni * 1024);
+          const char* hb = smem + IMG_OF[t] * HB;
+          const int toff = (A1_OF[t] * p.Wp + B1_OF[t]) << 6;
+  #pragma unroll
+          for (int mi = 0; mi < MI; ++mi) {
+            const int at = A[mi] + toff;
+            pf[mi] = *(const vec8*)(hb + (at ^ ((at >> 3) & 32)));
+          }
+        }
+        constexpr int NH = t >= 1 ? ((NHP2 == 1 && ((t - 1) & 1)) ? 0 : PPH) : 0;
+        if (t >= 1) {
+          constexpr int qi = (t - 1) >> 1, h = (t - 1) & 1;
+  #pragma unroll
+          for (int e = 0; e < NH; ++e) issue_img(qi == 0 ? ci : ci + 1, qi == 0 ? 3 : qi - 1, qi == 0 ? 3 : qi - 1, h * PPH + e);
+        }
+        issue_slab(t + 2 < TAPS ? ci : ci + 1, (t + 2) % TAPS, (k + 2) & (RING - 1));
+        pp_wait_vm<NWI + NH>();
+        pp_barrier();
+        pp_wait_lgkm0();
+        __builtin_amdgcn_sched_barrier(0);
+  #pragma unroll
+        for (int ni = 0; ni < NI; ++ni)
+  #pragma unroll
+          for (int mi = 0; mi < MI; ++mi) acc[mi][ni] = TT::mfma(wf[ni], pf[mi], acc[mi][ni]);
+        pp_barrier();
+      });
+    }
   }
   if (grp == 0) pp_barrier();
   pp_wait_vm<0>();
@@ -745,6 +818,8 @@
 extern "C" int frmap_conv_pp_ds(int v) { conv_tuning().h_ds = v; return 0; }
 extern "C" int frmap_conv_pp_im(int v) { conv_tuning().h_im = v; return 0; }
 extern "C" int frmap_conv_pp_ri(int v) { conv_tuning().h_ri = v; return 0; }
+extern "C" int frmap_conv_pp_gap(int v) { conv_tuning().h_gap = v; return 0; }
+extern "C" int frmap_conv_pp_s2_pair(int v) { conv_tuning().h_s2_pair = v; return 0; }
 
 static PPParams pp_params(const ConvPlan& q, const void* in, const void* w, int N, int Hi, int Wi, int Cin, int Cout, int Ho, int Wo,
                           int Hp) {
@@ -761,6 +836,7 @@
 
 template <typename TT, int WM, int NHP, int KS>
 static const void* pp_kernel_3x3(const ConvPlan& q) {
+  if (q.GP) return (const void*)conv3x3_pp_kernel<TT, 7, WM, NHP, KS, false, false, false, false, true>;
   if constexpr (KS == 1 && !(WM == 4 && NHP == 3)) {
     if (q.DS) return (const void*)conv3x3_pp_kernel<TT, 7, WM, NHP, KS, true, false>;
   }
@@ -788,11 +864,11 @@
       return nullptr;
     case CK_PP_S2:
       switch (key) {
-        case 211: return (const void*)conv3x3s2_pp_kernel<TT, 7, 2, 1>;
-        case 221: return (const void*)conv3x3s2_pp_kernel<TT, 7, 2, 2>;
-        case 411: return (const void*)conv3x3s2_pp_kernel<TT, 7, 4, 1>;
-        case 421: return (const void*)conv3x3s2_pp_kernel<TT, 7, 4, 2>;
-        case 441: return (const void*)conv3x3s2_pp_kernel<TT, 7, 4, 4>;
+        case 211: return q.PAIR ? (const void*)conv3x3s2_pp_kernel<TT, 7, 2, 1, true> : (const void*)conv3x3s2_pp_kernel<TT, 7, 2, 1>;
+        case 221: return q.PAIR ? (const void*)conv3x3s2_pp_kernel<TT, 7, 2, 2, true> : (const void*)conv3x3s2_pp_kernel<TT, 7, 2, 2>;
+        case 411: return q.PAIR ? (const void*)conv3x3s2_pp_kernel<TT, 7, 4, 1, true> : (const void*)conv3x3s2_pp_kernel<TT, 7, 4, 1>;
+        case 421: return q.PAIR ? (const void*)conv3x3s2_pp_kernel<TT, 7, 4, 2, true> : (const void*)conv3x3s2_pp_kernel<TT, 7, 4, 2>;
+        case 441: return q.PAIR ? (const void*)conv3x3s2_pp_kernel<TT, 7, 4, 4, true> : (const void*)conv3x3s2_pp_kernel<TT, 7, 4, 4>;
       }
       return nullptr;
     case CK_PP_1X1:
@@ -813,10 +889,13 @@
 }
 
 int frmap_conv_pp_launch(const ConvLayer& L, const ConvPlan& q, const void* in, const void* w_packed, const float* shift,
-                         const void* residual, void* out, const void* ds_in, const void* ds_w, int relu, int dtype, hipStream_t st) {
+                         const void* residual, void* out, const void* ds_in, const void* ds_w, int relu, int dtype, hipStream_t st,
+                         float* gap_out) {
   const int Ho = L.Ho(), Wo = L.Wo(), Hp = q.kernel == CK_PP ? L.Hi + 2 : (q.kernel == CK_PP_S2 ? Ho + 1 : Ho);
   PPParams p = pp_params(q, in, w_packed, L.B, L.Hi, L.Wi, L.Cin, L.Cout, Ho, Wo, Hp);
   p.shift = shift; p.res = residual; p.out = out; p.relu = relu;
+  FRMAP_REQUIRE(!q.GP == !gap_out, "conv_pp: the pooled form and its output go together");
+  p.gap_out = gap_out;
   if (q.kernel == CK_PP_1X1) p.ds_stride = L.stride;
   if (q.DS) {
     p.ds_in = ds_in; p.ds_w = ds_w; p.ds_Hi = L.ds_Hi; p.ds_Wi = L.ds_Wi; p.ds_Cin = L.ds_Cin; p.ds_stride = L.ds_stride;
@@ -824,6 +903,29 @@
   }
   if (q.PL) { p.Wo2 = L.Wi / 2; p.dWo2 = frmap_div_make((uint32_t)p.Wo2); }
   return pp_launch(dtype == FRMAP_BF16 ? pp_kernel<BF16>(q) : pp_kernel<F16>(q), q, q.lds_bytes, p, st);
+}
+
+template <typename TT>
+__global__ __launch_bounds__(256) void gap_sum_kernel(const typename TT::elem* __restrict__ map, float* __restrict__ sums, int B, int HW, int C) {
+  const long long e = (long long)blockIdx.x * 256 + threadIdx.x, C2 = C / 2;
+  if (e >= (long long)B * C2) return;
+  const int n = (int)(e / C2), c2 = (int)(e - (long long)n * C2);
+  const typename TT::elem* s = map + (size_t)n * HW * C + c2 * 2;
+  float a0 = 0.f, a1 = 0.f;
+  for (int px = 0; px < HW; ++px) {
+    float f[8];
+    unpack8<TT>((u32x4_t){*(const unsigned*)(s + (size_t)px * C), 0u, 0u, 0u}, f);
+    a0 += f[0]; a1 += f[1];
+  }
+  sums[(size_t)n * C + c2 * 2] = a0;
+  sums[(size_t)n * C + c2 * 2 + 1] = a1;
+}
+int frmap_gap_sum_launch(const void* map, float* sums, int B, int HW, int C, int dtype, hipStream_t st) {
+  const long long n = (long long)B * (C / 2);
+  if (dtype == FRMAP_BF16) hipLaunchKernelGGL(gap_sum_kernel<BF16>, dim3((unsigned)((n + 255) / 256)), dim3(256), 0, st, (const __bf16*)map, sums, B, HW, C);
+  else hipLaunchKernelGGL(gap_sum_kernel<F16>, dim3((unsigned)((n + 255) / 256)), dim3(256), 0, st, (const _Float16*)map, sums, B, HW, C);
+  FRMAP_LAUNCH_CHECK();
+  return 0;
 }
 
 template <int MM>
diff --git a/facerecognition-multiarchitecture-pipeline_amd/csrc/frmap_common.h b/facerecognition-multiarchitecture-pipeline_amd/csrc/frmap_common.h
--- a/facerecognition-multiarchitecture-pipeline_amd/csrc/frmap_common.h
+++ b/facerecognition-multiarchitecture-pipeline_amd/csrc/frmap_common.h
@@ -470,12 +470,12 @@
     match_epilogue_topr<MI>(acc, b_base, b_end, n0, G, D, M, stat_a, stat_w, (MatchRecK*)recs, lane);
 }
 
-template <typename TT, int MI, int NI>
+template <typename TT, int MI, int NI, bool STAGE = false>
 __device__ __forceinline__ void conv_epilogue(const f32x4_t (&acc)[MI][NI], char* scratch, int m_wave0, int M,
                                               int Cout, int co0, const float* __restrict__ shift,
                                               const typename TT::elem* __restrict__ res,
                                               typename TT::elem* __restrict__ out, int relu, int lane,
-                                              const u32x4_t* rv_pre = nullptr) {
+                                              const u32x4_t* rv_pre = nullptr, char* stage = nullptr, int stage_pitch = 0) {
   constexpr int PITCH = NI * 64 + 16;
   constexpr int PARTS = NI * 2;
   constexpr int PER_LANE = PARTS / 4;
@@ -529,7 +529,13 @@
 #pragma unroll
           for (int e = 0; e < 8; ++e) v[e] = 0.5f * v[e] * (1.0f + erff(v[e] * 0.70710678118654752f));
         }
-        *(u32x4_t*)(out + o) = pack8<TT>(v);
+        if constexpr (STAGE) {
+          const u32x4_t pk = pack8<TT>(v);
+          if (out) *(u32x4_t*)(out + o) = pk;
+          *(u32x4_t*)(stage + (mi * 16 + prow[j]) * stage_pitch + part[j] * 16) = pk;
+        } else {
+          *(u32x4_t*)(out + o) = pack8<TT>(v);
+        }
       }
     }
   }
@@ -640,7 +646,9 @@
 int frmap_cu_count();
 ConvPlan frmap_conv_plan(const ConvLayer& L);
 int frmap_conv_pp_launch(const ConvLayer& L, const ConvPlan& q, const void* in, const void* w_packed, const float* shift,
-                         const void* residual, void* out, const void* ds_in, const void* ds_w, int relu, int dtype, hipStream_t st);
+                         const void* residual, void* out, const void* ds_in, const void* ds_w, int relu, int dtype, hipStream_t st,
+                         float* gap_out = nullptr);
+int frmap_gap_sum_launch(const void* map, float* sums, int B, int HW, int C, int dtype, hipStream_t st);
 struct FrmapVerifyGemm {
   const float* A;
   const float* B;
diff --git a/facerecognition-multiarchitecture-pipeline_amd/csrc/head_match.hip b/facerecognition-multiarchitecture-pipeline_amd/csrc/head_match.hip
--- a/facerecognition-multiarchitecture-pipeline_amd/csrc/head_match.hip
+++ b/facerecognition-multiarchitecture-pipeline_amd/csrc/head_match.hip
@@ -359,7 +359,7 @@
   }
 }
 
-template <typename TT>
+template <typename TT, bool POOLED = false>
 __global__ __launch_bounds__(256) void gap_norm_match_kernel(const typename TT::elem* __restrict__ map, const float* __restrict__ gal,
                                                              float* __restrict__ emb_out, int32_t* __restrict__ idx_out,
                                                              float* __restrict__ dist_out, int32_t* __restrict__ id_thr_out,
@@ -404,18 +404,22 @@
 #pragma unroll
     for (int j = 0; j < 8; ++j) s_part[part * C + c8 * 8 + j] = a[j];
   };
-  if (C8 < 256) {
-    if (tid < C8 * nparts) pool_group(tid % C8, tid / C8);
-  } else {
-    for (int c8 = tid; c8 < C8; c8 += 256) pool_group(c8, 0);
-  }
-  __syncthreads();
+  if constexpr (!POOLED) {
+    if (C8 < 256) {
+      if (tid < C8 * nparts) pool_group(tid % C8, tid / C8);
+    } else {
+      for (int c8 = tid; c8 < C8; c8 += 256) pool_group(c8, 0);
+    }
+    __syncthreads();
+  }
   float ss = 0.f;
   {
     const float inv = 1.0f / (float)HW;
     for (int k = tid; k < C; k += 256) {
       float v = 0.f;
-      for (int q = 0; q < nparts; ++q) v += s_part[q * C + k];
+      if constexpr (POOLED) v = ((const float*)map)[(size_t)b * C + k];
+      else
+        for (int q = 0; q < nparts; ++q) v += s_part[q * C + k];
       v *= inv;
       s_e[k] = v;
       ss += v * v;
@@ -499,6 +503,19 @@
   else
     hipLaunchKernelGGL(gap_norm_match_kernel<F16>, dim3(B), dim3(256), lds, st, (const _Float16*)map, gallery, emb_out, idx_out,
                        dist_out, id_or_unknown_out, packed_out, thresh, normalize, eps, HW, C, G);
+  FRMAP_LAUNCH_CHECK();
+  return 0;
+}
+
+extern "C" int frmap_gap_norm_match_pooled(const float* sums, const float* gallery, float* emb_out, int32_t* idx_out, float* dist_out,
+                                           int32_t* id_or_unknown_out, int32_t* packed_out, float thresh, int normalize, float eps,
+                                           int B, int HW, int C, int G, void* stream) {
+  FRMAP_REQUIRE(sums && idx_out && dist_out, "gap_norm_match_pooled: null pointer");
+  FRMAP_REQUIRE(B > 0 && HW > 0 && C > 0 && C % 8 == 0 && C <= 4096, "gap_norm_match_pooled: bad shape B=%d HW=%d C=%d", B, HW, C);
+  FRMAP_REQUIRE(G >= 0 && G <= 64 && (G == 0 || gallery), "gap_norm_match_pooled: gallery of 0..64 rows expected (got %d)", G);
+  const size_t lds = (size_t)(C + 8) * sizeof(float);
+  hipLaunchKernelGGL((gap_norm_match_kernel<BF16, true>), dim3(B), dim3(256), lds, (hipStream_t)stream, (const __bf16*)(const void*)sums,
+                     gallery, emb_out, idx_out, dist_out, id_or_unknown_out, packed_out, thresh, normalize, eps, HW, C, G);
   FRMAP_LAUNCH_CHECK();
   return 0;
 }
diff --git a/facerecognition-multiarchitecture-pipeline_amd/csrc/model_api.cpp b/facerecognition-multiarchitecture-pipeline_amd/csrc/model_api.cpp
--- a/facerecognition-multiarchitecture-pipeline_amd/csrc/model_api.cpp
+++ b/facerecognition-multiarchitecture-pipeline_amd/csrc/model_api.cpp
@@ -191,7 +191,8 @@
   return (s + 255) / 256 * 256;
 }
 
-MapOut trunk_features(Run& r, const void* x, int x_kind, int H, int W, char* slots, size_t slot, void* final_out) {
+MapOut trunk_features(Run& r, const void* x, int x_kind, int H, int W, char* slots, size_t slot, void* final_out,
+                      float* pooled_sums = nullptr) {
   frmap_model* m = r.m;
   void* buf[3] = {slots, slots + slot, slots + 2 * slot};
   const int Hc = (H + 6 - 7) / 2 + 1, Wc = (W + 6 - 7) / 2 + 1;
@@ -225,6 +226,15 @@
     void* third = buf[(cur + 2) % 3];
     const int ho = (h + 2 - 3) / b.c1.stride + 1, wo = (w + 2 - 3) / b.c1.stride + 1;
     conv(r, b.c1, xin, h, w, nullptr, hb, 1);
+    if (!b.has_ds && bi == 7 && pooled_sums && !final_out && !r.rc && b.c2.k == 3 && b.c2.stride == 1 &&
+        frmap_conv_igemm_gap_supported(r.B, ho, wo, b.c2.cin, b.c2.cout)) {
+      const double M = (double)r.B * ho * wo;
+      Traced t(r, "conv3x3_pp_kernel<%s, GP>", 2.0 * M * b.c2.cout * b.c2.cin * 9,
+               2.0 * (2.0 * M * b.c2.cin + (double)b.c2.cout * b.c2.cin * 9) + 4.0 * r.B * b.c2.cout);
+      r.rc = frmap_conv_igemm_gap(hb, b.c2.wpk, b.c2.shift, xin, nullptr, pooled_sums, nullptr, r.B, ho, wo, b.c2.cin, b.c2.cout, 1,
+                                  m->dtype, r.st);
+      return MapOut{nullptr, ho, wo};
+    }
     if (!b.has_ds) {
       void* dst = last ? final_out : third;
       conv(r, b.c2, hb, ho, wo, xin, dst, 1);
@@ -509,9 +519,15 @@
   const int D = m->kind >= KIND_BASELINE ? frmap_model_embedding_dim(m) : 512;
   if (m->kind == KIND_CNN && G <= 64) {
     const size_t slot = act_slot_bytes(B, H, W);
-    const MapOut map = trunk_features(r, x, x_kind, H, W, (char*)workspace, slot, nullptr);
+    float* sums = (float*)((char*)workspace + 3 * slot);
+    const MapOut map = trunk_features(r, x, x_kind, H, W, (char*)workspace, slot, nullptr, sums);
     if (r.rc) return r.rc;
     const int HW = map.h * map.w;
+    if (!map.p) {
+      Traced t(r, "gap_norm_match_kernel<%s, POOLED>", 2.0 * B * 512 * G, 4.0 * B * 512 + 4.0 * G * 512 + 16.0 * B);
+      return frmap_gap_norm_match_pooled(sums, gallery, emb_out, idx_out, dist_out, id_or_unknown_out, packed_out, thresh, normalize ? 1 : 0,
+                                         1e-12f, B, HW, 512, G, r.st);
+    }
     Traced t(r, "gap_norm_match_kernel<%s>", 2.0 * B * 512 * G, 2.0 * B * HW * 512 + 4.0 * G * 512 + 16.0 * B);
     return frmap_gap_norm_match(map.p, gallery, emb_out, idx_out, dist_out, id_or_unknown_out, packed_out, thresh, normalize ? 1 : 0,
                                 1e-12f, B, HW, 512, G, m->dtype, r.st);
diff --git a/facerecognition-multiarchitecture-pipeline_amd/ops.py b/facerecognition-multiarchitecture-pipeline_amd/ops.py
--- a/facerecognition-multiarchitecture-pipeline_amd/ops.py
+++ b/facerecognition-multiarchitecture-pipeline_amd/ops.py
@@ -209,6 +209,35 @@
                                                   B, H, W, Cin, Cout, int(relu), dt_code(x.dtype), _stream()),
                "conv_igemm_pool2")
     return out
+
+
+def conv_gap_supported(B: int, H: int, W: int, Cin: int, Cout: int) -> bool:
+    return bool(_lib.load().frmap_conv_igemm_gap_supported(B, H, W, Cin, Cout))
+
+
+def conv_igemm_gap(x: torch.Tensor, wpk: torch.Tensor, shift: torch.Tensor, Cout: int, relu, residual: Optional[torch.Tensor] = None,
+                   want_map: bool = True):
+    x = _dev(x, "conv_igemm_gap.x")
+    B, H, W, Cin = x.shape
+    if wpk.numel() != Cout * Cin * 9 or wpk.dtype != x.dtype:
+        raise ValueError("conv_igemm_gap: packed weight does not match Cout*Cin*9 / dtype")
+    if shift.numel() != Cout:
+        raise ValueError("conv_igemm_gap: shift must have Cout elements")
+    res_ptr = 0
+    if residual is not None:
+        residual = _dev(residual, "conv_igemm_gap.residual", x.dtype)
+        if tuple(residual.shape) != (B, H, W, Cout):
+            raise ValueError(f"conv_igemm_gap: residual shape {tuple(residual.shape)} != output {(B, H, W, Cout)}")
+        res_ptr = residual.data_ptr()
+    lib = _lib.load()
+    out = torch.empty((B, H, W, Cout), dtype=x.dtype, device=x.device) if want_map else None
+    sums = torch.empty((B, Cout), dtype=torch.float32, device=x.device)
+    nws = 0 if want_map else int(lib.frmap_conv_igemm_gap_workspace_bytes(B, H, W, Cin, Cout))
+    ws = torch.empty((nws,), dtype=torch.uint8, device=x.device) if nws else None
+    _lib.check(lib.frmap_conv_igemm_gap(x.data_ptr(), _dev(wpk, "wpk").data_ptr(), _dev(shift, "shift", torch.float32).data_ptr(), res_ptr,
+                                        out.data_ptr() if out is not None else 0, sums.data_ptr(), ws.data_ptr() if ws is not None else 0,
+                                        B, H, W, Cin, Cout, int(relu), dt_code(x.dtype), _stream()), "conv_igemm_gap")
+    return out, sums
 
 
 _ds_ok_cache: dict = {}
diff --git a/include/frmap_hip.h b/include/frmap_hip.h
--- a/include/frmap_hip.h
+++ b/include/frmap_hip.h
@@ -82,6 +82,12 @@
 int frmap_conv_pp_pitch(int v);
 int frmap_conv_pp_ds(int v);
 int frmap_conv_pp_im(int v);
+int frmap_conv_igemm_gap_supported(int B, int Hi, int Wi, int Cin, int Cout);
+size_t frmap_conv_igemm_gap_workspace_bytes(int B, int Hi, int Wi, int Cin, int Cout);
+int frmap_conv_igemm_gap(const void* in, const void* w_packed, const float* shift, const void* residual, void* out, float* pooled,
+                         void* workspace, int B, int Hi, int Wi, int Cin, int Cout, int relu, int dtype, void* stream);
+int frmap_conv_pp_gap(int v);
+int frmap_conv_pp_s2_pair(int v);
 int frmap_conv3x3_pp_layout(int B, int Hi, int Wi, int Cin, int Cout);
 int frmap_conv3x3s2_pp_layout(int B, int Hi, int Wi, int Cin, int Cout);
 int frmap_conv3x3_pp_ds_layout(int B, int Hi, int Wi, int Cin, int Cout, int ds_Hi, int ds_Wi, int ds_Cin, int ds_stride);
@@ -160,6 +166,9 @@
                               int pair_filter, int32_t* count_out, uint64_t* total_out, int32_t* pair_out, float* dist_out,
                               long long capacity, uint64_t* rescored_out, void* workspace, void* stream);
 
+int frmap_gap_norm_match_pooled(const float* sums, const float* gallery, float* emb_out, int32_t* idx_out, float* dist_out,
+                                int32_t* id_or_unknown_out, int32_t* packed_out, float thresh, int normalize, float eps, int B,
+                                int HW, int C, int G, void* stream);
 int frmap_gap_norm_match(const void* map, const float* gallery, float* emb_out, int32_t* idx_out, float* dist_out,
                          int32_t* id_or_unknown_out, int32_t* packed_out, float thresh, int normalize, float eps,
                          int B, int HW, int C, int G, int dtype, void* stream);
```
